# hyperplane-lab/RGBManip

Hardware: AMD Instinct MI355X
Metric: adapose_poses_per_sec_batch256 (higher is better)
Workload: dtype bf16

## Files before the change

### include/rgbm.h

```cpp
#ifndef RGBM_H_
#define RGBM_H_
#include <stddef.h>
#include <stdint.h>

#ifdef __cplusplus
extern "C" {
#endif

#define RGBM_VERSION 100
#define RGBM_F32 0
#define RGBM_BF16 1
#define RGBM_F16 2
#define RGBM_BF16X3 3

int rgbm_version(void);
const char* rgbm_last_error(void);

typedef struct rgbm_weight_desc {
  const char* name;
  const float* data;
  int ndim;
  const int64_t* shape;
} rgbm_weight_desc;

// ... 15 lines not shown
int rgbm_adapose_set_dropout(rgbm_adapose_t* h, float p, uint64_t seed);
int rgbm_adapose_dropout_masks(rgbm_adapose_t* h, int B, float* out_dev);
int rgbm_adapose_set_dropout_masks(rgbm_adapose_t* h, int B, const float* masks_dev);
int rgbm_adapose_forward(rgbm_adapose_t* h, int B, const float* img1, const float* img2, const int32_t* choose1,
                         const int32_t* choose2, const float* P1, const float* P2, const float* depths, void* workspace,
                         size_t workspace_bytes, const rgbm_adapose_out* out, void* stream);

int rgbm_adapose_postprocess(int B, int P, int img_size, const float* nocs1, const float* depth1, const float* r1,
                             const int32_t* choose1, const double* Kcrop, const double* E1, double* bbox_world, double* ts,
                             int32_t* valid, void* stream);
int rgbm_adapose_postprocess_scratch_bytes(int B, size_t* bytes);
int rgbm_adapose_postprocess_ws(int B, int P, int img_size, const float* nocs1, const float* depth1, const float* r1,
                                const int32_t* choose1, const double* Kcrop, const double* E1, double* bbox_world, double* ts,
                                int32_t* valid, void* scratch, size_t scratch_bytes, void* stream);

int rgbm_adapose_postprocess_regressed(int B, int P, const float* nocs1, const float* r1, const float* t1, const float* s1,
                                       const double* E1, double* bbox_world, double* ts, int32_t* valid, void* stream);

int rgbm_adapose_postprocess_ransac(int B, int P, int img_size, uint32_t seed, const float* nocs1, const float* depth1,
                                    const int32_t* choose1, const double* Kcrop, const double* E1, double* bbox_world, double* srt,
                                    int32_t* valid, void* stream);
int rgbm_adapose_postprocess_pnp(int B, int P, uint32_t seed, const float* nocs1, const float* pts2d1, const float* nocs2,
                                 const float* pts2d2, const double* K, const double* E1, const double* E2, double* bbox_out,
                                 double* srt_out, int32_t* info_out, int32_t* valid_out, void* stream);

int rgbm_prepare_inputs(const float* rgb_dev, const uint8_t* mask_dev, const double* K_dev, int N, int H, int W, int S, int P,
                        uint32_t seed, float* img_out, int32_t* choose_out, float* pts2d_out, double* Kcrop_out,
                        int32_t* window_out, int32_t* valid_out, uint8_t* scratch, void* stream);

int rgbm_prepare_inputs_indexed(const float* rgb_dev, const uint8_t* mask_dev, const double* K_dev, const int32_t* frame_map_dev,
                                int N, int H, int W, int S, int P, uint32_t seed, float* img_out, int32_t* choose_out,
                                float* pts2d_out, double* Kcrop_out, int32_t* window_out, int32_t* valid_out, uint8_t* scratch,
                                void* stream);
int rgbm_prepare_inputs_ex(const float* rgb_dev, const uint8_t* mask_dev, const double* K_dev, const int32_t* frame_map_dev,
                           int frame0, int N, int H, int W, int S, int P, uint32_t seed, float* img_out, int32_t* choose_out,
                           float* pts2d_out, double* Kcrop_out, int32_t* window_out, int32_t* valid_out, uint8_t* scratch,
                           void* stream);
int rgbm_prepare_inputs_u8(const uint8_t* rgb_dev, const uint8_t* mask_dev, const double* K_dev, const int32_t* frame_map_dev,
                           int frame0, int N, int H, int W, int S, int P, uint32_t seed, float* img_out, int32_t* choose_out,
                           float* pts2d_out, double* Kcrop_out, int32_t* window_out, int32_t* valid_out, uint8_t* scratch,
                           void* stream);
int rgbm_prepare_inputs_opt(const void* rgb_dev, int pixel_type, int normalize, const uint8_t* mask_dev, const double* K_dev,
                            const int32_t* frame_map_dev, int frame0, int N, int H, int W, int S, int P, uint32_t seed, float* img_out,
                            int32_t* choose_out, float* pts2d_out, double* Kcrop_out, int32_t* window_out, int32_t* valid_out,
                            uint8_t* scratch, void* stream);
int rgbm_prepare_inputs_windows(const void* pix_dev, int pixel_type, int normalize, const uint8_t* mask_pix_dev, const int64_t* offset_dev,
                                const int32_t* window_dev, const int32_t* valid_in_dev, const double* K_dev, int frame0, int N, int H, int W,
                                int S, int P, uint32_t seed, float* img_out, int32_t* choose_out, float* pts2d_out, double* Kcrop_out,
                                int32_t* valid_out, uint8_t* scratch, void* stream);
int rgbm_quantize_frames(const float* src_dev, uint8_t* dst_dev, size_t n, void* stream);

int rgbm_projection(const double* Kcrop_dev, const double* E_dev, float* P_dev, int N, void* stream);
int rgbm_mask_extent(const uint8_t* mask_dev, int N, int H, int W, int32_t* ext_out, int32_t* count_out, void* stream);

int rgbm_lookat_quat(const double* dir_dev, int N, int batch_zero, double* quat_dev, void* stream);
int rgbm_control_action_to_pose(const float* action_dev, int lda, const double* pose_mid, const double* pose_min,
                                const double* pose_max, int N, double* pose_dev, void* stream);
typedef struct rgbm_control_reward_args {
  const float* action;
  const double* cam_pose;
  const double* target;
  const float* move_success;
  const double* bbox;
  const double* avail;
  const double* gt_bbox;
  const double* pred_bbox;
  const double* pose_cur;
  const double* pose_prev;
  const double* robot_pose;
  const double* success;
  double* reward;
  double* terms;
  double coef[14];
  double proper_pos[3];
  double precision2;
  int N, T, lda, pots, first;
  int pad_;
} rgbm_control_reward_args;
int rgbm_control_reward(const rgbm_control_reward_args* args, void* stream);
int rgbm_control_grasp_frame(const double* est_dev, int N, double* center_dev, double* direction_dev, void* stream);

typedef struct rgbm_synth_scene {
  const double* cam_pose;
  const double* robot_pose;
  const double* box;
  double fx, fy, cx, cy;
  int N, H, W, env0;
} rgbm_synth_scene;
int rgbm_synth_camera(const rgbm_synth_scene* scene, double* K_dev, double* E_dev, double* rays_dev, void* stream);
int rgbm_synth_render(const rgbm_synth_scene* scene, const double* rays_dev, float* color_dev, uint8_t* mask_dev, void* stream);
int rgbm_synth_render_u8(const rgbm_synth_scene* scene, const double* rays_dev, uint8_t* color_dev, uint8_t* mask_dev,
                         int32_t* extent_dev, int32_t* count_dev, void* stream);

int rgbm_gae(int T, int N, const float* rewards, const uint8_t* dones, const float* values, const float* last_values,
             float gamma, float lam, float* returns, float* adv, double* sums, void* stream);
int rgbm_adv_normalise(int64_t n_local, float* adv, const double* sums, double count_total, void* stream);

typedef struct rgbm_policy_layout {
  int dims[5];
  int log_std;
  int w[2][4];
  int b[2][4];
  int total;
} rgbm_policy_layout;
int rgbm_policy_forward(const float* params, const rgbm_policy_layout* L, int n, int mode, const float* obs, const float* noise,
                        float* actions, float* logp, float* value, float* mu, void* stream);
int rgbm_ppo_partial_floats(const rgbm_policy_layout* L, int n, size_t* count);
int rgbm_ppo_minibatch_fwd_bwd(const float* params, const rgbm_policy_layout* L, int n, const float* obs, const float* actions,
                               const float* old_logp, const float* adv, const float* returns, const float* old_values,
                               const float* old_mu, const float* old_log_std, float clip, float vcoef, float ecoef,
                               float* partial_scratch, float* grads_flat, void* stream);
int rgbm_ppo_clip_adam(float* params, const float* grads_flat, float* exp_avg, float* exp_avg_sq, void* opt_state,
                       const rgbm_policy_layout* L, float inv_world, float max_norm, float desired_kl, float lr_min,
                       float lr_max, int adaptive, void* stream);

#define RGBM_POLICY_MAX_HIDDEN 6
#define RGBM_POLICY_MAX_WIDTH 512
#define RGBM_POLICY_MAX_ACT 32
#define RGBM_ACT_ELU 0
#define RGBM_ACT_SELU 1
#define RGBM_ACT_RELU 2
#define RGBM_ACT_LRELU 3
#define RGBM_ACT_TANH 4
#define RGBM_ACT_SIGMOID 5
typedef struct rgbm_policy_desc {
  int obs_dim, state_dim, act_dim;
  int activation;
  int asymmetric;
  int n_hidden[2];
  int hidden[2][RGBM_POLICY_MAX_HIDDEN];
  int w[2][RGBM_POLICY_MAX_HIDDEN + 1];
  int b[2][RGBM_POLICY_MAX_HIDDEN + 1];
  int log_std;
  int total;
} rgbm_policy_desc;
int rgbm_policy_forward_ex(const float* params, const rgbm_policy_desc* D, int n, int mode, const float* obs, const float* states,
                           const float* noise, float* actions, float* logp, float* value, float* mu, void* stream);
int rgbm_ppo_scratch_floats_ex(const rgbm_policy_desc* D, int n, int clipped_value_loss, size_t* count);
int rgbm_ppo_minibatch_fwd_bwd_ex(const float* params, const rgbm_policy_desc* D, int n, const float* obs, const float* states,
                                  const float* actions, const float* old_logp, const float* adv, const float* returns,
                                  const float* old_values, const float* old_mu, const float* old_log_std, float clip, float vcoef,
                                  float ecoef, int clipped_value_loss, float* scratch, float* grads_flat, void* stream);
int rgbm_ppo_clip_adam_ex(float* params, const float* grads_flat, float* exp_avg, float* exp_avg_sq, void* opt_state, int total,
                          float inv_world, float max_norm, float desired_kl, float lr_min, float lr_max, int adaptive, void* stream);

int rgbm_conv_nd(int dtype, const void* in_dev, int N, int D, int H, int W, int Cin, int Cin_pad, const float* w_host,
                 int Cout, int Cout_pad, int KD, int KH, int KW, int stride_d, int stride_hw, int pad_d, int pad_hw,
                 int dil_hw, int transposed, const float* bias_host, const float* bn_scale_host, const float* bn_shift_host,
                 const void* res_dev, int res_mode, int act, float slope, void* out_dev, void* stream);
#define RGBM_CONV_PLAN_INTS 9
int rgbm_conv_plan(int dtype, int N, int D, int H, int W, int Cin, int Cin_pad, int Cout, int Cout_pad, int KD, int KH, int KW,
                   int stride_d, int stride_hw, int pad_d, int pad_hw, int dil_hw, int transposed, int has_bias, int res_mode, int act,
                   int cls, int n_cu, int32_t* plan);
int rgbm_bn_per_sample_scratch_bytes(int V, size_t* bytes);
int rgbm_bn_per_sample(int dtype, void* y_dev, const void* res_dev, const float* gamma_dev, const float* beta_dev, void* scratch_dev,
                       int V, int64_t nvox, int C, int relu, void* stream);
int rgbm_conv3d_tile(int layer, int dtype, const void* in_dev, int N, int D, int H, int W, const float* w_host,
                     const float* bn_scale_host, const float* bn_shift_host, const void* res_dev, void* out_dev, void* stream);
int rgbm_upsample_conv3x3(int dtype, const void* in_dev, int V, int h, int w, int Cin, const float* w_host, int Cout,
                          const float* bias_host, int act, float slope, void* z_scratch_dev, void* out_dev, void* stream);
int rgbm_upsample_conv3x3_final(int dtype, const void* in_dev, int V, int h, int w, const float* w3_host, const float* b3_host,
                                float slope, const float* wf_host, const float* bf_host, void* out_dev, int out_f32, void* stream);
int rgbm_stem(int dtype, const float* img1_dev, const float* img2_dev, const float* w_host, void* out_dev, int B, int S, void* stream);
int rgbm_maxpool3x3s2(int dtype, const void* in_dev, void* out_dev, int V, int H, int W, int C, void* stream);
int rgbm_resize_bilinear_ac(int dtype, const void* in_dev, void* out_dev, int V, int Hs, int Ws, int C, int Ho, int Wo,
                            void* stream);
int rgbm_adaptive_avgpool(int dtype, const void* in_dev, void* out_dev, int V, int H, int W, int C, int S, void* stream);
int rgbm_build_volume(int dtype, const void* feat_dev, const float* P_views_dev, const float* depths_dev, float* homog_scratch,
                      void* vol_dev, int V, int B, int D, int H, int W, void* stream);
int rgbm_conv0_sweep(const void* feat_dev, const float* P_views_dev, const float* depths_dev, float* homog_scratch,
                     const float* w_host, const float* bn_scale_host, const float* bn_shift_host, void* out_dev,
                     int V, int B, int D, int H, int W, void* stream);
int rgbm_conv0_sweep_dt(int dtype, const void* feat_dev, const float* P_views_dev, const float* depths_dev, float* homog_scratch,
                        const float* w_host, const float* bn_scale_host, const float* bn_shift_host, void* out_dev,
                        int V, int B, int D, int H, int W, void* stream);
int rgbm_conv0_sweep_f16feat(const void* feat_f16_dev, const float* P_views_dev, const float* depths_dev, float* homog_scratch,
                             const float* w_host, const float* bn_scale_host, const float* bn_shift_host, void* out_bf16_dev,
                             int V, int B, int D, int H, int W, void* stream);
int rgbm_adapose_forward_ex(rgbm_adapose_t* h, int B, const float* img1, const float* img2, const int32_t* choose1,
                            const int32_t* choose2, const float* P1, const float* P2, const float* depths, void* workspace,
                            size_t workspace_bytes, const rgbm_adapose_out* out, int stop_after, void* stream);
int rgbm_adapose_forward_graph(rgbm_adapose_t* h, int B, const float* img1, const float* img2, const int32_t* choose1,
                               const int32_t* choose2, const float* P1, const float* P2, const float* depths, void* workspace,
                               size_t workspace_bytes, const rgbm_adapose_out* out, void* stream, int32_t* n_nodes, int32_t* captured);
int rgbm_adapose_graph_clear(rgbm_adapose_t* h);
int rgbm_adapose_feature_bytes(rgbm_adapose_t* h, size_t* bytes);
int rgbm_adapose_features_workspace_bytes(rgbm_adapose_t* h, int V, size_t* bytes);
int rgbm_adapose_features(rgbm_adapose_t* h, int V, const float* img, const int32_t* slots_dev, void* pool, int pool_records,
                          void* workspace, size_t workspace_bytes, void* stream);
int rgbm_adapose_forward_cached(rgbm_adapose_t* h, int B, const void* pool, int pool_records, const int32_t* slot1_dev,
                                const int32_t* slot2_dev, const int32_t* choose1, const int32_t* choose2, const float* P1, const float* P2,
                                const float* depths, void* workspace, size_t workspace_bytes, const rgbm_adapose_out* out, void* stream);
int rgbm_adapose_fetch(rgbm_adapose_t* h, int B, void* workspace, const char* name, float* out_dev, size_t capacity,
                       size_t* n_elems, void* stream);
int rgbm_crop_fingerprint(const float* img, int V, int n_words, uint64_t* keys_out, void* stream);

#define RGBM_PROF_ROWS 42
int rgbm_debug_flags(int flags);
int rgbm_set_tuning(const char* key, long long value);
int rgbm_microbench_mfma_scratch_floats(int* n);
int rgbm_microbench_mfma(float* scratch, int iters, int random_operands, double* flops, void* stream);
int rgbm_microbench_copy(const void* src, void* dst, size_t bytes, void* stream);
int rgbm_prof_rows(void);
int rgbm_prof_start(void);
int rgbm_prof_stop(double* stats);
int rgbm_prof_select(int row);

#ifdef __cplusplus
}
#endif
#endif
```

### rgbmanip_amd/_lib.py

```python
from __future__ import annotations

import ctypes as C
import os

_HERE = os.path.dirname(os.path.abspath(__file__))
LIB_PATH = os.environ.get("RGBM_HIP_LIB") or os.path.join(_HERE, "librgbm_hip.so")

F32, BF16, F16, BF16X3 = 0, 1, 2, 3
ACT_NONE, ACT_RELU, ACT_PRELU, ACT_TANH = 0, 1, 2, 3
RES_NONE, RES_PRE_ACT, RES_POST_ACT = 0, 1, 2


PROF_ROWS = 42
PROF_KERNELS = [
    ("conv_igemm_glds_kernel<float, 16, 256>", "fp32"), ("conv_igemm_glds_kernel<float, 32, 256>", "fp32"),
    ("conv_igemm_glds_kernel<float, 64, 256>", "fp32"), ("conv_igemm_glds_kernel<float, 128, 128>", "fp32"),
    ("conv_igemm_glds_kernel<unsigned short, 16, 256>", "bf16"), ("conv_igemm_glds_kernel<unsigned short, 32, 256>", "bf16"),
    ("conv_igemm_glds_kernel<unsigned short, 64, 256>", "bf16"), ("conv_igemm_glds_kernel<unsigned short, 128, 128>", "bf16"),
    ("conv3d_tile_kernel<float, ...> (conv1..conv11)", "fp32"), ("conv3d_tile_kernel<unsigned short, ...> (conv1..conv11)", "bf16"),
    ("conv3d_tile_kernel<float, 32, 16, 4, 8, 8, 1, false, true> (conv0 + fused plane sweep)", "fp32"),
    ("conv3d_tile_kernel<unsigned short, 32, 16, 4, 8, 8, 1, false, true> (conv0 + fused plane sweep)", "bf16"),
    ("conv_igemm_ws_kernel<float, ...>", "fp32"), ("conv_igemm_ws_kernel<unsigned short, false, false> (128 channels x 256 pixels)", "bf16"),
    ("conv0_sweep_persistent_kernel<unsigned short> (conv0 + fused plane sweep of bf16 nets; sweep_f16 = 0 / fp16 nets: conv0_sweep_kernel)", "bf16"), ("conv_igemm_ws64_kernel", "bf16"),
    ("conv3d_tile_kernel<unsigned short, 32, 16, 6, 8, 8, 1, false, false> (conv0 on a materialised volume)", "bf16"),
    ("conv3d_tile_kernel<unsigned short, 8, 16, 2, 8, 8, 2, false, false> (conv1)", "bf16"),
    ("conv3d_tile_kernel<unsigned short, 16, 16, 4, 8, 8, 1, false, false> (conv2)", "bf16"),
    ("conv3d_tile_kernel<unsigned short, 16, 32, 2, 8, 8, 2, false, false> (conv3)", "bf16"),
    ("conv3d_tile_kernel<unsigned short, 32, 32, 2, 8, 8, 1, false, false> (conv4)", "bf16"),
    ("conv3d_tile_kernel<unsigned short, 32, 64, 1, 8, 8, 2, false, false> (conv5)", "bf16"),
    ("conv3d_tile_kernel<unsigned short, 64, 64, 1, 8, 8, 1, false, false> (conv6)", "bf16"),
    ("conv3d_tile_kernel<unsigned short, 64, 32, 1, 8, 8, 1, true, false> (conv7)", "bf16"),
    ("conv3d_tile_kernel<unsigned short, 32, 16, 2, 8, 8, 1, true, false> (conv9)", "bf16"),
    ("conv3d_tile_kernel<unsigned short, 16, 16, 4, 8, 8, 1, true, false> (conv11)", "bf16"),
] + [("conv_igemm_glds_kernel<bx3_t, ...> (all channel tiles)", "bf16x3"), ("conv3d_tile_kernel<bx3_t, ...> (conv1..conv11)", "bf16x3"),
     ("conv0 + fused plane sweep <bx3_t>", "bf16x3"), ("conv_igemm_ws_kernel<rgbm::bx3_t, false, false> (128 channels x 256 pixels)", "bf16x3"),
     ("pose_mlp1_kernel (pose_mlp1.0 + pose_mlp1.2 of a bf16 net in one launch)", "bf16"),
     ("conv_igemm_m32_kernel<unsigned short, 256, 256> (256 channels x 256 pixels, 32x32x16 MFMAs; gemm_kernel = 0: conv_igemm_ws_kernel<unsigned short, true, false>, 256 x 128)", "bf16"),
     ("pose_mlp2_kernel (pose_mlp2.0 + pose_mlp2.2 + the sum over points of a bf16 net in one launch)", "bf16"),
     ("conv_igemm_m32_kernel<rgbm::bx3_t, 256, 256> (256 channels x 256 pixels, 32x32x16 MFMAs; gemm_kernel = 0: conv_igemm_ws_kernel<rgbm::bx3_t, true, false>, 256 x 128)", "bf16x3"),
     ("conv_igemm_ws_kernel<rgbm::bx3_t, false, false, true> (64 channels x 256 pixels, four multiply waves)", "bf16x3"),
     ("conv_igemm_ws_kernel<unsigned short, false, false, true> (64 channels x 256 pixels, four multiply waves)", "bf16"),
     ("conv_igemm_ws_kernel<float, false, false, true> (64 channels x 256 pixels, four multiply waves)", "fp32"),
     ("upconv_combine_kernel<16-bit> (PSPUpsample tap combination)", "bf16"), ("upconv_combine_kernel<4-byte> (PSPUpsample tap combination)", "bf16x3"),
     ("upconv_final_kernel (up_3 + final in one kernel; either storage width)", "bf16"),
     ("conv_igemm_m32_kernel<unsigned short, 128, 64 / 128 / 256> (128-pixel tiles: tail and small-batch launches of the 256-channel GEMM)", "bf16"),
     ("conv_igemm_m32_kernel<rgbm::bx3_t, 128, 64 / 128 / 256> (128-pixel tiles: tail and small-batch launches of the 256-channel GEMM)", "bf16x3")]
assert len(PROF_KERNELS) == PROF_ROWS


class RgbmError(RuntimeError):
    pass


class WeightDesc(C.Structure):
    _fields_ = [("name", C.c_char_p), ("data", C.c_void_p), ("ndim", C.c_int), ("shape", C.POINTER(C.c_int64))]


class PolicyLayout(C.Structure):
    _fields_ = [("dims", C.c_int * 5), ("log_std", C.c_int), ("w", (C.c_int * 4) * 2), ("b", (C.c_int * 4) * 2), ("total", C.c_int)]


POLICY_MAX_HIDDEN, POLICY_MAX_WIDTH, POLICY_MAX_ACT = 6, 512, 32
POLICY_ACTIVATIONS = {"elu": 0, "selu": 1, "relu": 2, "crelu": 2, "lrelu": 3, "tanh": 4, "sigmoid": 5}


class PolicyDesc(C.Structure):
    _fields_ = [("obs_dim", C.c_int), ("state_dim", C.c_int), ("act_dim", C.c_int), ("activation", C.c_int), ("asymmetric", C.c_int),
                ("n_hidden", C.c_int * 2), ("hidden", (C.c_int * POLICY_MAX_HIDDEN) * 2),
                ("w", (C.c_int * (POLICY_MAX_HIDDEN + 1)) * 2), ("b", (C.c_int * (POLICY_MAX_HIDDEN + 1)) * 2),
                ("log_std", C.c_int), ("total", C.c_int)]


class AdaposeOut(C.Structure):
    _fields_ = [(n, C.c_void_p) for n in ("view1_nocs", "view2_nocs", "view1_depth", "view2_depth", "view1_r", "view2_r",
                                           "view1_t", "view2_t", "view1_s", "view2_s")]


class ControlRewardArgs(C.Structure):
    _fields_ = [(n, C.c_void_p) for n in ("action", "cam_pose", "target", "move_success", "bbox", "avail", "gt_bbox", "pred_bbox",
                                           "pose_cur", "pose_prev", "robot_pose", "success", "reward", "terms")] + [
        ("coef", C.c_double * 14), ("proper_pos", C.c_double * 3), ("precision2", C.c_double),
        ("N", C.c_int), ("T", C.c_int), ("lda", C.c_int), ("pots", C.c_int), ("first", C.c_int), ("pad_", C.c_int)]


class SynthScene(C.Structure):
    _fields_ = [("cam_pose", C.c_void_p), ("robot_pose", C.c_void_p), ("box", C.c_void_p),
                ("fx", C.c_double), ("fy", C.c_double), ("cx", C.c_double), ("cy", C.c_double),
                ("N", C.c_int), ("H", C.c_int), ("W", C.c_int), ("env0", C.c_int)]


_vp, _i, _f, _d, _sz, _i64 = C.c_void_p, C.c_int, C.c_float, C.c_double, C.c_size_t, C.c_int64

SIGNATURES = {
    "rgbm_version": (_i, []),
    "rgbm_last_error": (C.c_char_p, []),
    "rgbm_adapose_create": (_i, [C.POINTER(_vp), _i, C.POINTER(WeightDesc), _i, _i, _i]),
    "rgbm_adapose_destroy": (_i, [_vp]),
    "rgbm_adapose_set_chunk": (_i, [_vp, _i]),
    "rgbm_adapose_set_option": (_i, [_vp, C.c_char_p, _i]),
    "rgbm_adapose_workspace_bytes": (_i, [_vp, _i, C.POINTER(_sz)]),
    "rgbm_adapose_set_dropout": (_i, [_vp, _f, C.c_uint64]),
    "rgbm_adapose_dropout_masks": (_i, [_vp, _i, _vp]),
    "rgbm_adapose_set_dropout_masks": (_i, [_vp, _i, _vp]),
    "rgbm_adapose_forward": (_i, [_vp, _i, _vp, _vp, _vp, _vp, _vp, _vp, _vp, _vp, _sz, C.POINTER(AdaposeOut), _vp]),
    "rgbm_adapose_forward_ex": (_i, [_vp, _i, _vp, _vp, _vp, _vp, _vp, _vp, _vp, _vp, _sz, C.POINTER(AdaposeOut), _i, _vp]),
    "rgbm_adapose_forward_graph": (_i, [_vp, _i, _vp, _vp, _vp, _vp, _vp, _vp, _vp, _vp, _sz, C.POINTER(AdaposeOut), _vp, C.POINTER(C.c_int32),
                                        C.POINTER(C.c_int32)]),
    "rgbm_adapose_graph_clear": (_i, [_vp]),
    "rgbm_adapose_feature_bytes": (_i, [_vp, C.POINTER(_sz)]),
    "rgbm_adapose_features_workspace_bytes": (_i, [_vp, _i, C.POINTER(_sz)]),
    "rgbm_adapose_features": (_i, [_vp, _i, _vp, _vp, _vp, _i, _vp, _sz, _vp]),
    "rgbm_adapose_forward_cached": (_i, [_vp, _i, _vp, _i, _vp, _vp, _vp, _vp, _vp, _vp, _vp, _vp, _sz, C.POINTER(AdaposeOut), _vp]),
    "rgbm_crop_fingerprint": (_i, [_vp, _i, _i, _vp, _vp]),
    "rgbm_adapose_fetch": (_i, [_vp, _i, _vp, C.c_char_p, _vp, _sz, C.POINTER(_sz), _vp]),
    "rgbm_adapose_postprocess": (_i, [_i, _i, _i, _vp, _vp, _vp, _vp, _vp, _vp, _vp, _vp, _vp, _vp]),
    "rgbm_adapose_postprocess_scratch_bytes": (_i, [_i, C.POINTER(_sz)]),
    "rgbm_adapose_postprocess_ws": (_i, [_i, _i, _i, _vp, _vp, _vp, _vp, _vp, _vp, _vp, _vp, _vp, _vp, _sz, _vp]),
    "rgbm_adapose_postprocess_regressed": (_i, [_i, _i, _vp, _vp, _vp, _vp, _vp, _vp, _vp, _vp, _vp]),
    "rgbm_adapose_postprocess_ransac": (_i, [_i, _i, _i, C.c_uint32, _vp, _vp, _vp, _vp, _vp, _vp, _vp, _vp, _vp]),
    "rgbm_adapose_postprocess_pnp": (_i, [_i, _i, C.c_uint32, _vp, _vp, _vp, _vp, _vp, _vp, _vp, _vp, _vp, _vp, _vp, _vp]),
    "rgbm_gae": (_i, [_i, _i, _vp, _vp, _vp, _vp, _f, _f, _vp, _vp, _vp, _vp]),
    "rgbm_adv_normalise": (_i, [_i64, _vp, _vp, _d, _vp]),
    "rgbm_policy_forward": (_i, [_vp, _vp, _i, _i, _vp, _vp, _vp, _vp, _vp, _vp, _vp]),
    "rgbm_ppo_partial_floats": (_i, [_vp, _i, C.POINTER(_sz)]),
    "rgbm_ppo_minibatch_fwd_bwd": (_i, [_vp, _vp, _i, _vp, _vp, _vp, _vp, _vp, _vp, _vp, _vp, _f, _f, _f, _vp, _vp, _vp]),
    "rgbm_ppo_clip_adam": (_i, [_vp, _vp, _vp, _vp, _vp, _vp, _f, _f, _f, _f, _f, _i, _vp]),
    "rgbm_policy_forward_ex": (_i, [_vp, _vp, _i, _i, _vp, _vp, _vp, _vp, _vp, _vp, _vp, _vp]),
    "rgbm_ppo_scratch_floats_ex": (_i, [_vp, _i, _i, C.POINTER(_sz)]),
    "rgbm_ppo_minibatch_fwd_bwd_ex": (_i, [_vp, _vp, _i, _vp, _vp, _vp, _vp, _vp, _vp, _vp, _vp, _vp, _f, _f, _f, _i, _vp, _vp, _vp]),
    "rgbm_ppo_clip_adam_ex": (_i, [_vp, _vp, _vp, _vp, _vp, _i, _f, _f, _f, _f, _f, _i, _vp]),
    "rgbm_conv_nd": (_i, [_i, _vp, _i, _i, _i, _i, _i, _i, _vp, _i, _i, _i, _i, _i, _i, _i, _i, _i, _i, _i, _vp, _vp, _vp,
                          _vp, _i, _i, _f, _vp, _vp]),
    "rgbm_conv_plan": (_i, [_i] * 23 + [C.POINTER(C.c_int32)]),
    "rgbm_bn_per_sample_scratch_bytes": (_i, [_i, C.POINTER(_sz)]),
    "rgbm_bn_per_sample": (_i, [_i, _vp, _vp, _vp, _vp, _vp, _i, _i64, _i, _i, _vp]),
    "rgbm_conv3d_tile": (_i, [_i, _i, _vp, _i, _i, _i, _i, _vp, _vp, _vp, _vp, _vp, _vp]),
    "rgbm_upsample_conv3x3": (_i, [_i, _vp, _i, _i, _i, _i, _vp, _i, _vp, _i, _f, _vp, _vp, _vp]),
    "rgbm_upsample_conv3x3_final": (_i, [_i, _vp, _i, _i, _i, _vp, _vp, _f, _vp, _vp, _vp, _i, _vp]),
    "rgbm_stem": (_i, [_i, _vp, _vp, _vp, _vp, _i, _i, _vp]),
    "rgbm_maxpool3x3s2": (_i, [_i, _vp, _vp, _i, _i, _i, _i, _vp]),
    "rgbm_resize_bilinear_ac": (_i, [_i, _vp, _vp, _i, _i, _i, _i, _i, _i, _vp]),
    "rgbm_adaptive_avgpool": (_i, [_i, _vp, _vp, _i, _i, _i, _i, _i, _vp]),
    "rgbm_build_volume": (_i, [_i, _vp, _vp, _vp, _vp, _vp, _i, _i, _i, _i, _i, _vp]),
    "rgbm_conv0_sweep": (_i, [_vp, _vp, _vp, _vp, _vp, _vp, _vp, _vp, _i, _i, _i, _i, _i, _vp]),
    "rgbm_conv0_sweep_dt": (_i, [_i, _vp, _vp, _vp, _vp, _vp, _vp, _vp, _vp, _i, _i, _i, _i, _i, _vp]),
    "rgbm_conv0_sweep_f16feat": (_i, [_vp, _vp, _vp, _vp, _vp, _vp, _vp, _vp, _i, _i, _i, _i, _i, _vp]),
    "rgbm_prepare_inputs": (_i, [_vp, _vp, _vp, _i, _i, _i, _i, _i, C.c_uint32, _vp, _vp, _vp, _vp, _vp, _vp, _vp, _vp]),
    "rgbm_prepare_inputs_indexed": (_i, [_vp, _vp, _vp, _vp, _i, _i, _i, _i, _i, C.c_uint32, _vp, _vp, _vp, _vp, _vp, _vp, _vp, _vp]),
    "rgbm_prepare_inputs_ex": (_i, [_vp, _vp, _vp, _vp, _i, _i, _i, _i, _i, _i, C.c_uint32, _vp, _vp, _vp, _vp, _vp, _vp, _vp, _vp]),
    "rgbm_prepare_inputs_u8": (_i, [_vp, _vp, _vp, _vp, _i, _i, _i, _i, _i, _i, C.c_uint32, _vp, _vp, _vp, _vp, _vp, _vp, _vp, _vp]),
    "rgbm_prepare_inputs_opt": (_i, [_vp, _i, _i, _vp, _vp, _vp, _i, _i, _i, _i, _i, _i, C.c_uint32, _vp, _vp, _vp, _vp, _vp, _vp, _vp, _vp]),
    "rgbm_prepare_inputs_windows": (_i, [_vp, _i, _i, _vp, _vp, _vp, _vp, _vp, _i, _i, _i, _i, _i, _i, C.c_uint32, _vp, _vp, _vp, _vp, _vp, _vp, _vp]),
    "rgbm_quantize_frames": (_i, [_vp, _vp, C.c_size_t, _vp]),
    "rgbm_projection": (_i, [_vp, _vp, _vp, _i, _vp]),
    "rgbm_mask_extent": (_i, [_vp, _i, _i, _i, _vp, _vp, _vp]),
    "rgbm_lookat_quat": (_i, [_vp, _i, _i, _vp, _vp]),
    "rgbm_control_action_to_pose": (_i, [_vp, _i, C.POINTER(C.c_double), C.POINTER(C.c_double), C.POINTER(C.c_double), _i, _vp, _vp]),
    "rgbm_control_reward": (_i, [C.POINTER(ControlRewardArgs), _vp]),
    "rgbm_control_grasp_frame": (_i, [_vp, _i, _vp, _vp, _vp]),
    "rgbm_synth_camera": (_i, [C.POINTER(SynthScene), _vp, _vp, _vp, _vp]),
    "rgbm_synth_render": (_i, [C.POINTER(SynthScene), _vp, _vp, _vp, _vp]),
    "rgbm_synth_render_u8": (_i, [C.POINTER(SynthScene), _vp, _vp, _vp, _vp, _vp, _vp]),
    "rgbm_debug_flags": (_i, [_i]),
    "rgbm_set_tuning": (_i, [C.c_char_p, _i64]),
    "rgbm_prof_rows": (_i, []),
    "rgbm_microbench_mfma_scratch_floats": (_i, [C.POINTER(C.c_int)]),
    "rgbm_microbench_mfma": (_i, [_vp, _i, _i, C.POINTER(C.c_double), _vp]),
    "rgbm_microbench_copy": (_i, [_vp, _vp, C.c_size_t, _vp]),
    "rgbm_prof_start": (_i, []),
    "rgbm_prof_select": (_i, [_i]),
    "rgbm_prof_stop": (_i, [C.POINTER(C.c_double)]),
}

_lib = None


def load():
    global _lib
    if _lib is not None:
        return _lib
    if not os.path.exists(LIB_PATH):
        raise RgbmError(f"{LIB_PATH} not found: build it with rgbmanip_amd/csrc/build.sh "
                        f"(or `python -c 'import __graft_entry__ as g; g.build()'`). There is no CPU fallback.")
    lib = C.CDLL(LIB_PATH)
    for name, (res, args) in SIGNATURES.items():
        fn = getattr(lib, name)
        fn.restype = res
        fn.argtypes = args
    if lib.rgbm_prof_rows() != PROF_ROWS:
        raise RgbmError(f"{LIB_PATH}: rgbm_prof_rows() = {lib.rgbm_prof_rows()}, this binding expects {PROF_ROWS} (stale build?)")
    _lib = lib
    return lib


def check(rc: int, what: str = ""):
    if rc != 0:
        msg = load().rgbm_last_error()
        raise RgbmError(f"{what} failed (code {rc}): {msg.decode() if msg else ''}")


def stream_ptr(stream=None):
    import torch
    s = stream if stream is not None else torch.cuda.current_stream()
    return C.c_void_p(s.cuda_stream)


def ptr(t):
    return C.c_void_p(t.data_ptr()) if t is not None else C.c_void_p(0)
```

### rgbmanip_amd/csrc/capi.cpp

```cpp
#include "../../include/rgbm.h"

#include <string.h>

#include <algorithm>
#include <string>
#include <vector>

#include "adapose.h"
#include "control.h"
#include "conv_plan.h"
#include "prof.h"

using namespace rgbm;

struct ForwardGraph {
  int B = 0;
  const void* in[7] = {nullptr};
  void* ws = nullptr;
  size_t ws_bytes = 0;
  rgbm_adapose_out out;
  int opt_version = 0;
  int tuning_version = 0;
  hipGraph_t graph = nullptr;
  hipGraphExec_t exec = nullptr;
  size_t nodes = 0;
  unsigned long long last_use = 0;
};

struct rgbm_adapose {
  AdaPose net;
  int device;
  int opt_version = 0;
  unsigned long long tick = 0;
  std::vector<ForwardGraph> graphs;
};
static const size_t kMaxGraphs = 8;

static int ensure_dropout_capacity(rgbm_adapose* h, int B) {
  AdaPose& n = h->net;
  if (2 * B <= n.drop_cap_views) return 0;
  const int views = std::max(2 * B, 2 * n.drop_cap_views);
  float* m = nullptr;
  RGBM_CHECK_HIP(hipMalloc(&m, (size_t)views * kDropoutPerView * sizeof(float)));
  if (n.drop_masks) {
    (void)hipDeviceSynchronize();
    (void)hipFree(n.drop_masks);
  }
  n.drop_masks = m;
  n.drop_cap_views = views;
  ++h->opt_version;
  return 0;
}

static void drop_graph(ForwardGraph& g) {
  if (g.exec) (void)hipGraphExecDestroy(g.exec);
  if (g.graph) (void)hipGraphDestroy(g.graph);
  g.exec = nullptr; g.graph = nullptr;
}


extern "C" {

int rgbm_version(void) { return RGBM_VERSION; }
const char* rgbm_last_error(void) { return last_error_cstr(); }

int rgbm_adapose_create(rgbm_adapose_t** h, int device, const rgbm_weight_desc* w, int n_w, int dtype, int norm_mode) {
  RGBM_REQUIRE(h != nullptr && w != nullptr && n_w > 0, "create arguments");
  RGBM_REQUIRE(dtype == RGBM_F32 || dtype == RGBM_BF16 || dtype == RGBM_F16 || dtype == RGBM_BF16X3, "dtype must be 0 (fp32), 1 (bf16), 2 (fp16) or 3 (bf16x3)");
  RGBM_REQUIRE(norm_mode == 0 || norm_mode == 1, "norm_mode: 0 = eval-mode (folded) BatchNorm3d, 1 = per-sample statistics");
  RGBM_CHECK_HIP(hipSetDevice(device));
  StateDict sd;
  for (int i = 0; i < n_w; ++i) {
    std::string name = w[i].name;
    if (name.rfind("module.", 0) == 0) name = name.substr(7);
    HostTensor t;
    t.data = w[i].data;
    for (int d = 0; d < w[i].ndim; ++d) t.shape.push_back(w[i].shape[d]);
    sd[name] = t;
  }
  rgbm_adapose* obj = new rgbm_adapose();
  obj->device = device;
  int rc = obj->net.create(sd, dtype, norm_mode);
  if (rc) { obj->net.destroy(); delete obj; return rc; }
  *h = obj;
  return 0;
}

int rgbm_adapose_destroy(rgbm_adapose_t* h) {
  if (!h) return 0;
  for (auto& g : h->graphs) drop_graph(g);
  h->net.destroy();
  delete h;
  return 0;
}

int rgbm_adapose_set_chunk(rgbm_adapose_t* h, int max_chunk_views) {
  RGBM_REQUIRE(h && max_chunk_views > 0, "set_chunk arguments");
  h->net.max_chunk = max_chunk_views;
  ++h->opt_version;
  return 0;
}

int rgbm_adapose_set_option(rgbm_adapose_t* h, const char* key, int value) {
  RGBM_REQUIRE(h && key, "set_option arguments");
  const std::string k = key;
  if (k == "max_chunk") { RGBM_REQUIRE(value > 0, "max_chunk"); h->net.max_chunk = value; }
  else if (k == "igemm_conv6") { RGBM_REQUIRE(value == 0 || value == 1, "igemm_conv6"); h->net.igemm_conv6 = value; }
  else if (k == "fuse_final") { RGBM_REQUIRE(value == 0 || value == 1, "fuse_final"); h->net.fuse_final = value; }
  else if (k == "sparse_tail") { RGBM_REQUIRE(value == 0 || value == 1, "sparse_tail"); h->net.sparse_tail = value; }
  else if (k == "upconv") { RGBM_REQUIRE(value >= 0 && value <= 7, "upconv"); h->net.upconv = value; }
  else if (k == "sparse_dec") { RGBM_REQUIRE(value >= 0 && value <= 2, "sparse_dec"); h->net.sparse_dec = value; }
  else if (k == "stem") { RGBM_REQUIRE(value == 0 || value == 1, "stem"); h->net.stem = value; }
  else if (k == "view2_heads") { RGBM_REQUIRE(value == 0 || value == 1, "view2_heads"); h->net.view2_heads = value; }
  else if (k == "sweep_f16") { RGBM_REQUIRE(value == 0 || value == 1, "sweep_f16"); h->net.sweep_f16 = value; }
  else if (k == "cost_impl") { RGBM_REQUIRE(value >= 0 && value <= 3, "cost_impl"); h->net.cost_impl = value; }
  else { set_error("unknown option " + k); return -1; }
  ++h->opt_version;
  return 0;
}

int rgbm_adapose_set_dropout(rgbm_adapose_t* h, float p, uint64_t seed) {
  RGBM_REQUIRE(h && (p == 0.f || (p > 0.f && p < 1.f)), "set_dropout: p must be 0 (off) or lie in (0, 1)");
  RGBM_CHECK_HIP(hipSetDevice(h->device));
  if (!h->net.drop_state) RGBM_CHECK_HIP(hipMalloc(&h->net.drop_state, 2 * sizeof(unsigned long long)));
  RGBM_CHECK_HIP(hipDeviceSynchronize());
  RGBM_CHECK_HIP(hipMemset(h->net.drop_state, 0, 2 * sizeof(unsigned long long)));
  RGBM_CHECK_HIP(hipDeviceSynchronize());
  h->net.drop_p = p;
  h->net.drop_seed = (unsigned long long)seed;
  ++h->opt_version;
  return 0;
}

int rgbm_adapose_dropout_masks(rgbm_adapose_t* h, int B, float* out_dev) {
  RGBM_REQUIRE(h && out_dev && B > 0, "dropout_masks arguments");
  RGBM_REQUIRE(h->net.drop_last_B == B && h->net.drop_masks, "dropout_masks: the last forward with dropout had batch " +
               std::to_string(h->net.drop_last_B) + ", not " + std::to_string(B));
  RGBM_CHECK_HIP(hipSetDevice(h->device));
  RGBM_CHECK_HIP(hipDeviceSynchronize());
  RGBM_CHECK_HIP(hipMemcpy(out_dev, h->net.drop_masks, (size_t)2 * B * kDropoutPerView * sizeof(float), hipMemcpyDeviceToDevice));
  return 0;
}

int rgbm_adapose_set_dropout_masks(rgbm_adapose_t* h, int B, const float* masks_dev) {
  RGBM_REQUIRE(h && masks_dev && B > 0, "set_dropout_masks arguments");
  RGBM_CHECK_HIP(hipSetDevice(h->device));
  if (int rc = ensure_dropout_capacity(h, B)) return rc;
  RGBM_CHECK_HIP(hipDeviceSynchronize());
  RGBM_CHECK_HIP(hipMemcpy(h->net.drop_masks, masks_dev, (size_t)2 * B * kDropoutPerView * sizeof(float), hipMemcpyDeviceToDevice));
  h->net.drop_explicit = B;
  return 0;
}

int rgbm_adapose_workspace_bytes(rgbm_adapose_t* h, int B, size_t* bytes) {
  RGBM_REQUIRE(h && bytes && B > 0, "workspace_bytes arguments");
  *bytes = h->net.workspace_bytes(B);
  return 0;
}

static AdaPose::Outputs to_out(const rgbm_adapose_out* o) {
  AdaPose::Outputs r;
  r.nocs1 = o->view1_nocs; r.nocs2 = o->view2_nocs; r.depth1 = o->view1_depth; r.depth2 = o->view2_depth;
  r.r1 = o->view1_r; r.r2 = o->view2_r; r.t1 = o->view1_t; r.t2 = o->view2_t; r.s1 = o->view1_s; r.s2 = o->view2_s;
// ... 64 lines not shown
    if (int rc = ensure_dropout_capacity(h, B)) return rc;
  if (prof_enabled() || h->net.drop_explicit) {
    if (captured) *captured = -1;
    return h->net.forward(B, img1, img2, choose1, choose2, P1, P2, depths, workspace, workspace_bytes, to_out(out), s, 0);
  }
  RGBM_REQUIRE(s != nullptr, "forward_graph: stream capture is not allowed on the default (null) stream; pass a created stream");
  const void* in[7] = {img1, img2, choose1, choose2, P1, P2, depths};
  ForwardGraph* hit = nullptr;
  for (size_t i = 0; i < h->graphs.size();) {
    ForwardGraph& g = h->graphs[i];
    if (g.opt_version != h->opt_version || g.tuning_version != g_tuning_version) {
      drop_graph(g);
      h->graphs.erase(h->graphs.begin() + i);
      continue;
    }
    if (g.B == B && !memcmp(g.in, in, sizeof(in)) && g.ws == workspace && g.ws_bytes == workspace_bytes &&
        !memcmp(&g.out, out, sizeof(*out))) hit = &g;
    ++i;
  }
  if (!hit) {
    h->net.drop_no_advance = 1;
    const int rw = h->net.forward(B, img1, img2, choose1, choose2, P1, P2, depths, workspace, workspace_bytes, to_out(out), s, 0);
    h->net.drop_no_advance = 0;
    if (rw) return rw;
    ForwardGraph g;
    g.B = B; memcpy(g.in, in, sizeof(in)); g.ws = workspace; g.ws_bytes = workspace_bytes; g.out = *out;
    g.opt_version = h->opt_version; g.tuning_version = g_tuning_version;
    RGBM_CHECK_HIP(hipStreamBeginCapture(s, hipStreamCaptureModeThreadLocal));
    const int rc = h->net.forward(B, img1, img2, choose1, choose2, P1, P2, depths, workspace, workspace_bytes, to_out(out), s, 0);
    const hipError_t ee = hipStreamEndCapture(s, &g.graph);
    if (rc) { if (g.graph) (void)hipGraphDestroy(g.graph); return rc; }
    if (ee != hipSuccess || !g.graph) { set_error(std::string("hipStreamEndCapture: ") + hipGetErrorString(ee)); return -2; }
    if (hipGraphGetNodes(g.graph, nullptr, &g.nodes) != hipSuccess) g.nodes = 0;
    const hipError_t ei = hipGraphInstantiate(&g.exec, g.graph, nullptr, nullptr, 0);
    if (ei != hipSuccess) { (void)hipGraphDestroy(g.graph); set_error(std::string("hipGraphInstantiate: ") + hipGetErrorString(ei)); return -2; }
    if (h->graphs.size() >= kMaxGraphs) {
      size_t lru = 0;
      for (size_t i = 1; i < h->graphs.size(); ++i) if (h->graphs[i].last_use < h->graphs[lru].last_use) lru = i;
      drop_graph(h->graphs[lru]);
      h->graphs.erase(h->graphs.begin() + lru);
    }
    h->graphs.push_back(g);
    hit = &h->graphs.back();
    if (captured) *captured = 1;
  }
  hit->last_use = ++h->tick;
  if (n_nodes) *n_nodes = (int32_t)hit->nodes;
  RGBM_CHECK_HIP(hipGraphLaunch(hit->exec, s));
  return 0;
}

int rgbm_adapose_fetch(rgbm_adapose_t* h, int B, void* workspace, const char* name, float* out_dev, size_t capacity,
                       size_t* n_elems, void* stream) {
  RGBM_REQUIRE(h && workspace && name && out_dev && n_elems, "fetch arguments");
  const AdaPose& n = h->net;
  Arena A(workspace, 0);
  AdaPose::Buffers bf;
  n.plan(B, A, bf);
  const size_t V = 2 * (size_t)B, S = n.img, P = n.n_pts, D = n.n_depth;
  const size_t Vc = n.chunk_views((int)V);
  const std::string nm = name;
  const void* src = nullptr; size_t cnt = 0; int dt = n.dtype;
  if (nm == "imgpad") { src = bf.imgpad; cnt = V * S * S * n.img_cpad; }
  else if (nm == "conv1") { src = bf.c1; cnt = V * (S / 2) * (S / 2) * 64; }
  else if (nm == "layer4") { src = bf.lb[n.last_f_index]; cnt = V * (S / 8) * (S / 8) * 512; }
  else if (nm == "cat") { src = bf.cat; cnt = V * (S / 8) * (S / 8) * 1024; }
  else if (nm == "u1") { src = bf.u1; cnt = V * (S / 4) * (S / 4) * 256; }
  else if (nm == "u2") { src = bf.u2; cnt = V * (S / 2) * (S / 2) * 64; }
  else if (nm == "u3") { src = bf.u3; cnt = V * S * S * 64; }
  else if (nm == "feat") { src = bf.feat; cnt = V * S * S * 32; if (n.feat_f32_only()) { src = bf.featf; dt = F32; } else if (n.feat_f16()) dt = F16; }
  else if (nm == "vol") { src = bf.vol; cnt = Vc * D * S * S * 32; }
  else if (nm == "c0") { src = bf.c[0]; cnt = Vc * D * S * S * 8; }
  else if (nm == "c2") { src = bf.c[2]; cnt = Vc * (D / 2) * (S / 2) * (S / 2) * 16; }
  else if (nm == "c4") { src = bf.c[4]; cnt = Vc * (D / 4) * (S / 4) * (S / 4) * 32; }
  else if (nm == "c6") { src = bf.c[6]; cnt = Vc * (D / 8) * (S / 8) * (S / 8) * 64; }
  else if (nm == "u7") { src = bf.u7; cnt = Vc * (D / 4) * (S / 4) * (S / 4) * 32; }
  else if (nm == "u9") { src = bf.u9; cnt = Vc * (D / 2) * (S / 2) * (S / 2) * 16; }
  else if (nm == "u11") { src = bf.u11; cnt = Vc * D * S * S * 8; }
  else if (nm == "homog") { src = bf.homog; cnt = V * 12; dt = F32; }
  else if (nm == "prob") { src = bf.prob; cnt = V * P * D; dt = F32; }
  else if (nm == "pf96") { src = bf.PF96; cnt = V * P * 96; dt = n.pose_dtype() == BF16X3 ? BF16X3 : F32; }
  else if (nm == "pf2") { src = bf.pf2; cnt = V * 256; dt = F32; }
  else if (nm == "r6") { src = bf.r6; cnt = V * 6; dt = F32; }
  RGBM_REQUIRE(src != nullptr, "unknown intermediate name: " + nm);
  const bool tap3d = nm == "c0" || nm == "c2" || nm == "c4" || nm == "c6" || nm == "u7" || nm == "u9";
  RGBM_REQUIRE(!(tap3d && n.sparse_active()), "tap '" + nm + "' needs a dense cost regularisation: set option sparse_dec = 0 before the forward "
               "(the default computes it only inside the chosen pixels' dependency cones)");
  *n_elems = cnt;
  RGBM_REQUIRE(cnt <= capacity, "fetch capacity too small");
  return launch_to_f32(dt, src, out_dev, (long long)cnt, (hipStream_t)stream);
}

int rgbm_adapose_postprocess(int B, int P, int img_size, const float* nocs1, const float* depth1, const float* r1,
                             const int32_t* choose1, const double* Kcrop, const double* E1, double* bbox_world, double* ts,
                             int32_t* valid, void* stream) {
  RGBM_REQUIRE(B > 0 && nocs1 && depth1 && r1 && choose1 && Kcrop && E1 && bbox_world && ts && valid, "postprocess arguments");
  return launch_postprocess(nocs1, depth1, r1, choose1, Kcrop, E1, bbox_world, ts, valid, B, P, img_size, (hipStream_t)stream);
}

int rgbm_adapose_postprocess_scratch_bytes(int B, size_t* bytes) {
  RGBM_REQUIRE(B > 0 && bytes, "postprocess_scratch_bytes arguments");
  *bytes = postprocess_slices(B) > 1 ? postprocess_scratch_bytes(B) : 0;
  return 0;
}

int rgbm_adapose_postprocess_ws(int B, int P, int img_size, const float* nocs1, const float* depth1, const float* r1,
                                const int32_t* choose1, const double* Kcrop, const double* E1, double* bbox_world, double* ts,
                                int32_t* valid, void* scratch, size_t scratch_bytes, void* stream) {
  RGBM_REQUIRE(B > 0 && nocs1 && depth1 && r1 && choose1 && Kcrop && E1 && bbox_world && ts && valid, "postprocess arguments");
  return launch_postprocess(nocs1, depth1, r1, choose1, Kcrop, E1, bbox_world, ts, valid, B, P, img_size, (hipStream_t)stream,
                            scratch, scratch_bytes);
}

int rgbm_adapose_postprocess_ransac(int B, int P, int img_size, uint32_t seed, const float* nocs1, const float* depth1,
                                    const int32_t* choose1, const double* Kcrop, const double* E1, double* bbox_world, double* srt,
                                    int32_t* valid, void* stream) {
  return launch_umeyama_ransac(nocs1, depth1, choose1, Kcrop, E1, bbox_world, srt, valid, B, P, img_size, seed, (hipStream_t)stream);
}

int rgbm_gae(int T, int N, const float* rewards, const uint8_t* dones, const float* values, const float* last_values,
             float gamma, float lam, float* returns, float* adv, double* sums, void* stream) {
  RGBM_REQUIRE(rewards && dones && values && last_values && returns && adv && sums, "gae arguments");
  return launch_gae(T, N, rewards, dones, values, last_values, gamma, lam, returns, adv, sums, (hipStream_t)stream);
}

int rgbm_adv_normalise(int64_t n_local, float* adv, const double* sums, double count_total, void* stream) {
  RGBM_REQUIRE(adv && sums && n_local > 0 && count_total > 1.0, "adv_normalise arguments");
  return launch_adv_normalise(n_local, adv, sums, count_total, (hipStream_t)stream);
}

static ConvGeom conv_nd_geom(int Cin, int Cout, int KD, int KH, int KW, int stride_d, int stride_hw, int pad_d, int pad_hw, int dil_hw,
                             int transposed, int act, float slope) {
  ConvGeom g;
  g.Cin = Cin; g.Cout = Cout; g.KD = KD; g.KH = KH; g.KW = KW;
  g.sd = stride_d; g.sh = g.sw = stride_hw; g.pd = pad_d; g.ph = g.pw = pad_hw;
  g.dild = 1; g.dilh = g.dilw = dil_hw; g.transposed = transposed != 0; g.act = act; g.slope = slope;
  return g;
}

int rgbm_conv_nd(int dtype, const void* in_dev, int N, int D, int H, int W, int Cin, int Cin_pad, const float* w_host,
                 int Cout, int Cout_pad, int KD, int KH, int KW, int stride_d, int stride_hw, int pad_d, int pad_hw,
                 int dil_hw, int transposed, const float* bias_host, const float* bn_scale_host, const float* bn_shift_host,
                 const void* res_dev, int res_mode, int act, float slope, void* out_dev, void* stream) {
  RGBM_REQUIRE(in_dev && w_host && out_dev, "conv arguments");
  const ConvGeom g = conv_nd_geom(Cin, Cout, KD, KH, KW, stride_d, stride_hw, pad_d, pad_hw, dil_hw, transposed, act, slope);
  ConvLayer L;
  int rc = L.init(dtype, g, w_host, bias_host, bn_scale_host, bn_shift_host, Cin_pad, Cout_pad);
  if (!rc) rc = L.run(in_dev, out_dev, N, D, H, W, Cout_pad, res_dev, res_mode, nullptr, 0, (hipStream_t)stream);
  if (!rc) { hipError_t e = hipStreamSynchronize((hipStream_t)stream); if (e != hipSuccess) { set_error(hipGetErrorString(e)); rc = -2; } }
  L.destroy();
  return rc;
}

int rgbm_conv_plan(int dtype, int N, int D, int H, int W, int Cin, int Cin_pad, int Cout, int Cout_pad, int KD, int KH, int KW,
                   int stride_d, int stride_hw, int pad_d, int pad_hw, int dil_hw, int transposed, int has_bias, int res_mode, int act,
                   int cls, int n_cu, int32_t* plan) {
  RGBM_REQUIRE(plan && n_cu >= 0 && dtype >= F32 && dtype <= BF16X3 && N > 0 && D > 0 && H > 0 && W > 0, "conv_plan arguments");
  const ConvGeom g = conv_nd_geom(Cin, Cout, KD, KH, KW, stride_d, stride_hw, pad_d, pad_hw, dil_hw, transposed, act, 0.f);
  PackedConv pc;
  if (int rc = conv_pack_geom(g, dtype, Cin_pad, Cout_pad, cls, &pc)) return rc;
  ConvDesc d;
  conv_desc_geom(d, g, pc, Cin_pad, Cout_pad, N, D, H, W, Cout_pad, cls);
  alignas(16) static const float buffer[4] = {};
  d.in = d.wgt = buffer; d.out = const_cast<float*>(buffer);
  d.bias = has_bias ? buffer : nullptr;
  d.res = res_mode != RES_NONE ? buffer : nullptr;
  d.res_mode = res_mode;
  ConvTuning t;
  ConvPlan p;
  if (int rc = conv_tuning(n_cu, &t)) return rc;
  if (int rc = plan_conv(d, dtype, t, &p)) return rc;
  const int32_t v[RGBM_CONV_PLAN_INTS] = {p.kernel, p.bch, p.bpix, p.ksplit, (int32_t)p.main_rows, p.tail_bch, p.identity_residual, (int32_t)d.M, d.KT};
  memcpy(plan, v, sizeof(v));
  return 0;
}

int rgbm_upsample_conv3x3(int dtype, const void* in_dev, int V, int h, int w, int Cin, const float* w_host, int Cout,
                          const float* bias_host, int act, float slope, void* z_scratch_dev, void* out_dev, void* stream) {
  RGBM_REQUIRE(in_dev && w_host && z_scratch_dev && out_dev, "upsample_conv3x3 arguments");
  UpConvLayer L;
  int rc = L.init(dtype, Cin, Cout, w_host, bias_host, act, slope);
  if (!rc) rc = L.run(in_dev, z_scratch_dev, out_dev, V, h, w, Cout, (hipStream_t)stream);
  if (!rc) { hipError_t e = hipStreamSynchronize((hipStream_t)stream); if (e != hipSuccess) { set_error(hipGetErrorString(e)); rc = -2; } }
  L.destroy();
  return rc;
}

int rgbm_upsample_conv3x3_final(int dtype, const void* in_dev, int V, int h, int w, const float* w3_host, const float* b3_host,
                                float slope, const float* wf_host, const float* bf_host, void* out_dev, int out_f32, void* stream) {
  RGBM_REQUIRE(in_dev && w3_host && b3_host && wf_host && bf_host && out_dev, "upsample_conv3x3_final arguments");
  UpConvFinal L;
  int rc = L.init(dtype, w3_host, b3_host, slope, wf_host, bf_host);
  if (!rc) rc = L.run(in_dev, out_dev, out_f32, V, h, w, (hipStream_t)stream);
  if (!rc) { hipError_t e = hipStreamSynchronize((hipStream_t)stream); if (e != hipSuccess) { set_error(hipGetErrorString(e)); rc = -2; } }
  L.destroy();
  return rc;
}

int rgbm_stem(int dtype, const float* img1_dev, const float* img2_dev, const float* w_host, void* out_dev, int B, int S, void* stream) {
  RGBM_REQUIRE(img1_dev && img2_dev && w_host && out_dev && B > 0, "stem arguments");
  std::vector<float> pk;
  stem_pack(w_host, pk);
  void* wd = nullptr;
  int rc = upload_packed(pk, dtype, &wd);
  if (!rc) rc = launch_stem(dtype, img1_dev, img2_dev, wd, out_dev, B, 2 * B, S, (hipStream_t)stream);
  if (!rc) { hipError_t e = hipStreamSynchronize((hipStream_t)stream); if (e != hipSuccess) { set_error(hipGetErrorString(e)); rc = -2; } }
  if (wd) (void)hipFree(wd);
  return rc;
}

int rgbm_bn_per_sample_scratch_bytes(int V, size_t* bytes) {
  RGBM_REQUIRE(V > 0 && bytes, "bn_per_sample_scratch_bytes arguments");
  *bytes = bn_scratch_bytes(V);
  return 0;
}
int rgbm_bn_per_sample(int dtype, void* y_dev, const void* res_dev, const float* gamma_dev, const float* beta_dev, void* scratch_dev,
                       int V, int64_t nvox, int C, int relu, void* stream) {
  RGBM_REQUIRE(y_dev && gamma_dev && beta_dev && scratch_dev, "bn_per_sample arguments");
  return launch_bn_per_sample(dtype, y_dev, res_dev, gamma_dev, beta_dev, scratch_dev, V, (long long)nvox, C, relu, (hipStream_t)stream);
}
int rgbm_maxpool3x3s2(int dtype, const void* in_dev, void* out_dev, int V, int H, int W, int C, void* stream) {
  return launch_maxpool3x3s2(dtype, in_dev, out_dev, V, H, W, C, (hipStream_t)stream);
}
int rgbm_resize_bilinear_ac(int dtype, const void* in_dev, void* out_dev, int V, int Hs, int Ws, int C, int Ho, int Wo,
                            void* stream) {
  return launch_resize_bilinear_ac(dtype, in_dev, out_dev, V, Hs, Ws, C, Ho, Wo, C, 0, (hipStream_t)stream);
}
int rgbm_adaptive_avgpool(int dtype, const void* in_dev, void* out_dev, int V, int H, int W, int C, int S, void* stream) {
  return launch_adaptive_avgpool(dtype, in_dev, out_dev, V, H, W, C, S, (hipStream_t)stream);
}
int rgbm_build_volume(int dtype, const void* feat_dev, const float* P_views_dev, const float* depths_dev, float* homog_scratch,
                      void* vol_dev, int V, int B, int D, int H, int W, void* stream) {
  if (int rc = launch_homography(P_views_dev, homog_scratch, V, B, (hipStream_t)stream)) return rc;
  return launch_build_volume(dtype, feat_dev, homog_scratch, depths_dev, vol_dev, 0, V, V, B, D, H, W, (hipStream_t)stream);
}

}

#include "prof.h"
extern "C" {
int rgbm_prof_rows(void) { return rgbm::kProfVariants; }
int rgbm_microbench_mfma_scratch_floats(int* n) {
  RGBM_REQUIRE(n, "microbench_mfma_scratch_floats arguments");
  return rgbm::microbench_mfma_scratch_floats(n);
}
int rgbm_microbench_mfma(float* scratch, int iters, int random_operands, double* flops, void* stream) {
  return rgbm::launch_microbench_mfma(scratch, iters, random_operands, flops, (hipStream_t)stream);
}
int rgbm_microbench_copy(const void* src, void* dst, size_t bytes, void* stream) {
  return rgbm::launch_microbench_copy(src, dst, bytes, (hipStream_t)stream);
}
int rgbm_prof_start(void) { return rgbm::prof_start(); }
int rgbm_prof_select(int row) {
  RGBM_REQUIRE(row >= -1 && row < rgbm::kProfVariants, "prof_select: row out of range");
  return rgbm::prof_select(row);
}
int rgbm_prof_stop(double* stats) {
  RGBM_REQUIRE(stats != nullptr, "prof_stop arguments");
  return rgbm::prof_stop(stats, rgbm::kProfVariants);
}
}

extern "C" int rgbm_conv3d_tile(int layer, int dtype, const void* in_dev, int N, int D, int H, int W, const float* w_host,
                                const float* bn_scale_host, const float* bn_shift_host, const void* res_dev, void* out_dev,
                                void* stream) {
  static const int cin[10] = {32, 8, 16, 16, 32, 32, 64, 64, 32, 16};
  static const int cout[10] = {8, 16, 16, 32, 32, 64, 64, 32, 16, 8};
  static const int stride[10] = {1, 2, 1, 2, 1, 2, 1, 1, 1, 1};
  RGBM_REQUIRE(layer >= 0 && layer < 10 && in_dev && w_host && bn_scale_host && bn_shift_host && out_dev, "conv3d_tile arguments");
  const bool tr = layer >= 7;
  const int coutp = cout[layer] < 16 ? 16 : cout[layer];
  std::vector<float> packed;
  conv3d_tile_pack(w_host, bn_scale_host, cin[layer], cout[layer], coutp, tr, dtype, packed);
  void* wdev = nullptr; float* bdev = nullptr;
  if (upload_packed(packed, dtype, &wdev)) return -2;
  std::vector<float> bpad(coutp, 0.f);
  for (int o = 0; o < cout[layer]; ++o) bpad[o] = bn_shift_host[o];
  if (upload_f32(bpad.data(), bpad.size(), &bdev)) return -2;
  Conv3dTileDesc d;
  memset(&d, 0, sizeof(d));
  d.in = in_dev; d.wgt = wdev; d.out = out_dev; d.bias = bdev; d.res = res_dev;
  d.N = N; d.Di = D; d.Hi = H; d.Wi = W;
  if (tr) { d.Do = 2 * D; d.Ho = 2 * H; d.Wo = 2 * W; d.Dq = D; d.Hq = H; d.Wq = W; }
  else {
    const int s = stride[layer];
    d.Do = (D + 2 - 3) / s + 1; d.Ho = (H + 2 - 3) / s + 1; d.Wo = (W + 2 - 3) / s + 1;
    d.Dq = d.Do; d.Hq = d.Ho; d.Wq = d.Wo;
  }
  d.Cout = cout[layer]; d.relu = 1; d.prof_variant = -1;
  int rc = launch_conv3d_tile(layer, dtype, d, (hipStream_t)stream);
  if (!rc) { hipError_t e = hipStreamSynchronize((hipStream_t)stream); if (e != hipSuccess) { set_error(hipGetErrorString(e)); rc = -2; } }
  (void)hipFree(wdev); (void)hipFree(bdev);
  return rc;
}

static int conv0_sweep_entry(int dtype, int feat_f16, const void* feat_dev, const float* P_views_dev, const float* depths_dev,
                             float* homog_scratch, const float* w_host, const float* bn_scale_host, const float* bn_shift_host,
                             void* out_dev, int V, int B, int D, int H, int W, void* stream) {
  RGBM_REQUIRE(feat_dev && P_views_dev && depths_dev && homog_scratch && w_host && bn_scale_host && bn_shift_host && out_dev,
               "conv0_sweep arguments");
  RGBM_REQUIRE(dtype == BF16 || dtype == F16 || dtype == BF16X3, "conv0_sweep: 16-bit storage types or bf16x3 (fp32 features in, split-pair c0 out)");
  if (int rc = launch_homography(P_views_dev, homog_scratch, V, B, (hipStream_t)stream)) return rc;
  std::vector<float> packed;
  conv0_sweep_pack(w_host, bn_scale_host, packed);
  void* wdev = nullptr; float* bdev = nullptr;
  if (dtype == BF16X3) { if (conv0_sweep_x3_upload(packed, &wdev)) return -2; }
  else if (upload_packed(packed, feat_f16 ? (int)F16 : dtype, &wdev)) return -2;
  std::vector<float> bpad(16, 0.f);
  for (int o = 0; o < 8; ++o) bpad[o] = bn_shift_host[o];
  if (upload_f32(bpad.data(), bpad.size(), &bdev)) return -2;
  Conv3dTileDesc d;
  memset(&d, 0, sizeof(d));
  d.wgt = wdev; d.out = out_dev; d.bias = bdev;
  d.N = V; d.Di = D; d.Hi = H; d.Wi = W; d.Do = D; d.Ho = H; d.Wo = W; d.Dq = D; d.Hq = H; d.Wq = W;
  d.Cout = 8; d.relu = 1; d.prof_variant = -1;
  d.feat = feat_dev; d.homog = homog_scratch; d.depths = depths_dev; d.v0 = 0; d.V = V; d.B = B;
  d.feat_f16 = feat_f16;
  int rc = dtype == BF16X3 ? launch_conv0_sweep_x3(d, (hipStream_t)stream) : launch_conv0_sweep(d, dtype, (hipStream_t)stream);
  if (!rc) { hipError_t e = hipStreamSynchronize((hipStream_t)stream); if (e != hipSuccess) { set_error(hipGetErrorString(e)); rc = -2; } }
  (void)hipFree(wdev); (void)hipFree(bdev);
  return rc;
}

extern "C" int rgbm_conv0_sweep_dt(int dtype, const void* feat_dev, const float* P_views_dev, const float* depths_dev,
                                   float* homog_scratch, const float* w_host, const float* bn_scale_host, const float* bn_shift_host,
                                   void* out_dev, int V, int B, int D, int H, int W, void* stream) {
  return conv0_sweep_entry(dtype, 0, feat_dev, P_views_dev, depths_dev, homog_scratch, w_host, bn_scale_host, bn_shift_host, out_dev, V, B, D,
                           H, W, stream);
}

extern "C" int rgbm_conv0_sweep_f16feat(const void* feat_f16_dev, const float* P_views_dev, const float* depths_dev,
                                        float* homog_scratch, const float* w_host, const float* bn_scale_host,
                                        const float* bn_shift_host, void* out_bf16_dev, int V, int B, int D, int H, int W, void* stream) {
  return conv0_sweep_entry(BF16, 1, feat_f16_dev, P_views_dev, depths_dev, homog_scratch, w_host, bn_scale_host, bn_shift_host, out_bf16_dev,
                           V, B, D, H, W, stream);
}

extern "C" int rgbm_conv0_sweep(const void* feat_dev, const float* P_views_dev, const float* depths_dev, float* homog_scratch,
                                const float* w_host, const float* bn_scale_host, const float* bn_shift_host, void* out_dev,
                                int V, int B, int D, int H, int W, void* stream) {
  return rgbm_conv0_sweep_dt(BF16, feat_dev, P_views_dev, depths_dev, homog_scratch, w_host, bn_scale_host, bn_shift_host, out_dev,
                             V, B, D, H, W, stream);
}

extern "C" int rgbm_prepare_inputs(const float* rgb_dev, const uint8_t* mask_dev, const double* K_dev, int N, int H, int W, int S,
                                   int P, uint32_t seed, float* img_out, int32_t* choose_out, float* pts2d_out, double* Kcrop_out,
                                   int32_t* window_out, int32_t* valid_out, uint8_t* scratch, void* stream) {
  return launch_prepare_inputs(rgb_dev, mask_dev, K_dev, nullptr, N, H, W, S, P, seed, img_out, choose_out, pts2d_out, Kcrop_out,
                               window_out, valid_out, scratch, (hipStream_t)stream);
}

extern "C" int rgbm_prepare_inputs_indexed(const float* rgb_dev, const uint8_t* mask_dev, const double* K_dev,
                                           const int32_t* frame_map_dev, int N, int H, int W, int S, int P, uint32_t seed,
                                           float* img_out, int32_t* choose_out, float* pts2d_out, double* Kcrop_out,
                                           int32_t* window_out, int32_t* valid_out, uint8_t* scratch, void* stream) {
  RGBM_REQUIRE(frame_map_dev, "prepare_inputs_indexed frame_map");
  return launch_prepare_inputs(rgb_dev, mask_dev, K_dev, frame_map_dev, N, H, W, S, P, seed, img_out, choose_out, pts2d_out,
                               Kcrop_out, window_out, valid_out, scratch, (hipStream_t)stream);
}

extern "C" int rgbm_prepare_inputs_ex(const float* rgb_dev, const uint8_t* mask_dev, const double* K_dev, const int32_t* frame_map_dev,
                                      int frame0, int N, int H, int W, int S, int P, uint32_t seed, float* img_out, int32_t* choose_out,
                                      float* pts2d_out, double* Kcrop_out, int32_t* window_out, int32_t* valid_out, uint8_t* scratch,
                                      void* stream) {
  RGBM_REQUIRE(frame0 >= 0, "prepare_inputs_ex frame0");
  return launch_prepare_inputs(rgb_dev, mask_dev, K_dev, frame_map_dev, N, H, W, S, P, seed, img_out, choose_out, pts2d_out,
                               Kcrop_out, window_out, valid_out, scratch, (hipStream_t)stream, frame0);
}

extern "C" int rgbm_prepare_inputs_u8(const uint8_t* rgb_dev, const uint8_t* mask_dev, const double* K_dev, const int32_t* frame_map_dev,
                                      int frame0, int N, int H, int W, int S, int P, uint32_t seed, float* img_out, int32_t* choose_out,
                                      float* pts2d_out, double* Kcrop_out, int32_t* window_out, int32_t* valid_out, uint8_t* scratch,
                                      void* stream) {
  RGBM_REQUIRE(frame0 >= 0, "prepare_inputs_u8 frame0");
  return launch_prepare_inputs_u8(rgb_dev, mask_dev, K_dev, frame_map_dev, N, H, W, S, P, seed, img_out, choose_out, pts2d_out,
                                  Kcrop_out, window_out, valid_out, scratch, (hipStream_t)stream, frame0);
}

extern "C" int rgbm_prepare_inputs_opt(const void* rgb_dev, int pixel_type, int normalize, const uint8_t* mask_dev, const double* K_dev,
                                       const int32_t* frame_map_dev, int frame0, int N, int H, int W, int S, int P, uint32_t seed,
                                       float* img_out, int32_t* choose_out, float* pts2d_out, double* Kcrop_out, int32_t* window_out,
                                       int32_t* valid_out, uint8_t* scratch, void* stream) {
  RGBM_REQUIRE(frame0 >= 0, "prepare_inputs_opt frame0");
  return launch_prepare_inputs_opt(rgb_dev, pixel_type, normalize, mask_dev, K_dev, frame_map_dev, N, H, W, S, P, seed, img_out, choose_out,
                                   pts2d_out, Kcrop_out, window_out, valid_out, scratch, (hipStream_t)stream, frame0);
}

extern "C" int rgbm_prepare_inputs_windows(const void* pix_dev, int pixel_type, int normalize, const uint8_t* mask_pix_dev,
                                           const int64_t* offset_dev, const int32_t* window_dev, const int32_t* valid_in_dev, const double* K_dev,
                                           int frame0, int N, int H, int W, int S, int P, uint32_t seed, float* img_out, int32_t* choose_out,
                                           float* pts2d_out, double* Kcrop_out, int32_t* valid_out, uint8_t* scratch, void* stream) {
  static_assert(sizeof(int64_t) == sizeof(long long), "offset table");
  return launch_prepare_inputs_windows(pix_dev, pixel_type, normalize, mask_pix_dev, reinterpret_cast<const long long*>(offset_dev), window_dev,
                                       valid_in_dev, K_dev, frame0, N, H, W, S, P, seed, img_out, choose_out, pts2d_out, Kcrop_out, valid_out,
                                       scratch, (hipStream_t)stream);
}

extern "C" int rgbm_adapose_postprocess_regressed(int B, int P, const float* nocs1, const float* r1, const float* t1, const float* s1,
                                                  const double* E1, double* bbox_out, double* ts_out, int32_t* valid_out, void* stream) {
  return launch_postprocess_regressed(nocs1, r1, t1, s1, E1, bbox_out, ts_out, valid_out, B, P, (hipStream_t)stream);
}

extern "C" int rgbm_quantize_frames(const float* src_dev, uint8_t* dst_dev, size_t n, void* stream) {
  return launch_quantize_frames(src_dev, dst_dev, n, (hipStream_t)stream);
}

extern "C" int rgbm_adapose_postprocess_pnp(int B, int P, uint32_t seed, const float* nocs1, const float* pts2d1, const float* nocs2,
                                            const float* pts2d2, const double* K, const double* E1, const double* E2, double* bbox_out,
                                            double* srt_out, int32_t* info_out, int32_t* valid_out, void* stream) {
  return launch_pnp_ransac(nocs1, pts2d1, nocs2, pts2d2, K, E1, E2, bbox_out, srt_out, info_out, valid_out, B, P, seed, (hipStream_t)stream);
}

extern "C" int rgbm_projection(const double* Kcrop_dev, const double* E_dev, float* P_dev, int N, void* stream) {
  return launch_projection(Kcrop_dev, E_dev, P_dev, N, (hipStream_t)stream);
}

extern "C" int rgbm_mask_extent(const uint8_t* mask_dev, int N, int H, int W, int32_t* ext_out, int32_t* count_out, void* stream) {
  return launch_mask_extent(mask_dev, N, H, W, ext_out, count_out, (hipStream_t)stream);
}

static_assert(sizeof(rgbm_control_reward_args) == sizeof(rgbm::ControlRewardArgs), "control reward args ABI mismatch");
static_assert(sizeof(rgbm_synth_scene) == sizeof(rgbm::SynthScene), "synth scene ABI mismatch");
extern "C" int rgbm_lookat_quat(const double* dir_dev, int N, int batch_zero, double* quat_dev, void* stream) {
  return rgbm::launch_lookat_quat(dir_dev, quat_dev, N, batch_zero, (hipStream_t)stream);
}
extern "C" int rgbm_control_action_to_pose(const float* action_dev, int lda, const double* pose_mid, const double* pose_min,
                                           const double* pose_max, int N, double* pose_dev, void* stream) {
  return rgbm::launch_control_action(action_dev, lda, pose_mid, pose_min, pose_max, pose_dev, N, (hipStream_t)stream);
}
extern "C" int rgbm_control_reward(const rgbm_control_reward_args* args, void* stream) {
  RGBM_REQUIRE(args, "control_reward args");
  return rgbm::launch_control_reward(*reinterpret_cast<const rgbm::ControlRewardArgs*>(args), (hipStream_t)stream);
}
extern "C" int rgbm_control_grasp_frame(const double* est_dev, int N, double* center_dev, double* direction_dev, void* stream) {
  return rgbm::launch_control_grasp_frame(est_dev, center_dev, direction_dev, N, (hipStream_t)stream);
}
extern "C" int rgbm_synth_camera(const rgbm_synth_scene* scene, double* K_dev, double* E_dev, double* rays_dev, void* stream) {
  RGBM_REQUIRE(scene, "synth_camera scene");
  return rgbm::launch_synth_camera(*reinterpret_cast<const rgbm::SynthScene*>(scene), K_dev, E_dev, rays_dev, (hipStream_t)stream);
}
extern "C" int rgbm_synth_render(const rgbm_synth_scene* scene, const double* rays_dev, float* color_dev, uint8_t* mask_dev,
                                 void* stream) {
  RGBM_REQUIRE(scene, "synth_render scene");
  return rgbm::launch_synth_render(*reinterpret_cast<const rgbm::SynthScene*>(scene), rays_dev, color_dev, mask_dev,
                                   (hipStream_t)stream);
}
extern "C" int rgbm_synth_render_u8(const rgbm_synth_scene* scene, const double* rays_dev, uint8_t* color_dev, uint8_t* mask_dev,
                                    int32_t* extent_dev, int32_t* count_dev, void* stream) {
  RGBM_REQUIRE(scene, "synth_render_u8 scene");
  return rgbm::launch_synth_render_u8(*reinterpret_cast<const rgbm::SynthScene*>(scene), rays_dev, color_dev, mask_dev, extent_dev,
                                      count_dev, (hipStream_t)stream);
}

extern "C" int rgbm_debug_flags(int flags) { rgbm::g_debug_flags = flags; ++rgbm::g_tuning_version; return 0; }

extern "C" int rgbm_set_tuning(const char* key, long long value) {
  RGBM_REQUIRE(key != nullptr, "set_tuning arguments");
  const std::string k = key;
  if (k == "ws_min_rows") { RGBM_REQUIRE(value >= 0, "ws_min_rows"); rgbm::g_ws_min_rows = value; }
  else if (k == "gemm_kernel") { RGBM_REQUIRE(value >= 0 && value <= 2, "gemm_kernel"); rgbm::g_gemm_kernel = (int)value; }
  else { set_error("unknown tuning key " + k); return -1; }
  ++rgbm::g_tuning_version;
  return 0;
}

static_assert(sizeof(rgbm_policy_layout) == sizeof(rgbm::PolicyLayout), "policy layout ABI mismatch");
static_assert(sizeof(rgbm::PolicyOptState) == 40 || sizeof(rgbm::PolicyOptState) == 48, "opt state size");
extern "C" {
int rgbm_policy_forward(const float* params, const rgbm_policy_layout* L, int n, int mode, const float* obs, const float* noise,
                        float* actions, float* logp, float* value, float* mu, void* stream) {
  RGBM_REQUIRE(params && L && obs && mu, "policy_forward arguments");
  RGBM_REQUIRE(mode == 1 || (logp && value && actions), "policy_forward outputs");
  RGBM_REQUIRE(mode != 0 || noise, "policy_forward: act needs noise");
  return launch_policy_forward(params, *reinterpret_cast<const PolicyLayout*>(L), n, mode, obs, noise, actions, logp, value, mu,
                               (hipStream_t)stream);
}
int rgbm_ppo_partial_floats(const rgbm_policy_layout* L, int n, size_t* count) {
  RGBM_REQUIRE(L && count && n > 0, "ppo_partial_floats arguments");
  *count = (size_t)policy_partial_floats(*reinterpret_cast<const PolicyLayout*>(L), n);
  return 0;
}
int rgbm_ppo_minibatch_fwd_bwd(const float* params, const rgbm_policy_layout* L, int n, const float* obs, const float* actions,
                               const float* old_logp, const float* adv, const float* returns, const float* old_values,
                               const float* old_mu, const float* old_log_std, float clip, float vcoef, float ecoef,
                               float* partial_scratch, float* grads_flat, void* stream) {
  RGBM_REQUIRE(params && L && obs && actions && old_logp && adv && returns && old_values && old_mu && old_log_std &&
               partial_scratch && grads_flat, "ppo_minibatch arguments");
  return launch_ppo_minibatch(params, *reinterpret_cast<const PolicyLayout*>(L), n, obs, actions, old_logp, adv, returns,
                              old_values, old_mu, old_log_std, clip, vcoef, ecoef, partial_scratch, grads_flat, (hipStream_t)stream);
}
static_assert(sizeof(rgbm_policy_desc) == sizeof(rgbm::PolicyDesc), "policy desc ABI mismatch");
static_assert(RGBM_POLICY_MAX_HIDDEN == rgbm::POLICY_MAX_HIDDEN && RGBM_POLICY_MAX_WIDTH == rgbm::POLICY_MAX_WIDTH &&
                  RGBM_POLICY_MAX_ACT == rgbm::POLICY_MAX_ACT && RGBM_ACT_ELU == rgbm::PACT_ELU && RGBM_ACT_SIGMOID == rgbm::PACT_SIGMOID,
              "policy desc constants");

int rgbm_policy_forward_ex(const float* params, const rgbm_policy_desc* D, int n, int mode, const float* obs, const float* states,
                           const float* noise, float* actions, float* logp, float* value, float* mu, void* stream) {
  RGBM_REQUIRE(params && D && obs && mu, "policy_forward_ex arguments");
  RGBM_REQUIRE(mode == 1 || (logp && value && actions), "policy_forward_ex outputs");
  RGBM_REQUIRE(mode != 0 || noise, "policy_forward_ex: act needs noise");
  return launch_policy_forward_ex(params, *reinterpret_cast<const PolicyDesc*>(D), n, mode, obs, states, noise, actions, logp, value,
                                  mu, (hipStream_t)stream);
}
int rgbm_ppo_scratch_floats_ex(const rgbm_policy_desc* D, int n, int clipped_value_loss, size_t* count) {
  RGBM_REQUIRE(D && count && n > 0, "ppo_scratch_floats_ex arguments");
  return ppo_scratch_floats_ex(*reinterpret_cast<const PolicyDesc*>(D), n, clipped_value_loss, count);
}
int rgbm_ppo_minibatch_fwd_bwd_ex(const float* params, const rgbm_policy_desc* D, int n, const float* obs, const float* states,
                                  const float* actions, const float* old_logp, const float* adv, const float* returns,
                                  const float* old_values, const float* old_mu, const float* old_sigma, float clip, float vcoef,
                                  float ecoef, int clipped_value_loss, float* scratch, float* grads_flat, void* stream) {
  RGBM_REQUIRE(params && D && obs && actions && old_logp && adv && returns && old_mu && old_sigma && scratch && grads_flat,
               "ppo_minibatch_ex arguments");
  return launch_ppo_minibatch_ex(params, *reinterpret_cast<const PolicyDesc*>(D), n, obs, states, actions, old_logp, adv, returns,
                                 old_values, old_mu, old_sigma, clip, vcoef, ecoef, clipped_value_loss, scratch, grads_flat,
                                 (hipStream_t)stream);
}
int rgbm_ppo_clip_adam_ex(float* params, const float* grads_flat, float* exp_avg, float* exp_avg_sq, void* opt_state, int total,
                          float inv_world, float max_norm, float desired_kl, float lr_min, float lr_max, int adaptive, void* stream) {
  RGBM_REQUIRE(params && grads_flat && exp_avg && exp_avg_sq && opt_state && total > 0, "ppo_clip_adam_ex arguments");
  return launch_ppo_adam(params, grads_flat, exp_avg, exp_avg_sq, reinterpret_cast<PolicyOptState*>(opt_state), total, inv_world,
                         max_norm, desired_kl, lr_min, lr_max, adaptive, (hipStream_t)stream);
}
int rgbm_ppo_clip_adam(float* params, const float* grads_flat, float* exp_avg, float* exp_avg_sq, void* opt_state,
                       const rgbm_policy_layout* L, float inv_world, float max_norm, float desired_kl, float lr_min,
                       float lr_max, int adaptive, void* stream) {
  RGBM_REQUIRE(params && grads_flat && exp_avg && exp_avg_sq && opt_state && L, "ppo_clip_adam arguments");
  return launch_ppo_adam(params, grads_flat, exp_avg, exp_avg_sq, reinterpret_cast<PolicyOptState*>(opt_state), L->total,
                         inv_world, max_norm, desired_kl, lr_min, lr_max, adaptive, (hipStream_t)stream);
}
}
```

### rgbmanip_amd/csrc/common.h

```cpp
#pragma once
#include <hip/hip_runtime.h>
#include <stdint.h>
#include <stdio.h>
#include <string>

namespace rgbm {

enum DType { F32 = 0, BF16 = 1, F16 = 2, BF16X3 = 3 };
enum Act { ACT_NONE = 0, ACT_RELU = 1, ACT_PRELU = 2, ACT_TANH = 3 };
enum ResMode { RES_NONE = 0, RES_PRE_ACT = 1, RES_POST_ACT = 2 };

typedef __attribute__((ext_vector_type(8))) __bf16 bf16x8;
typedef _Float16 f16_t;
typedef __attribute__((ext_vector_type(8))) _Float16 f16x8;
typedef __attribute__((ext_vector_type(4))) _Float16 f16x4;
typedef __attribute__((ext_vector_type(8))) float f32x8;
typedef __attribute__((ext_vector_type(4))) float f32x4;

void set_error(const std::string& s);
int fail(const char* what, const char* file, int line);

#define RGBM_CHECK_HIP(expr)                                                             \
  do {                                                                                   \
    hipError_t _e = (expr);                                                              \
// ... 37 lines not shown

template <typename T> struct Elem;
template <> struct Elem<float> {
  static constexpr int kPerChunk = 4;
  __device__ static __forceinline__ float ld(const float* p) { return *p; }
  __device__ static __forceinline__ void st(float* p, float v) { *p = v; }
};
template <> struct Elem<unsigned short> {
  static constexpr int kPerChunk = 8;
  __device__ static __forceinline__ float ld(const unsigned short* p) { return bf16_to_f32(*p); }
  __device__ static __forceinline__ void st(unsigned short* p, float v) { *p = f32_to_bf16(v); }
};

template <> struct Elem<f16_t> {
  static constexpr int kPerChunk = 8;
  __device__ static __forceinline__ float ld(const f16_t* p) { return (float)*p; }
  __device__ static __forceinline__ void st(f16_t* p, float v) { *p = (f16_t)(v != v ? v : fminf(fmaxf(v, -65504.f), 65504.f)); }
};
struct bx3_t { unsigned raw; };

__device__ __forceinline__ uint4 bx3_split4(float a, float b, float c, float d) {
  uint4 o;
  o.x = pack2_bf16(a, b);
  o.y = pack2_bf16(c, d);
  o.z = pack2_bf16(a - __uint_as_float(o.x << 16), b - __uint_as_float(o.x & 0xffff0000u));
  o.w = pack2_bf16(c - __uint_as_float(o.y << 16), d - __uint_as_float(o.y & 0xffff0000u));
  return o;
}
__device__ __forceinline__ void bx3_join4(const uint4& c, float* v) {
  v[0] = __uint_as_float(c.x << 16) + __uint_as_float(c.z << 16);
  v[1] = __uint_as_float(c.x & 0xffff0000u) + __uint_as_float(c.z & 0xffff0000u);
  v[2] = __uint_as_float(c.y << 16) + __uint_as_float(c.w << 16);
  v[3] = __uint_as_float(c.y & 0xffff0000u) + __uint_as_float(c.w & 0xffff0000u);
}
template <> struct Elem<bx3_t> {
  static constexpr int kPerChunk = 4;
  __device__ static __forceinline__ float ld(const bx3_t* p) {
    const unsigned long long a = (unsigned long long)p;
    const unsigned short* ch = reinterpret_cast<const unsigned short*>(a & ~15ull);
    const int e = (int)((a >> 2) & 3);
    return bf16_to_f32(ch[e]) + bf16_to_f32(ch[4 + e]);
  }
  __device__ static __forceinline__ void st(bx3_t* p, float v) {
    const unsigned long long a = (unsigned long long)p;
    unsigned short* ch = reinterpret_cast<unsigned short*>(a & ~15ull);
    const int e = (int)((a >> 2) & 3);
    const unsigned short h = f32_to_bf16(v);
    ch[e] = h;
    ch[4 + e] = f32_to_bf16(v - bf16_to_f32(h));
  }
};

__device__ __forceinline__ float sat_f16(float v) { return v != v ? v : fminf(fmaxf(v, -65504.f), 65504.f); }

__device__ __forceinline__ void load4(const float* p, float v[4]) {
  float4 t = *reinterpret_cast<const float4*>(p);
  v[0] = t.x; v[1] = t.y; v[2] = t.z; v[3] = t.w;
}
__device__ __forceinline__ void load4(const unsigned short* p, float v[4]) {
  uint2 t = *reinterpret_cast<const uint2*>(p);
  v[0] = __uint_as_float(t.x << 16); v[1] = __uint_as_float(t.x & 0xffff0000u);
  v[2] = __uint_as_float(t.y << 16); v[3] = __uint_as_float(t.y & 0xffff0000u);
}
__device__ __forceinline__ void load4(const f16_t* p, float v[4]) {
  const f16x4 t = *reinterpret_cast<const f16x4*>(p);
  v[0] = (float)t[0]; v[1] = (float)t[1]; v[2] = (float)t[2]; v[3] = (float)t[3];
}
__device__ __forceinline__ void store4(f16_t* p, const float v[4]) {
  f16x4 t;
  t[0] = (f16_t)sat_f16(v[0]); t[1] = (f16_t)sat_f16(v[1]); t[2] = (f16_t)sat_f16(v[2]); t[3] = (f16_t)sat_f16(v[3]);
  *reinterpret_cast<f16x4*>(p) = t;
}
__device__ __forceinline__ void store4(float* p, const float v[4]) {
  *reinterpret_cast<float4*>(p) = make_float4(v[0], v[1], v[2], v[3]);
}
__device__ __forceinline__ void store4(unsigned short* p, const float v[4]) {
  uint2 t;
  t.x = pack2_bf16(v[0], v[1]);
  t.y = pack2_bf16(v[2], v[3]);
  *reinterpret_cast<uint2*>(p) = t;
}
__device__ __forceinline__ void load4(const bx3_t* p, float v[4]) { bx3_join4(*reinterpret_cast<const uint4*>(p), v); }
__device__ __forceinline__ void store4(bx3_t* p, const float v[4]) { *reinterpret_cast<uint4*>(p) = bx3_split4(v[0], v[1], v[2], v[3]); }
__device__ __forceinline__ void unpack_chunk(const uint4& c, float* v, bx3_t ) { bx3_join4(c, v); }
__device__ __forceinline__ uint4 pack_chunk(const float* v, bx3_t ) { return bx3_split4(v[0], v[1], v[2], v[3]); }
__device__ __forceinline__ void unpack_chunk(const uint4& c, float* v, float ) {
  v[0] = __uint_as_float(c.x); v[1] = __uint_as_float(c.y); v[2] = __uint_as_float(c.z); v[3] = __uint_as_float(c.w);
}
__device__ __forceinline__ void unpack_chunk(const uint4& c, float* v, unsigned short ) {
  v[0] = __uint_as_float(c.x << 16); v[1] = __uint_as_float(c.x & 0xffff0000u);
  v[2] = __uint_as_float(c.y << 16); v[3] = __uint_as_float(c.y & 0xffff0000u);
  v[4] = __uint_as_float(c.z << 16); v[5] = __uint_as_float(c.z & 0xffff0000u);
  v[6] = __uint_as_float(c.w << 16); v[7] = __uint_as_float(c.w & 0xffff0000u);
}
__device__ __forceinline__ void unpack_chunk(const uint4& c, float* v, f16_t ) {
  const f16x8 h = __builtin_bit_cast(f16x8, c);
#pragma unroll
  for (int e = 0; e < 8; ++e) v[e] = (float)h[e];
}
__device__ __forceinline__ uint4 pack_chunk(const float* v, f16_t ) {
  f16x8 h;
#pragma unroll
  for (int e = 0; e < 8; ++e) h[e] = (f16_t)sat_f16(v[e]);
  return __builtin_bit_cast(uint4, h);
}
__device__ __forceinline__ uint4 pack_chunk(const float* v, float ) {
  return make_uint4(__float_as_uint(v[0]), __float_as_uint(v[1]), __float_as_uint(v[2]), __float_as_uint(v[3]));
}
__device__ __forceinline__ uint4 pack_chunk(const float* v, unsigned short ) {
  uint4 c;
  c.x = pack2_bf16(v[0], v[1]);
  c.y = pack2_bf16(v[2], v[3]);
  c.z = pack2_bf16(v[4], v[5]);
  c.w = pack2_bf16(v[6], v[7]);
  return c;
}

typedef __attribute__((ext_vector_type(4))) short rgbm_s16x4;
__device__ __forceinline__ f32x4 mma_bx3_k16(const uint4& a, const uint4& b, f32x4 c) {
  const rgbm_s16x4 ah = __builtin_bit_cast(rgbm_s16x4, make_uint2(a.x, a.y)), al = __builtin_bit_cast(rgbm_s16x4, make_uint2(a.z, a.w));
  const rgbm_s16x4 bh = __builtin_bit_cast(rgbm_s16x4, make_uint2(b.x, b.y)), bl = __builtin_bit_cast(rgbm_s16x4, make_uint2(b.z, b.w));
  c = __builtin_amdgcn_mfma_f32_16x16x16bf16_1k(al, bh, c, 0, 0, 0);
  c = __builtin_amdgcn_mfma_f32_16x16x16bf16_1k(ah, bl, c, 0, 0, 0);
  c = __builtin_amdgcn_mfma_f32_16x16x16bf16_1k(ah, bh, c, 0, 0, 0);
  return c;
}
__device__ __forceinline__ void bx3_pair(const uint4& c0, const uint4& c1, uint4& hi, uint4& lo) {
  hi = make_uint4(c0.x, c0.y, c1.x, c1.y);
  lo = make_uint4(c0.z, c0.w, c1.z, c1.w);
}

struct ConvDesc {
  const void* in; const void* wgt; void* out; const float* bias; const void* res;
  int N, Di, Hi, Wi, Cin, lcin;
  int Dq, Hq, Wq;
  int sd, sh, sw, pd, ph, pw;
  int KD, KH, KW, dild, dilh, dilw;
  int ntaps, KT, Kpad;
  int Cout, ldo;
  int Do, Ho, Wo;
  int osd, osh, osw, opd, oph, opw;
  int act; float slope; int res_mode; int bias_stride;
  long long M;
  int n_pix_tiles, n_ch_tiles;
  int n_tiles; unsigned fd_m[3]; int fd_s[3];
  int korder;
  int buf_ok;
  const void* ident;
  long long m0;
  const void* w2; const float* bias2; void* out2; int ldo2, cout2, kpad2, act2; float slope2;
  double algo_flops, algo_bytes;
  int out_f32;
  int ksplit; float* kscratch; unsigned* kcount;
};

int launch_conv(const ConvDesc& d, int dtype, hipStream_t s);
bool conv_ws64_eligible(const ConvDesc& d, int dtype);
int conv_ch_tile(int Cout);
int conv_bk(int dtype);

}
```

### rgbmanip_amd/csrc/conv_igemm_glds.hip

```cpp
#include <map>
#include <mutex>
#include <type_traits>
#include <vector>
#include "common.h"
#include "conv_plan.h"
#include "kernels.h"
#include "prof.h"

#ifndef WS_BUF
#define WS_BUF 1
#endif

namespace rgbm {

int g_gemm_kernel = 2;
__device__ uint4 g_zero_page[4];

typedef __attribute__((address_space(3))) void* lds_ptr_t;
typedef const __attribute__((address_space(1))) void* gbl_ptr_t;

__device__ __forceinline__ void glds16(const void* gsrc, unsigned lds_off) {
  asm volatile("s_mov_b32 m0, %1\n\ts_nop 0\n\tglobal_load_lds_dwordx4 %0, off" :: "v"(gsrc), "s"(lds_off) : "memory");
}
__device__ __forceinline__ void blds16(unsigned voff, const __amdgpu_buffer_rsrc_t& rsrc, unsigned soff, unsigned lds_off) {
  asm volatile("s_mov_b32 m0, %3\n\ts_nop 0\n\tbuffer_load_dwordx4 %0, %1, %2 offen lds" :: "v"(voff), "s"(rsrc), "s"(soff), "s"(lds_off) : "memory");
}
__device__ __forceinline__ unsigned lds_addr(const void* p) {
  return (unsigned)(unsigned long long)(__attribute__((address_space(3))) const void*)p;
}

#define RGBM_BARRIER() do { asm volatile("" ::: "memory"); __builtin_amdgcn_s_barrier(); asm volatile("" ::: "memory"); } while (0)

template <typename T> struct MmaG;
template <> struct MmaG<unsigned short> {
  __device__ static __forceinline__ void run(const uint4& a, const uint4& b, f32x4& c) {
    c = __builtin_amdgcn_mfma_f32_16x16x32_bf16(__builtin_bit_cast(bf16x8, a), __builtin_bit_cast(bf16x8, b), c, 0, 0, 0);
  }
  __device__ static __forceinline__ f32x4 run2(const uint4& a, const uint4& b, const f32x4& c) {
    return __builtin_amdgcn_mfma_f32_16x16x32_bf16(__builtin_bit_cast(bf16x8, a), __builtin_bit_cast(bf16x8, b), c, 0, 0, 0);
  }
};
template <> struct MmaG<f16_t> {
  __device__ static __forceinline__ void run(const uint4& a, const uint4& b, f32x4& c) {
    c = __builtin_amdgcn_mfma_f32_16x16x32_f16(__builtin_bit_cast(f16x8, a), __builtin_bit_cast(f16x8, b), c, 0, 0, 0);
  }
  __device__ static __forceinline__ f32x4 run2(const uint4& a, const uint4& b, const f32x4& c) {
    return __builtin_amdgcn_mfma_f32_16x16x32_f16(__builtin_bit_cast(f16x8, a), __builtin_bit_cast(f16x8, b), c, 0, 0, 0);
  }
};
template <> struct MmaG<float> {
  __device__ static __forceinline__ void run(const uint4& a, const uint4& b, f32x4& c) {
    c = __builtin_amdgcn_mfma_f32_16x16x4f32(__uint_as_float(a.x), __uint_as_float(b.x), c, 0, 0, 0);
    c = __builtin_amdgcn_mfma_f32_16x16x4f32(__uint_as_float(a.y), __uint_as_float(b.y), c, 0, 0, 0);
    c = __builtin_amdgcn_mfma_f32_16x16x4f32(__uint_as_float(a.z), __uint_as_float(b.z), c, 0, 0, 0);
    c = __builtin_amdgcn_mfma_f32_16x16x4f32(__uint_as_float(a.w), __uint_as_float(b.w), c, 0, 0, 0);
  }
};

template <> struct MmaG<bx3_t> {
  __device__ static __forceinline__ void run(const uint4& a, const uint4& b, f32x4& c) { c = mma_bx3_k16(a, b, c); }
};
template <typename T> constexpr int prof_row_generic(int bch) {
  return std::is_same<T, bx3_t>::value ? 26 : (sizeof(T) == 2 ? 4 : 0) + (bch == 16 ? 0 : bch == 32 ? 1 : bch == 64 ? 2 : 3);
}
template <typename T> constexpr int prof_row_ws() { return std::is_same<T, bx3_t>::value ? 29 : sizeof(T) == 2 ? 13 : 12; }

template <int FM, int FN>
__device__ __forceinline__ void mma_bx3_tile(const uint4 (&a0)[FM], const uint4 (&a1)[FM], const uint4 (&b0)[FN], const uint4 (&b1)[FN],
                                             f32x4 (&acc)[FM][FN]) {
  uint4 ah[FM], al[FM], bh[FN], bl[FN];
#pragma unroll
  for (int a = 0; a < FM; ++a) bx3_pair(a0[a], a1[a], ah[a], al[a]);
#pragma unroll
  for (int b = 0; b < FN; ++b) bx3_pair(b0[b], b1[b], bh[b], bl[b]);
#pragma unroll
  for (int a = 0; a < FM; ++a)
#pragma unroll
    for (int b = 0; b < FN; ++b) MmaG<unsigned short>::run(al[a], bh[b], acc[a][b]);
#pragma unroll
  for (int a = 0; a < FM; ++a)
#pragma unroll
    for (int b = 0; b < FN; ++b) MmaG<unsigned short>::run(ah[a], bl[b], acc[a][b]);
#pragma unroll
  for (int a = 0; a < FM; ++a)
#pragma unroll
    for (int b = 0; b < FN; ++b) MmaG<unsigned short>::run(ah[a], bh[b], acc[a][b]);
}

template <int OFF>
__device__ __forceinline__ void lds_rd8(uint2& dst, unsigned addr) {
  asm volatile("ds_read_b64 %0, %1 offset:%2" : "=v"(dst) : "v"(addr), "n"(OFF) : "memory");
}

template <int FM, int FN>
__device__ __forceinline__ void mma_bx3_ops(const uint4 (&ah)[FM], const uint4 (&al)[FM], const uint4 (&bh)[FN], const uint4 (&bl)[FN],
                                            f32x4 (&acc)[FM][FN]) {
#pragma unroll
  for (int a = 0; a < FM; ++a)
#pragma unroll
    for (int b = 0; b < FN; ++b) MmaG<unsigned short>::run(al[a], bh[b], acc[a][b]);
#pragma unroll
  for (int a = 0; a < FM; ++a)
#pragma unroll
    for (int b = 0; b < FN; ++b) MmaG<unsigned short>::run(ah[a], bl[b], acc[a][b]);
#pragma unroll
  for (int a = 0; a < FM; ++a)
#pragma unroll
    for (int b = 0; b < FN; ++b) MmaG<unsigned short>::run(ah[a], bh[b], acc[a][b]);
}

template <int N> struct IC { static constexpr int value = N; };

__device__ __forceinline__ float apply_act_g(float v, int act, float slope) {
  if (act == ACT_RELU) return v < 0.f ? 0.f : v;
  if (act == ACT_PRELU) return v < 0.f ? v * slope : v;
  if (act == ACT_TANH) return tanhf(v);
  return v;
}

template <typename T, int BCH, int BPIX, bool UNI>
__global__ __launch_bounds__(256, 2) void conv_igemm_glds_kernel(const ConvDesc d) {
  constexpr int E = 16 / sizeof(T);
  constexpr int BK = 8 * E;
  constexpr int XR = BPIX / 32;
  constexpr int WL = BCH >= 32 ? BCH / 32 : 1;
  constexpr int WCH = BCH < 64 ? BCH : 64;
  constexpr int FM = WCH / 16;
  constexpr int FN = 4;
  constexpr int STAGE = (BCH + BPIX) * 8;
  __shared__ uint4 lds[2 * STAGE];

  const int tid = threadIdx.x;
  const int lane = tid & 63;
  const int wave = __builtin_amdgcn_readfirstlane(tid >> 6);

  const int nblk = gridDim.x;
  const int bq = nblk >> 3, br = nblk & 7;
  const int xcd = blockIdx.x & 7, bidx = blockIdx.x >> 3;
  const int lid = (xcd < br ? xcd * (bq + 1) : br * (bq + 1) + (xcd - br) * bq) + bidx;
  const int pix_tile = lid / d.n_ch_tiles;
  const int ch_tile = lid - pix_tile * d.n_ch_tiles;

  const T* __restrict__ in = reinterpret_cast<const T*>(d.in);
  const T* __restrict__ wgt = reinterpret_cast<const T*>(d.wgt);

  const int j = tid & 7;
  const int r0 = tid >> 3;
  const int js = j ^ ((r0 >> 1) & 7);
  int xn[XR], xd0[XR], xh0[XR], xw0[XR];
  const char* rowp[XR];
  unsigned rmask[XR];
#pragma unroll
  for (int i = 0; i < XR; ++i) {
    const long long m = (long long)pix_tile * BPIX + r0 + 32 * i;
    if (m < d.M) {
      unsigned t = (unsigned)m;
      const unsigned qw = t % (unsigned)d.Wq; t /= (unsigned)d.Wq;
      const unsigned qh = t % (unsigned)d.Hq; t /= (unsigned)d.Hq;
      const unsigned qd = t % (unsigned)d.Dq; t /= (unsigned)d.Dq;
      xn[i] = (int)t * d.Di;
      xd0[i] = (int)qd * d.sd - d.pd;
      xh0[i] = (int)qh * d.sh - d.ph;
      xw0[i] = (int)qw * d.sw - d.pw;
    } else {
      xn[i] = 0; xd0[i] = -(1 << 20); xh0[i] = 0; xw0[i] = 0;
    }
    if (UNI) {
      unsigned mk = 0;
// ... 1376 lines not shown
        RGBM_BARRIER();
        const uint4* W = lds3 + (st & 1) * STAGE;
        const uint4* X = W + HWROWS * 8;
#pragma unroll
        for (int kw = 0; kw < 3; ++kw) {
#pragma unroll
          for (int s2 = 0; s2 < 2; ++s2) {
            const int cidx = s2 * 4 + lg;
            uint4 af[FM], bf[FN];
#pragma unroll
            for (int a = 0; a < FM; ++a) {
              const int row = kw * 64 + a * 16 + lr;
              af[a] = W[row * 8 + (cidx ^ ((row >> 1) & 7))];
            }
#pragma unroll
            for (int b = 0; b < FN; ++b) {
              const int row = wpix + b * 16 + lr + kw * dil;
              const bool edge = kw == 0 ? eL[b] : (kw == 2 ? eR[b] : false);
              const uint4* src = edge ? zrow + cidx : X + row * 8 + (cidx ^ ((row >> 1) & 7));
              bf[b] = *src;
            }
#pragma unroll
            for (int a = 0; a < FM; ++a)
#pragma unroll
              for (int b = 0; b < FN; ++b) MmaG<T>::run(af[a], bf[b], acc[a][b]);
          }
        }
        ++st;
      }
    } else {
    for (int kt = 0; kt < KT; ++kt) {
      asm volatile("s_waitcnt lgkmcnt(0)" ::: "memory");
      RGBM_BARRIER();
      load_half(st, 0, af0, bf0);
      __builtin_amdgcn_sched_barrier(0);
      if (kt > 0) mma_half(af1, bf1);
      __builtin_amdgcn_sched_barrier(0);
      load_half(st, 1, af1, bf1);
      __builtin_amdgcn_sched_barrier(0);
      mma_half(af0, bf0);
      __builtin_amdgcn_sched_barrier(0);
      st = st == 2 ? 0 : st + 1;
    }
    mma_half(af1, bf1);
    }
    if (bias_lds && d.act != ACT_TANH) {
      const float slope = d.slope;
      auto pack_tile = [&](auto actc) {
        constexpr int ACT = decltype(actc)::value;
#pragma unroll
        for (int b = 0; b < FN; ++b) {
          const int row = wpix + b * 16 + lr;
#pragma unroll
          for (int a = 0; a < FM; ++a) {
            float v[4];
#pragma unroll
            for (int e = 0; e < 4; ++e) {
              const float x = acc[a][b][e];
              v[e] = ACT == ACT_RELU ? (x < 0.f ? 0.f : x) : ACT == ACT_PRELU ? (x < 0.f ? x * slope : x) : x;
            }
            store4(reinterpret_cast<T*>(stg + row * SROW + (a * 16 + lg * 4) * 2), v);
          }
        }
      };
      if (d.act == ACT_RELU) pack_tile(IC<ACT_RELU>{});
      else if (d.act == ACT_PRELU) pack_tile(IC<ACT_PRELU>{});
      else pack_tile(IC<ACT_NONE>{});
      continue;
    }
    const int pix_tile = tile_of(k);
#pragma unroll
    for (int b = 0; b < FN; ++b) {
      const int row = wpix + b * 16 + lr;
      int n = 0;
      if (d.bias && d.bias_stride != 0) {
        const long long m = (long long)pix_tile * BPIX + row;
        unsigned nn, qd, qh, qw;
        decode_row(d, m < d.M ? (unsigned)m : 0u, nn, qd, qh, qw);
        n = (int)nn;
      }
#pragma unroll
      for (int a = 0; a < FM; ++a) {
        const int ch = a * 16 + lg * 4;
        float v[4] = {acc[a][b][0], acc[a][b][1], acc[a][b][2], acc[a][b][3]};
        if (d.bias && !bias_lds && ch < d.Cout) {
          const float* bp = d.bias + (long long)n * d.bias_stride + ch;
#pragma unroll
          for (int e = 0; e < 4; ++e) v[e] += bp[e];
        }
#pragma unroll
        for (int e = 0; e < 4; ++e) v[e] = apply_act_g(v[e], d.act, d.slope);
        store4(reinterpret_cast<T*>(stg + row * SROW + ch * 2), v);
      }
    }
  }
  asm volatile("s_waitcnt lgkmcnt(0)" ::: "memory");
  RGBM_BARRIER();
}

template <typename T>
static int launch_ws64(ConvDesc d, bool rh, hipStream_t s) {
  constexpr int BCH = 64, BPIX = 256;
  const size_t LDS = (rh ? 2 * (size_t)(3 * BCH + 264) * 8 * sizeof(uint4) + 128 + (size_t)BPIX * 144
                         : 3 * (size_t)(BCH + BPIX) * 8 * sizeof(uint4) + (size_t)BPIX * 144) + BCH * sizeof(float);
  d.n_pix_tiles = (int)((d.M + BPIX - 1) / BPIX);
  d.n_ch_tiles = 1;
  d.n_tiles = d.n_pix_tiles;
  make_fastdiv(d.Wq, d.fd_m[0], d.fd_s[0]);
  make_fastdiv(d.Hq, d.fd_m[1], d.fd_s[1]);
  make_fastdiv(d.Dq, d.fd_m[2], d.fd_s[2]);
  if (int rc = ensure_dynamic_lds(reinterpret_cast<const void*>(conv_igemm_ws64_kernel<false, T>), 160 * 1024)) return rc;
  if (int rc = ensure_dynamic_lds(reinterpret_cast<const void*>(conv_igemm_ws64_kernel<true, T>), 160 * 1024)) return rc;
  int n_cu = 0;
  if (int rc = persistent_grid_cus(&n_cu)) return rc;
  const int grid = d.n_tiles < n_cu ? d.n_tiles : n_cu;
  prof_begin_launch(s, 15, d.algo_flops, d.algo_bytes);
  if (rh) hipLaunchKernelGGL((conv_igemm_ws64_kernel<true, T>), dim3((unsigned)grid), dim3(768), LDS, s, d);
  else hipLaunchKernelGGL((conv_igemm_ws64_kernel<false, T>), dim3((unsigned)grid), dim3(768), LDS, s, d);
  prof_end_launch(s);
  RGBM_CHECK_HIP(hipGetLastError());
  return 0;
}

template <typename T, bool UNI>
static int launch_v3(ConvDesc d, hipStream_t s) {
  constexpr int BCH = 128, BPIX = 256;
  constexpr size_t LDS = 3 * (BCH + BPIX) * 8 * sizeof(uint4);
  d.n_pix_tiles = (int)((d.M + BPIX - 1) / BPIX);
  d.n_ch_tiles = (d.Cout + BCH - 1) / BCH;
  const long long nblk = (long long)d.n_pix_tiles * d.n_ch_tiles;
  RGBM_REQUIRE(nblk > 0 && nblk < (1ll << 31), "conv grid out of range");
  if (int rc = ensure_dynamic_lds(reinterpret_cast<const void*>(conv_igemm_v3_kernel<T, UNI>), (int)LDS)) return rc;
  prof_begin_launch(s, prof_row_ws<T>(), d.algo_flops, d.algo_bytes);
  hipLaunchKernelGGL((conv_igemm_v3_kernel<T, UNI>), dim3((unsigned)nblk), dim3(512), LDS, s, d);
  prof_end_launch(s);
  RGBM_CHECK_HIP(hipGetLastError());
  return 0;
}

template <typename T, int BCH, int BPIX, bool UNI>
static int launch_one_g(ConvDesc d, hipStream_t s) {
  d.n_pix_tiles = (int)((d.M + BPIX - 1) / BPIX);
  d.n_ch_tiles = (d.Cout + BCH - 1) / BCH;
  const long long nblk = (long long)d.n_pix_tiles * d.n_ch_tiles;
  RGBM_REQUIRE(nblk > 0 && nblk < (1ll << 31), "conv grid out of range");
  prof_begin_launch(s, prof_row_generic<T>(BCH), d.algo_flops, d.algo_bytes);
  hipLaunchKernelGGL((conv_igemm_glds_kernel<T, BCH, BPIX, UNI>), dim3((unsigned)nblk), dim3(256), 0, s, d);
  prof_end_launch(s);
  RGBM_CHECK_HIP(hipGetLastError());
  return 0;
}

int conv_tuning(int n_cu, ConvTuning* t) {
  *t = ConvTuning{g_debug_flags, g_gemm_kernel, g_ws_min_rows, n_cu};
  return n_cu > 0 ? 0 : persistent_grid_cus(&t->n_cu);
}

template <typename T>
static int launch_plan(const ConvDesc& d, const ConvPlan& p, hipStream_t s) {
  constexpr bool M32 = sizeof(T) == 2 || std::is_same<T, bx3_t>::value;
  switch (p.kernel) {
    case CONV_GENERIC: {
      auto tile = [&](auto uni) {
        constexpr bool UNI = decltype(uni)::value;
        switch (p.bch) {
          case 16: return launch_one_g<T, 16, 256, UNI>(d, s);
          case 32: return launch_one_g<T, 32, 256, UNI>(d, s);
          case 64: return launch_one_g<T, 64, 256, UNI>(d, s);
          default: return launch_one_g<T, 128, 128, UNI>(d, s);
        }
      };
      return p.uniform_taps ? tile(IC<true>{}) : tile(IC<false>{});
    }
    case CONV_M32_SMALL:
      if constexpr (M32) return launch_m32_small<T>(d, p, s);
      break;
    case CONV_WS_SLIM: return launch_ws<T, false, false, true>(d, p, s);
    case CONV_M32:
      if constexpr (M32) return launch_m32<T>(d, p, s);
      break;
    case CONV_WS_WIDE: return launch_ws<T, true, false>(d, p, s);
    case CONV_WS: return launch_ws<T, false, false>(d, p, s);
    case CONV_V3: return p.uniform_taps ? launch_v3<T, true>(d, s) : launch_v3<T, false>(d, s);
    case CONV_WS64:
    case CONV_WS64_ROWHALO:
      if constexpr (sizeof(T) == 2) return launch_ws64<T>(d, p.kernel == CONV_WS64_ROWHALO, s);
      break;
  }
  RGBM_REQUIRE(false, "conv plan names a kernel this storage type does not have");
}

int launch_conv(const ConvDesc& d, int dtype, hipStream_t s) {
  ConvTuning t;
  ConvPlan p;
  if (int rc = conv_tuning(0, &t)) return rc;
  if (int rc = plan_conv(d, dtype, t, &p)) return rc;
  return dtype == BF16 ? launch_plan<unsigned short>(d, p, s) : dtype == F16 ? launch_plan<f16_t>(d, p, s)
         : dtype == BF16X3 ? launch_plan<bx3_t>(d, p, s) : launch_plan<float>(d, p, s);
}

bool conv_ws64_eligible(const ConvDesc& d, int dtype) {
  ConvTuning t;
  ConvPlan p;
  return !conv_tuning(0, &t) && !plan_conv(d, dtype, t, &p) && (p.kernel == CONV_WS64 || p.kernel == CONV_WS64_ROWHALO);
}

}
```

### rgbmanip_amd/csrc/conv_igemm_m32.inc

```
#ifndef M32_SHIFT
#define M32_SHIFT 1
#endif
#ifndef M32_RACE_PROBE
#define M32_RACE_PROBE 0
#endif
typedef __attribute__((ext_vector_type(16))) float f32x16;

template <typename T> struct Mma32;
template <> struct Mma32<unsigned short> {
  __device__ static __forceinline__ void run(const uint4& a, const uint4& b, f32x16& c) {
    c = __builtin_amdgcn_mfma_f32_32x32x16_bf16(__builtin_bit_cast(bf16x8, a), __builtin_bit_cast(bf16x8, b), c, 0, 0, 0);
  }
};
template <> struct Mma32<f16_t> {
  __device__ static __forceinline__ void run(const uint4& a, const uint4& b, f32x16& c) {
    c = __builtin_amdgcn_mfma_f32_32x32x16_f16(__builtin_bit_cast(f16x8, a), __builtin_bit_cast(f16x8, b), c, 0, 0, 0);
  }
};

template <> struct Mma32<bx3_t> {
  __device__ static __forceinline__ void run(const uint4&, const uint4&, f32x16&) {}
};

__device__ __forceinline__ int m32_row_channel(int i) { return ((i >> 2) & 1) * 16 + (i & 3) + 4 * (i >> 3); }

template <typename T, int BPIX, int BCH = 256>
__global__ __launch_bounds__(BPIX == 256 ? 768 : 512) void conv_igemm_m32_kernel(const ConvDesc d) {
  constexpr bool BIG = BPIX == 256;
  constexpr bool STAGED = BIG && BCH == 256;
  constexpr bool X3 = std::is_same<T, bx3_t>::value;
  constexpr int NMW = BIG ? 8 : 4;
  constexpr int NTH = (NMW + 4) * 64;
  constexpr int NST = BIG ? 2 : 3;
  static_assert(BCH == 256 || BCH == 128 || BCH == 64, "channel tiles of 256 / 128 / 64");
  constexpr int E = 16 / sizeof(T);
  constexpr int BK = 8 * E;
  constexpr int XR = BPIX / 32;
  constexpr int WL = BCH / 32;
  constexpr int NP = XR + WL;
  constexpr int FA = BCH / 64, FB = 2;
  constexpr int WCHW = FA * 32;
  constexpr int STAGE = (BCH + BPIX) * 8;
  extern __shared__ __attribute__((aligned(16))) uint4 lds3[];

  const int tid = threadIdx.x;
  const int lane = tid & 63;
  const int wave = __builtin_amdgcn_readfirstlane(tid >> 6);
  constexpr bool KSPLIT = !BIG && BCH <= 128;
  int KT = d.KT, kt0 = 0, part = 0, nsp = 1, vtile = -1;
  if constexpr (KSPLIT) {
    if (d.ksplit > 1) {
      nsp = d.ksplit;
      part = (int)blockIdx.x % nsp;
      vtile = (int)blockIdx.x / nsp;
      kt0 = (int)((long long)part * d.KT / nsp);
      KT = (int)((long long)(part + 1) * d.KT / nsp) - kt0;
    }
  }
  const bool res_in_acc = d.ident != nullptr && d.res_mode == RES_PRE_ACT;
  const int KR = (res_in_acc && part == nsp - 1) ? BCH / BK : 0;
  const int KTT = KT + KR;
  const int n_my = vtile >= 0 ? 1 : ((int)d.n_tiles - (int)blockIdx.x + (int)gridDim.x - 1) / (int)gridDim.x;
  const int total = n_my * KTT;
  auto tile_of = [&](int k, int& pix_tile, int& ch_tile) {
    const int v = vtile >= 0 ? vtile : (int)blockIdx.x + k * (int)gridDim.x;
    const int nblk = d.n_tiles, bq = nblk >> 3, br = nblk & 7, xcd = v & 7, bidx = v >> 3;
    const int lid = (xcd < br ? xcd * (bq + 1) : br * (bq + 1) + (xcd - br) * bq) + bidx;
    pix_tile = lid / d.n_ch_tiles;
    ch_tile = lid - pix_tile * d.n_ch_tiles;
  };

  float* lbias = reinterpret_cast<float*>(lds3 + NST * STAGE);
  const bool bias_lds = d.bias != nullptr && d.bias_stride == 0 && d.Cout <= 2560;
  if (bias_lds)
    for (int i = tid; i < d.Cout; i += NTH) lbias[i] = d.bias[i];
  __syncthreads();

  if (wave >= NMW) {
    const int pw = wave - NMW;
    const int tp = tid - NMW * 64;
    const int j = tp & 7;
    const int r0 = tp >> 3;
    const int js = j ^ ((r0 >> 1) & 7);
    unsigned rmask[XR], xoff[XR], woff[WL], roff[XR];
    int tkd = 0, tkh = 0, tkw = 0, tc = 0;
    unsigned wko = 0;
    const unsigned lds0 = __builtin_amdgcn_readfirstlane(lds_addr(lds3 + pw * 64));
    const long long xbias = ((long long)(d.pd * d.Hi + d.ph) * d.Wi + d.pw) * d.Cin * (long long)sizeof(T);
    const __amdgpu_buffer_rsrc_t rsrc_x = __builtin_amdgcn_make_buffer_rsrc(
        const_cast<char*>(reinterpret_cast<const char*>(d.in)) - xbias, 0,
        (int)(unsigned)((long long)d.N * d.Di * d.Hi * d.Wi * d.Cin * (long long)sizeof(T) + xbias), 0x00020000);
    const __amdgpu_buffer_rsrc_t rsrc_w = __builtin_amdgcn_make_buffer_rsrc(
        const_cast<char*>(reinterpret_cast<const char*>(d.wgt)), 0, (int)(unsigned)((long long)d.n_ch_tiles * BCH * d.Kpad * (long long)sizeof(T)), 0x00020000);

    const __amdgpu_buffer_rsrc_t rsrc_r = __builtin_amdgcn_make_buffer_rsrc(
        const_cast<char*>(reinterpret_cast<const char*>(d.res)), 0, (int)(unsigned)(d.M * d.ldo * (long long)sizeof(T)), 0x00020000);
    const __amdgpu_buffer_rsrc_t rsrc_i = __builtin_amdgcn_make_buffer_rsrc(
        const_cast<char*>(reinterpret_cast<const char*>(d.ident)), 0, (int)(unsigned)(256 * 256 * sizeof(T)), 0x00020000);
    long long mybase = 0;
    unsigned mymask = 0;
    int my_ch_tile = 0, my_pix_tile = 0;
    auto prepare_tile = [&](int k) {
      int pix_tile, ch_tile;
      tile_of(k, pix_tile, ch_tile);
      my_ch_tile = ch_tile;
      my_pix_tile = pix_tile;
      mybase = 0;
      mymask = 0;
      if (j < XR) {
        const long long m = d.m0 + (long long)pix_tile * BPIX + r0 + 32 * j;
        int xn = 0, xd0 = -(1 << 20), xh0 = 0, xw0 = 0;
        if (m < d.M) {
          unsigned n, qd, qh, qw;
          decode_row(d, (unsigned)m, n, qd, qh, qw);
          xn = (int)n * d.Di;
          xd0 = (int)qd * d.sd - d.pd;
          xh0 = (int)qh * d.sh - d.ph;
          xw0 = (int)qw * d.sw - d.pw;
        }
        for (int kk = 0; kk < d.KD; ++kk) mymask |= (unsigned)((unsigned)(xd0 + kk * d.dild) < (unsigned)d.Di) << kk;
        for (int kk = 0; kk < d.KH; ++kk) mymask |= (unsigned)((unsigned)(xh0 + kk * d.dilh) < (unsigned)d.Hi) << (8 + kk);
        for (int kk = 0; kk < d.KW; ++kk) mymask |= (unsigned)((unsigned)(xw0 + kk * d.dilw) < (unsigned)d.Wi) << (16 + kk);
        const long long pix0 = ((long long)(xn + xd0) * d.Hi + xh0) * d.Wi + xw0;
        mybase = pix0 * d.Cin * (long long)sizeof(T);
      }
    };
    auto enter_tile = [&]() {
      const int grp = (tp & 63) & 56;
#pragma unroll
      for (int i = 0; i < XR; ++i) {
        const long long b = __shfl(mybase, grp | i, 64);
        rmask[i] = (unsigned)__shfl((int)mymask, grp | i, 64);
        xoff[i] = (unsigned)(b + xbias + (long long)(js * E) * (long long)sizeof(T));
        if (KR) {
          const long long m = d.m0 + (long long)my_pix_tile * BPIX + r0 + 32 * i;
          roff[i] = m < d.M ? (unsigned)((m * d.ldo + my_ch_tile * BCH + js * E) * (long long)sizeof(T)) : 0xffffffffu;
        }
      }
#pragma unroll
      for (int i = 0; i < WL; ++i) {
        const int row = r0 + 32 * i;
        woff[i] = (unsigned)(((long long)(my_ch_tile * BCH + row) * d.Kpad + js * E) * (long long)sizeof(T));
      }
      tkd = tkh = tkw = tc = 0;
      wko = 0;
      if (kt0 > 0) {
        if (d.korder && d.lcin >= 0) {
          const int tap = kt0 % d.ntaps, cb = kt0 / d.ntaps;
          tkw = tap % d.KW; tkh = (tap / d.KW) % d.KH; tkd = tap / (d.KW * d.KH);
          tc = cb * BK;
          wko = (unsigned)(((long long)tap * d.Cin + tc) * (long long)sizeof(T));
        } else {
          wko = (unsigned)kt0 * (unsigned)(BK * sizeof(T));
          if (d.lcin >= 0) {
            const int cpt = d.Cin / BK, tap = kt0 / cpt;
            tc = (kt0 - tap * cpt) * BK;
            tkw = tap % d.KW; tkh = (tap / d.KW) % d.KH; tkd = tap / (d.KW * d.KH);
          } else {
            tc = kt0 * BK;
          }
        }
      }
    };

    int ikt = 0, itile = 0;
    auto issue = [&](int stage) {
      if (ikt == 0) enter_tile();
      const unsigned sbase = lds0 + (unsigned)stage * (STAGE * 16);
      const unsigned sel = (1u << tkd) | (256u << tkh) | (65536u << tkw);
      const unsigned soff = (unsigned)(((long long)((tkd * d.dild * d.Hi + tkh * d.dilh) * d.Wi + tkw * d.dilw) * d.Cin + tc) * (long long)sizeof(T));
      const bool cok = tkd < d.KD && tc + js * E < d.Cin;
      if (ikt >= KT) {
        const unsigned ro = (unsigned)(ikt - KT) * (unsigned)(BK * sizeof(T));
#pragma unroll
        for (int i = 0; i < XR; ++i) blds16(roff[i], rsrc_r, ro, sbase + (BCH * 8 + i * 256) * 16);
        if (!BIG) {
#pragma unroll
          for (int i = 0; i < WL; ++i) blds16((unsigned)(((r0 + 32 * i) * 256 + js * E) * (int)sizeof(T)), rsrc_i, ro, sbase + (i * 256) * 16);
        }
      } else {
#pragma unroll
        for (int i = 0; i < XR; ++i) {
          const bool ok = cok && (rmask[i] & sel) == sel;
          blds16(ok ? xoff[i] : 0xffffffffu, rsrc_x, soff, sbase + (BCH * 8 + i * 256) * 16);
        }
#pragma unroll
        for (int i = 0; i < WL; ++i) blds16(woff[i], rsrc_w, wko, sbase + (i * 256) * 16);
      }
      if (ikt >= KT) {
      } else if (d.korder && d.lcin >= 0) {
        wko += (unsigned)d.Cin * (unsigned)sizeof(T);
        if (++tkw == d.KW) { tkw = 0; if (++tkh == d.KH) { tkh = 0; if (++tkd == d.KD) { tkd = 0; tc += BK; wko = (unsigned)tc * (unsigned)sizeof(T); } } }
      } else {
        wko += BK * (unsigned)sizeof(T);
        tc += BK;
        if (d.lcin >= 0 && tc >= d.Cin) {
          tc = 0;
          if (++tkw == d.KW) { tkw = 0; if (++tkh == d.KH) { tkh = 0; ++tkd; } }
        }
      }
      if (++ikt == KTT) { ikt = 0; ++itile; if (itile < n_my) prepare_tile(itile); }
    };

    if (total > 0) prepare_tile(0);
    if (total > 0) issue(0);
    if (NST == 3 && total > 1) issue(1);
    int st = 0, gk = 0;
    for (int g = 0; g < total; ++g) {
      if (NST == 2 || g + 1 >= total) asm volatile("s_waitcnt vmcnt(0)" ::: "memory");
      else asm volatile("s_waitcnt vmcnt(%0)" :: "n"(NP) : "memory");
      RGBM_BARRIER();
      if (NST == 3) { if (g + 2 < total) issue(st == 0 ? 2 : st - 1); }
      else { if (g + 1 < total) issue(st ^ 1); }
      st = st == NST - 1 ? 0 : st + 1;
      if (STAGED) { if (++gk == KTT) { gk = 0; RGBM_BARRIER(); } }
    }
    return;
  }

  const int wch = BIG ? (wave >> 2) * WCHW : (wave >> 1) * WCHW;
  const int wpix = BIG ? (wave & 3) * 64 : (wave & 1) * 64;
  const int li = lane & 31, lh = lane >> 5;
  const int rowA = wch + m32_row_channel(li), rowB = wpix + li;
  const unsigned offA = (unsigned)(rowA * 8 + (lh ^ ((rowA >> 1) & 7))) * 16u;
  const unsigned offB = (unsigned)(BCH * 8 + rowB * 8 + (lh ^ ((rowB >> 1) & 7))) * 16u;
  const char* ldsc = reinterpret_cast<const char*>(lds3);
  f32x16 acc[FA][FB];
  auto ident_frag = [&](int sub) {
    int lq = lane;
    asm volatile("" : "+v"(lq));
    const int qi = lq & 31, qh = lq >> 5;
    const int id_s = (qi >> 2) & 1, id_c = (qi & 3) + 4 * (qi >> 3);
    const int lh = qh;
    const unsigned one = std::is_same<T, f16_t>::value ? 0x3c00u : 0x3f80u;
    const bool mine = sub == id_s && lh == (id_c >> 3);
    const unsigned w = mine ? one << (16 * (id_c & 1)) : 0u;
    const int q = (id_c & 7) >> 1;
    return make_uint4(q == 0 ? w : 0u, q == 1 ? w : 0u, q == 2 ? w : 0u, q == 3 ? w : 0u);
  };
  auto load_step = [&](int st, int s, uint4 (&af)[FA], uint4 (&bf)[FB]) {
    const char* base = ldsc + st * (STAGE * 16);
    const unsigned oa = offA ^ ((unsigned)s << 5), ob = offB ^ ((unsigned)s << 5);
#pragma unroll
    for (int b = 0; b < FB; ++b) bf[b] = *reinterpret_cast<const uint4*>(base + ob + b * 4096);
#pragma unroll
    for (int a = 0; a < FA; ++a) af[a] = *reinterpret_cast<const uint4*>(base + oa + a * 4096);
  };
  auto mma_step = [&](const uint4 (&af)[FA], const uint4 (&bf)[FB]) {
#pragma unroll
    for (int a = 0; a < FA; ++a)
#pragma unroll
      for (int b = 0; b < FB; ++b) {
        Mma32<T>::run(af[a], bf[b], acc[a][b]);
      }
  };
  T* __restrict__ out = reinterpret_cast<T*>(d.out);
  const T* __restrict__ res = reinterpret_cast<const T*>(d.res);
  auto tile_interior = [&](int pix_tile, int ch_tile) {
    return (d.bias == nullptr || bias_lds) && d.m0 + (long long)(pix_tile + 1) * BPIX <= d.M && (ch_tile + 1) * BCH <= d.Cout && d.act != ACT_TANH;
  };
  int st = 0;
  for (int k = 0; k < n_my; ++k) {
    {
      int pt, ct;
      tile_of(k, pt, ct);
      if (tile_interior(pt, ct) && d.bias && part == 0) {
        const float* bp = lbias + ct * BCH + wch + lh * 16;
#pragma unroll
        for (int a = 0; a < FA; ++a) {
          f32x16 b16;
#pragma unroll
          for (int q = 0; q < 4; ++q) {
            const f32x4 b4 = *reinterpret_cast<const f32x4*>(bp + a * 32 + q * 4);
            b16[q * 4 + 0] = b4[0]; b16[q * 4 + 1] = b4[1]; b16[q * 4 + 2] = b4[2]; b16[q * 4 + 3] = b4[3];
          }
#pragma unroll
          for (int b = 0; b < FB; ++b) acc[a][b] = b16;
        }
      } else {
#pragma unroll
        for (int a = 0; a < FA; ++a)
#pragma unroll
          for (int b = 0; b < FB; ++b)
#pragma unroll
            for (int e = 0; e < 16; ++e) acc[a][b][e] = 0.f;
      }
    }
    if constexpr (X3) {
      const int zA = (rowA >> 1) & 7, zB = (rowB >> 1) & 7;
      unsigned oA3 = (unsigned)(rowA * 128) + (unsigned)(((2 * lh) ^ zA) << 4);
      unsigned oB3 = (unsigned)(BCH * 128 + rowB * 128) + (unsigned)(((2 * lh) ^ zB) << 4);
      const char* sb = ldsc;
      auto rdp = [&](unsigned off, uint4& hi, uint4& lo) {
        const uint4 c0 = *reinterpret_cast<const uint4*>(sb + off), c1 = *reinterpret_cast<const uint4*>(sb + (off ^ 16u));
        hi = make_uint4(c0.x, c0.y, c1.x, c1.y);
        lo = make_uint4(c0.z, c0.w, c1.z, c1.w);
      };
      const int KTM = BIG ? KT : KTT;
      for (int kt = 0; kt < KTM; ++kt) {
        asm volatile("s_waitcnt lgkmcnt(0)" ::: "memory");
        RGBM_BARRIER();
        asm volatile("" : "+v"(oA3), "+v"(oB3));
        sb = ldsc + st * (STAGE * 16);
#pragma unroll
        for (int s = 0; s < 2; ++s) {
          uint4 Bh[FB], Bl[FB], Al, Ah, Aln, Ahn;
          const unsigned ob = oB3 ^ ((unsigned)s << 6), oa = oA3 ^ ((unsigned)s << 6);
#pragma unroll
          for (int b = 0; b < FB; ++b) rdp(ob + b * 4096, Bh[b], Bl[b]);
          rdp(oa, Ah, Al);
          __builtin_amdgcn_sched_barrier(0);
#pragma unroll
          for (int a = 0; a < FA; ++a) {
            if (a + 1 < FA) rdp(oa + (a + 1) * 4096, Ahn, Aln);
            __builtin_amdgcn_sched_barrier(0);
#pragma unroll
            for (int b = 0; b < FB; ++b) Mma32<unsigned short>::run(Al, Bh[b], acc[a][b]);
#pragma unroll
            for (int b = 0; b < FB; ++b) Mma32<unsigned short>::run(Ah, Bl[b], acc[a][b]);
#pragma unroll
            for (int b = 0; b < FB; ++b) Mma32<unsigned short>::run(Ah, Bh[b], acc[a][b]);
            __builtin_amdgcn_sched_barrier(0);
            if (a + 1 < FA) { Al = Aln; Ah = Ahn; }
          }
        }
        st = st == NST - 1 ? 0 : st + 1;
      }
      if constexpr (BIG) {
        if (KR) {
#pragma unroll
          for (int r = 0; r < BCH / BK; ++r) {
            asm volatile("s_waitcnt lgkmcnt(0)" ::: "memory");
            RGBM_BARRIER();
            if (wch == ((32 * r) / WCHW) * WCHW) {
              asm volatile("" : "+v"(oB3));
              sb = ldsc + st * (STAGE * 16);
#pragma unroll
              for (int s2 = 0; s2 < 2; ++s2) {
                uint4 Bh[FB], Bl[FB];
                const unsigned ob = oB3 ^ ((unsigned)s2 << 6);
#pragma unroll
                for (int b = 0; b < FB; ++b) rdp(ob + b * 4096, Bh[b], Bl[b]);
                const uint4 Aid = ident_frag(s2);
#pragma unroll
                for (int b = 0; b < FB; ++b) Mma32<unsigned short>::run(Aid, Bl[b], acc[((32 * r) % WCHW) / 32][b]);
#pragma unroll
                for (int b = 0; b < FB; ++b) Mma32<unsigned short>::run(Aid, Bh[b], acc[((32 * r) % WCHW) / 32][b]);
              }
            }
            st ^= 1;
          }
        }
      }
    } else if constexpr (BIG) {
      uint4 A[FA], B[FB], Bn[FB];
      unsigned oA = offA, oB = offB;
      auto ldA = [&](int s, int a) { A[a] = *reinterpret_cast<const uint4*>(ldsc + st * (STAGE * 16) + (oA ^ ((unsigned)s << 5)) + a * 4096); };
      auto ldB = [&](int s, uint4 (&bf)[FB]) {
#pragma unroll
        for (int b = 0; b < FB; ++b) bf[b] = *reinterpret_cast<const uint4*>(ldsc + st * (STAGE * 16) + (oB ^ ((unsigned)s << 5)) + b * 4096);
      };
      auto ldAs = [&](int stg, int s, int a) { A[a] = *reinterpret_cast<const uint4*>(ldsc + stg * (STAGE * 16) + (oA ^ ((unsigned)s << 5)) + a * 4096); };
      auto ldBs = [&](int stg, int s, uint4 (&bf)[FB]) {
#pragma unroll
        for (int b = 0; b < FB; ++b) bf[b] = *reinterpret_cast<const uint4*>(ldsc + stg * (STAGE * 16) + (oB ^ ((unsigned)s << 5)) + b * 4096);
      };
      auto first3 = [&]() {
#pragma unroll
        for (int s = 0; s < 3; ++s) {
          ldBs(st, s + 1, Bn);
          __builtin_amdgcn_sched_barrier(0);
#pragma unroll
          for (int a = 0; a < FA; ++a) {
            Mma32<T>::run(A[a], B[0], acc[a][0]);
            Mma32<T>::run(A[a], B[1], acc[a][1]);
            __builtin_amdgcn_sched_barrier(0);
            ldAs(st, s + 1, a);
            __builtin_amdgcn_sched_barrier(0);
          }
          B[0] = Bn[0]; B[1] = Bn[1];
        }
      };
      asm volatile("s_waitcnt lgkmcnt(0)" ::: "memory");
      RGBM_BARRIER();
      asm volatile("" : "+v"(oA), "+v"(oB));
      ldBs(st, 0, B);
#pragma unroll
      for (int a = 0; a < FA; ++a) ldAs(st, 0, a);
      __builtin_amdgcn_sched_barrier(0);
      for (int kt = 0; kt + 1 < KT; ++kt) {
        first3();
        if (M32_SHIFT) {
          asm volatile("s_waitcnt lgkmcnt(0)" ::: "memory");
          RGBM_BARRIER();
          asm volatile("" : "+v"(oA), "+v"(oB));
          ldBs(st ^ 1, 0, Bn);
          __builtin_amdgcn_sched_barrier(0);
#pragma unroll
          for (int a = 0; a < FA; ++a) {
            Mma32<T>::run(A[a], B[0], acc[a][0]);
            Mma32<T>::run(A[a], B[1], acc[a][1]);
            __builtin_amdgcn_sched_barrier(0);
            ldAs(st ^ 1, 0, a);
            __builtin_amdgcn_sched_barrier(0);
          }
          B[0] = Bn[0]; B[1] = Bn[1];
        } else {
#pragma unroll
          for (int a = 0; a < FA; ++a) {
            Mma32<T>::run(A[a], B[0], acc[a][0]);
            Mma32<T>::run(A[a], B[1], acc[a][1]);
            __builtin_amdgcn_sched_barrier(0);
          }
          asm volatile("s_waitcnt lgkmcnt(0)" ::: "memory");
          RGBM_BARRIER();
          asm volatile("" : "+v"(oA), "+v"(oB));
          ldBs(st ^ 1, 0, B);
#pragma unroll
          for (int a = 0; a < FA; ++a) ldAs(st ^ 1, 0, a);
          __builtin_amdgcn_sched_barrier(0);
        }
        st ^= 1;
      }
      first3();
#if M32_RACE_PROBE
      if (wave == 5 && !KR) { for (int q = 0; q < 32; ++q) __builtin_amdgcn_s_sleep(2); }
#endif
#pragma unroll
      for (int a = 0; a < FA; ++a) {
        Mma32<T>::run(A[a], B[0], acc[a][0]);
        Mma32<T>::run(A[a], B[1], acc[a][1]);
        __builtin_amdgcn_sched_barrier(0);
      }
      st ^= 1;
      if (KR) {
#pragma unroll
        for (int r = 0; r < BCH / BK; ++r) {
          asm volatile("s_waitcnt lgkmcnt(0)" ::: "memory");
          RGBM_BARRIER();
#if M32_RACE_PROBE
          if (wave == 5 && r == BCH / BK - 1) { for (int q = 0; q < 32; ++q) __builtin_amdgcn_s_sleep(2); }
#endif
          asm volatile("" : "+v"(oB));
#pragma unroll
          for (int s = 0; s < 4; ++s) {
            if (wch == ((64 * r + 16 * s) / WCHW) * WCHW) {
              ldB(s, B);
              const uint4 Aid = ident_frag(s & 1);
              Mma32<T>::run(Aid, B[0], acc[((64 * r + 16 * s) % WCHW) / 32][0]);
              Mma32<T>::run(Aid, B[1], acc[((64 * r + 16 * s) % WCHW) / 32][1]);
            }
          }
          st ^= 1;
        }
      }
    } else {
      uint4 A0[FA], B0[FB], A1[FA], B1[FB];
      for (int kt = 0; kt < KTT; ++kt) {
        asm volatile("s_waitcnt lgkmcnt(0)" ::: "memory");
        RGBM_BARRIER();
        load_step(st, 0, A0, B0);
        __builtin_amdgcn_sched_barrier(0);
        if (kt > 0) mma_step(A1, B1);
        __builtin_amdgcn_sched_barrier(0);
        load_step(st, 1, A1, B1);
        __builtin_amdgcn_sched_barrier(0);
        mma_step(A0, B0);
        __builtin_amdgcn_sched_barrier(0);
        load_step(st, 2, A0, B0);
        __builtin_amdgcn_sched_barrier(0);
        mma_step(A1, B1);
        __builtin_amdgcn_sched_barrier(0);
        load_step(st, 3, A1, B1);
        __builtin_amdgcn_sched_barrier(0);
        mma_step(A0, B0);
        __builtin_amdgcn_sched_barrier(0);
        st = st == 2 ? 0 : st + 1;
      }
      mma_step(A1, B1);
    }

    if constexpr (STAGED) {
      asm volatile("s_waitcnt lgkmcnt(0)" ::: "memory");
      RGBM_BARRIER();
    }
    if constexpr (KSPLIT) {
      if (nsp > 1) {
        constexpr int WFL = FA * FB * 64 * 16;
        float* sc = d.kscratch + (((long long)vtile * nsp + part) * NMW + wave) * WFL;
#pragma unroll
        for (int a = 0; a < FA; ++a)
#pragma unroll
          for (int b = 0; b < FB; ++b)
#pragma unroll
            for (int q = 0; q < 4; ++q)
            {
              const f32x4 v = f32x4{acc[a][b][4 * q], acc[a][b][4 * q + 1], acc[a][b][4 * q + 2], acc[a][b][4 * q + 3]};
              asm volatile("global_store_dwordx4 %0, %1, off sc1" :: "v"(sc + (((a * FB + b) * 4 + q) * 64 + lane) * 4), "v"(v) : "memory");
            }
        asm volatile("s_waitcnt vmcnt(0)" ::: "memory");
        unsigned arrived = 0;
        if (lane == 0) arrived = __hip_atomic_fetch_add(d.kcount + (long long)vtile * NMW + wave, 1u, __ATOMIC_RELAXED, __HIP_MEMORY_SCOPE_AGENT);
        arrived = (unsigned)__builtin_amdgcn_readfirstlane((int)arrived);
        if (arrived != (unsigned)(nsp - 1)) continue;
#pragma unroll
        for (int a = 0; a < FA; ++a)
#pragma unroll
          for (int b = 0; b < FB; ++b)
#pragma unroll
            for (int e = 0; e < 16; ++e) acc[a][b][e] = 0.f;
        for (int p = 0; p < nsp; ++p) {
          const float* sp = d.kscratch + (((long long)vtile * nsp + p) * NMW + wave) * WFL;
          f32x4 t[FA * FB * 4];
#pragma unroll
          for (int i = 0; i < FA * FB * 4; ++i)
            asm volatile("global_load_dwordx4 %0, %1, off sc1" : "=v"(t[i]) : "v"(sp + (i * 64 + lane) * 4) : "memory");
          asm volatile("s_waitcnt vmcnt(0)" ::: "memory");
#pragma unroll
          for (int i = 0; i < FA * FB * 4; ++i) asm volatile("" : "+v"(t[i]));
#pragma unroll
          for (int a = 0; a < FA; ++a)
#pragma unroll
            for (int b = 0; b < FB; ++b)
#pragma unroll
              for (int q = 0; q < 4; ++q)
#pragma unroll
                for (int e = 0; e < 4; ++e) acc[a][b][4 * q + e] += t[(a * FB + b) * 4 + q][e];
        }
        if (lane == 0) __hip_atomic_store(d.kcount + (long long)vtile * NMW + wave, 0u, __ATOMIC_RELAXED, __HIP_MEMORY_SCOPE_AGENT);
      }
    }
    int pix_tile, ch_tile;
    tile_of(k, pix_tile, ch_tile);
    const bool interior = tile_interior(pix_tile, ch_tile);
    long long obase[FB];
    int nn[FB];
    bool pok[FB];
    const bool dense_out = d.osd == 1 && d.osh == 1 && d.osw == 1 && d.opd == 0 && d.oph == 0 && d.opw == 0 && d.Dq == d.Do &&
                           d.Hq == d.Ho && d.Wq == d.Wo;
#pragma unroll
    for (int b = 0; b < FB; ++b) {
      const long long m = d.m0 + (long long)pix_tile * BPIX + wpix + b * 32 + li;
      pok[b] = m < d.M;
      if (dense_out && (interior || d.bias_stride == 0)) {
        nn[b] = 0;
        obase[b] = (pok[b] ? m : 0ll) * d.ldo;
        continue;
      }
      unsigned n, qd, qh, qw;
      decode_row(d, pok[b] ? (unsigned)m : 0u, n, qd, qh, qw);
      nn[b] = (int)n;
      obase[b] = ((((long long)n * d.Do + (qd * d.osd + d.opd)) * d.Ho + (qh * d.osh + d.oph)) * d.Wo + (qw * d.osw + d.opw)) * d.ldo;
    }
    constexpr int CHK = 16 / (int)sizeof(T);
    constexpr int NQ = 16 / CHK;
    if (interior) {
      const float nslope = d.act == ACT_RELU ? 0.f : d.act == ACT_PRELU ? d.slope : 1.f;
      auto fast = [&](auto resc) {
        constexpr int RES = decltype(resc)::value;
        constexpr int NF = FA * FB;
        constexpr int AR = FA < (X3 ? 2 : 4) ? FA : (X3 ? 2 : 4);
        static_assert(FA % AR == 0, "whole store rounds");
        uint4 pk[AR][NQ];
        uint4 rr[4][NQ];
        const long long mrow = d.m0 + (long long)pix_tile * BPIX + wpix;
        const int ch0 = ch_tile * BCH + wch;
        unsigned lofs_c = (unsigned)((li * d.ldo + lh * 16) * (int)sizeof(T));
        asm volatile("" : "+v"(lofs_c));
        auto rd = [&](int i) {
          const int b = i / FA, a = i % FA;
          const char* ub = reinterpret_cast<const char*>(res + (mrow + b * 32) * d.ldo + ch0 + a * 32);
#pragma unroll
          for (int q = 0; q < NQ; ++q) rr[i & 3][q] = *reinterpret_cast<const uint4*>(ub + lofs_c + q * 16);
        };
        auto make = [&](int i) {
          const int b = i / FA, a = i % FA;
#pragma unroll
          for (int q = 0; q < NQ; ++q) {
            float v[CHK], rv[CHK];
#pragma unroll
            for (int e = 0; e < CHK; ++e) v[e] = acc[a][b][q * CHK + e];
            if (RES != RES_NONE) unpack_chunk(rr[i & 3][q], rv, T());
            if (RES == RES_PRE_ACT) {
#pragma unroll
              for (int e = 0; e < CHK; ++e) v[e] += rv[e];
            }
#pragma unroll
            for (int e = 0; e < CHK; ++e) v[e] = v[e] < 0.f ? __builtin_fmaxf(v[e], -3.402823466e38f) * nslope : v[e];
            if (RES == RES_POST_ACT) {
#pragma unroll
              for (int e = 0; e < CHK; ++e) v[e] += rv[e];
            }
            pk[a % AR][q] = pack_chunk(v, T());
          }
        };
        auto store_round = [&](int b, int ar) {
          if constexpr (STAGED) {
            char* stg = const_cast<char*>(ldsc) + (st ^ 1) * (STAGE * 16) + wave * 8192;
            unsigned wofs = (unsigned)(li * 256 + (((lh * NQ) ^ (li & 15)) << 4));
            unsigned rofs = (unsigned)((lane >> 4) * 256 + (((lane & 15) ^ (lane >> 4)) << 4));
            unsigned gofs = (unsigned)(((lane >> 4) * d.ldo + (lane & 15) * CHK) * (int)sizeof(T));
            asm volatile("" : "+v"(wofs), "+v"(rofs), "+v"(gofs));
#pragma unroll
            for (int a = 0; a < AR; ++a)
#pragma unroll
              for (int q = 0; q < NQ; ++q)
                *reinterpret_cast<uint4*>(stg + (wofs ^ (unsigned)((a * 2 * NQ + q) << 4))) = pk[a][q];
            char* ob = reinterpret_cast<char*>(out + (mrow + b * 32) * d.ldo + ch0 + ar * AR * 32);
#pragma unroll
            for (int t = 0; t < 8; ++t) {
              const uint4 v = *reinterpret_cast<const uint4*>(stg + t * 1024 + (rofs ^ (unsigned)(((4 * t) & 15) << 4)));
              *reinterpret_cast<uint4*>(ob + (long long)(4 * t) * d.ldo * (long long)sizeof(T) + gofs) = v;
            }
          } else {
#pragma unroll
            for (int a = 0; a < AR; ++a)
#pragma unroll
              for (int q = 0; q < NQ; ++q)
                *reinterpret_cast<uint4*>(reinterpret_cast<char*>(out + (mrow + b * 32) * d.ldo + ch0 + (ar * AR + a) * 32) + lofs_c + q * 16) = pk[a][q];
          }
        };
        if (RES != RES_NONE) { rd(0); rd(1); __builtin_amdgcn_sched_barrier(0); }
#pragma unroll
        for (int i = 0; i < NF; ++i) {
          make(i);
          __builtin_amdgcn_sched_barrier(0);
          if (RES != RES_NONE) {
            if (i < FA - 1) rd(i + 2);
            else if (i == FA - 1) {
#pragma unroll
              for (int k = FA + 1; k < NF; ++k) rd(k);
            }
            __builtin_amdgcn_sched_barrier(0);
          }
          if (i % AR == AR - 1) { store_round(i / FA, (i % FA) / AR); __builtin_amdgcn_sched_barrier(0); }
        }
      };
      if (BIG || res_in_acc) fast(IC<RES_NONE>{});
      else if (d.res_mode == RES_NONE) fast(IC<RES_NONE>{});
      else if (d.res_mode == RES_PRE_ACT) fast(IC<RES_PRE_ACT>{});
      else fast(IC<RES_POST_ACT>{});
      continue;
    }
    if constexpr (BIG) continue;
#pragma unroll
    for (int a = 0; a < FA; ++a) {
      const int chL = ch_tile * BCH + wch + a * 32 + lh * 16;
#pragma unroll
      for (int b = 0; b < FB; ++b) {
#pragma unroll
        for (int q = 0; q < NQ; ++q) {
          const int c = chL + q * CHK;
          if (!pok[b] || c >= d.Cout) continue;
          const bool whole = c + CHK <= d.Cout;
          float v[CHK], rv[CHK];
#pragma unroll
          for (int e = 0; e < CHK; ++e) v[e] = acc[a][b][q * CHK + e];
          if (d.bias) {
            const float* bp = d.bias + (long long)nn[b] * d.bias_stride + c;
#pragma unroll
            for (int e = 0; e < CHK; ++e) if (e < 4 || whole) v[e] += bp[e];
          }
#pragma unroll
          for (int e = 0; e < CHK; ++e) rv[e] = 0.f;
          if (d.res_mode != RES_NONE && !res_in_acc) {
            if (whole) unpack_chunk(*reinterpret_cast<const uint4*>(res + obase[b] + c), rv, T());
            else load4(res + obase[b] + c, rv);
          }
          if (d.res_mode == RES_PRE_ACT && !res_in_acc) {
#pragma unroll
            for (int e = 0; e < CHK; ++e) v[e] += rv[e];
          }
#pragma unroll
          for (int e = 0; e < CHK; ++e) v[e] = apply_act_g(v[e], d.act, d.slope);
          if (d.res_mode == RES_POST_ACT) {
#pragma unroll
            for (int e = 0; e < CHK; ++e) v[e] += rv[e];
          }
          if (whole) *reinterpret_cast<uint4*>(out + obase[b] + c) = pack_chunk(v, T());
          else store4(out + obase[b] + c, v);
        }
      }
    }
  }
}

template <typename T, int BPIX, int BCH = 256>
static int launch_m32_range(ConvDesc d, hipStream_t s) {
  constexpr int NST = BPIX == 256 ? 2 : 3;
  constexpr size_t LDS = ((size_t)NST * (BCH + BPIX) * 8) * sizeof(uint4) + 2560 * sizeof(float);
  d.n_pix_tiles = (int)((d.M - d.m0 + BPIX - 1) / BPIX);
  d.n_ch_tiles = (d.Cout + BCH - 1) / BCH;
  const long long ntiles = (long long)d.n_pix_tiles * d.n_ch_tiles;
  RGBM_REQUIRE(ntiles > 0 && ntiles < (1ll << 31) && d.M < (1ll << 31), "conv grid out of range");
  d.n_tiles = (int)ntiles;
  make_fastdiv(d.Wq, d.fd_m[0], d.fd_s[0]);
  make_fastdiv(d.Hq, d.fd_m[1], d.fd_s[1]);
  make_fastdiv(d.Dq, d.fd_m[2], d.fd_s[2]);
  if (int rc = ensure_dynamic_lds(reinterpret_cast<const void*>(conv_igemm_m32_kernel<T, BPIX, BCH>), (int)LDS)) return rc;
  int n_cu = 0;
  if (int rc = persistent_grid_cus(&n_cu)) return rc;
  RGBM_REQUIRE(d.ksplit <= 1 || (BPIX == 128 && BCH <= 128 && ntiles * d.ksplit <= 4096 && d.kscratch && d.kcount), "K split: 64 / 128-channel x 128-pixel tiles, one workgroup per (tile, part)");
  const int grid = d.ksplit > 1 ? (int)(ntiles * d.ksplit) : ntiles < n_cu ? (int)ntiles : n_cu;
  prof_begin_launch(s, BPIX == 256 && BCH == 256 ? (std::is_same<T, bx3_t>::value ? 33 : 31) : (std::is_same<T, bx3_t>::value ? 41 : 40), d.algo_flops, d.algo_bytes);
  hipLaunchKernelGGL((conv_igemm_m32_kernel<T, BPIX, BCH>), dim3((unsigned)grid), dim3(BPIX == 256 ? 768 : 512), LDS, s, d);
  prof_end_launch(s);
  RGBM_CHECK_HIP(hipGetLastError());
  return 0;
}

template <typename T>
static int m32_identity(const void** out) {
  static std::mutex mu;
  static std::map<int, void*> per_dev;
  int dev = 0;
  RGBM_CHECK_HIP(hipGetDevice(&dev));
  std::lock_guard<std::mutex> lock(mu);
  void*& p = per_dev[dev];
  if (!p) {
    if (std::is_same<T, bx3_t>::value) {
      std::vector<unsigned short> h(256 * 256 * 2, 0);
      for (int i = 0; i < 256; ++i) h[(i * 256 + (i & ~3)) * 2 + (i & 3)] = 0x3f80;
      RGBM_CHECK_HIP(hipMalloc(&p, h.size() * 2));
      RGBM_CHECK_HIP(hipMemcpy(p, h.data(), h.size() * 2, hipMemcpyHostToDevice));
    } else {
      std::vector<unsigned short> h(256 * 256, 0);
      const unsigned short one = std::is_same<T, f16_t>::value ? 0x3c00 : 0x3f80;
      for (int i = 0; i < 256; ++i) h[i * 256 + i] = one;
      RGBM_CHECK_HIP(hipMalloc(&p, h.size() * 2));
      RGBM_CHECK_HIP(hipMemcpy(p, h.data(), h.size() * 2, hipMemcpyHostToDevice));
    }
  }
  *out = p;
  return 0;
}

static int m32_ksplit_buffers(hipStream_t s, float** scratch, unsigned** count) {
  static std::mutex mu;
  static std::map<std::pair<int, hipStream_t>, std::pair<float*, unsigned*>> per_stream;
  int dev = 0;
  RGBM_CHECK_HIP(hipGetDevice(&dev));
  std::lock_guard<std::mutex> lock(mu);
  auto& e = per_stream[std::make_pair(dev, s)];
  if (!e.first) {
    hipStreamCaptureStatus cs = hipStreamCaptureStatusNone;
    if (hipStreamIsCapturing(s, &cs) == hipSuccess && cs != hipStreamCaptureStatusNone) { *scratch = nullptr; *count = nullptr; return 0; }
    float* sc = nullptr; unsigned* cn = nullptr;
    RGBM_CHECK_HIP(hipMalloc(&sc, kM32SplitFloats * sizeof(float)));
    RGBM_CHECK_HIP(hipMalloc(&cn, kM32SplitCounters * sizeof(unsigned)));
    RGBM_CHECK_HIP(hipMemsetAsync(cn, 0, kM32SplitCounters * sizeof(unsigned), s));
    e.first = sc; e.second = cn;
  }
  *scratch = e.first; *count = e.second;
  return 0;
}

template <typename T>
static int m32_setup(ConvDesc& d, const ConvPlan& p, hipStream_t s) {
  d.m0 = 0;
  d.ident = nullptr;
  d.korder = p.korder;
  d.ksplit = 1; d.kscratch = nullptr; d.kcount = nullptr;
  if (p.ksplit > 1) {
    if (int rc = m32_ksplit_buffers(s, &d.kscratch, &d.kcount)) return rc;
    if (d.kscratch) d.ksplit = p.ksplit;
  }
  return p.identity_residual ? m32_identity<T>(&d.ident) : 0;
}

template <typename T>
static int launch_m32_tiles128(const ConvDesc& d, int bch, hipStream_t s) {
  return bch == 64 ? launch_m32_range<T, 128, 64>(d, s) : bch == 128 ? launch_m32_range<T, 128, 128>(d, s) : launch_m32_range<T, 128, 256>(d, s);
}

template <typename T>
static int launch_m32_small(ConvDesc d, const ConvPlan& p, hipStream_t s) {
  if (int rc = m32_setup<T>(d, p, s)) return rc;
  return launch_m32_tiles128<T>(d, p.bch, s);
}

template <typename T>
static int launch_m32(ConvDesc d, const ConvPlan& p, hipStream_t s) {
  if (int rc = m32_setup<T>(d, p, s)) return rc;
  if (p.main_rows > 0) {
    ConvDesc m = d;
    m.M = p.main_rows;
    const double frac = (double)m.M / (double)d.M;
    m.algo_flops = d.algo_flops * frac; m.algo_bytes = d.algo_bytes * frac;
    if (int rc = launch_m32_range<T, 256, 256>(m, s)) return rc;
    d.m0 = m.M;
    d.algo_flops *= 1.0 - frac; d.algo_bytes *= 1.0 - frac;
  }
  return p.tail_bch ? launch_m32_tiles128<T>(d, p.tail_bch, s) : 0;
}
```

### rgbmanip_amd/csrc/conv_plan.cpp

```cpp
#include "conv_plan.h"

#include "kernels.h"

namespace rgbm {

#ifndef M32_KSPLIT_MAX
#define M32_KSPLIT_MAX 4
#endif
#ifndef M32_KSPLIT_MINSTEPS
#define M32_KSPLIT_MINSTEPS 8
#endif

namespace {

bool uniform_taps(const ConvDesc& d, int bk) {
  if (d.KD > 8 || d.KH > 8 || d.KW > 8) return false;
  if (d.lcin < 0) return d.ntaps == 1;
  return d.Cin % bk == 0;
}

bool buffer_offsets_ok(const ConvDesc& d, int bch, long long esz) {
  const long long xbytes = ((long long)d.N * d.Di * d.Hi * d.Wi + (long long)(d.pd * d.Hi + d.ph) * d.Wi + d.pw) * d.Cin * esz;
  const long long wbytes = (long long)((d.Cout + bch - 1) / bch) * bch * d.Kpad * esz;
  return xbytes < (1ll << 32) - 65536 && wbytes < (1ll << 32) - 65536 && d.pd >= 0 && d.ph >= 0 && d.pw >= 0;
}

bool rowhalo_ok(const ConvDesc& d) {
  return d.KD == 1 && d.KH == 3 && d.KW == 3 && d.sd == 1 && d.sh == 1 && d.sw == 1 && d.Dq == 1 && d.Di == 1 &&
         d.dilh == d.dilw && d.dilw >= 1 && d.dilw <= 4 && d.ph == d.dilh && d.pw == d.dilw && d.pd == 0 &&
         d.lcin >= 6 && d.Hq == d.Hi && d.Wq == d.Wi && d.Wi > 2 * d.dilw && d.osh == 1 && d.osw == 1;
}

int m32_small_choice(const ConvDesc& d, int n_cu, bool slim_ok) {
  const long long p128 = (d.M + 127) / 128, p256 = (d.M + 255) / 256;
  auto cost = [&](long long tiles, int kb) { return (double)((tiles + n_cu - 1) / n_cu) * (double)(kb + 8); };
  double best = slim_ok ? cost(p256 * (d.Cout / 64), 40) : 1e30;
  int pick = 0;
  const int bch[3] = {64, 128, 256}, kb[3] = {24, 32, 48};
  for (int i = 0; i < 3; ++i) {
    if (d.Cout % bch[i]) continue;
    const double c = cost(p128 * (d.Cout / bch[i]), kb[i]);
    if (c < best * 0.999) { best = c; pick = bch[i]; }
  }
  return pick;
}

int m32_ksplit_choice(const ConvDesc& d, int flags, long long tiles, int n_cu, int bch, int n_waves) {
  if ((flags & DBG_NO_KSPLIT) || tiles <= 0 || bch > 128) return 1;
  int n = (int)(n_cu / tiles);
  if (n > M32_KSPLIT_MAX) n = M32_KSPLIT_MAX;
  while (n > 1 && d.KT / n < M32_KSPLIT_MINSTEPS) --n;
  if (n < 2) return 1;
  if ((size_t)tiles * n * bch * 128 > kM32SplitFloats || (size_t)tiles * n_waves > kM32SplitCounters) return 1;
  return n;
}

}

int plan_conv(const ConvDesc& d, int dtype, const ConvTuning& t, ConvPlan* out) {
  RGBM_REQUIRE(d.M > 0 && d.M < (1ll << 31), "conv M out of range");
  RGBM_REQUIRE(d.Cout % 4 == 0 && d.ldo % 4 == 0, "conv Cout/ldo must be multiples of 4");
  RGBM_REQUIRE(d.KT > 0 && d.Kpad == d.KT * conv_bk(dtype), "conv K padding mismatch");
  RGBM_REQUIRE(d.Cin % dtype_chunk(dtype) == 0, "conv Cin must be a multiple of the 16-byte chunk");
  if (d.lcin >= 0) {
    RGBM_REQUIRE((1 << d.lcin) == d.Cin, "conv lcin mismatch");
  } else {
    RGBM_REQUIRE(d.ntaps == 1, "linear-K mode needs a single tap");
  }
  const int f = t.flags, n_cu = t.n_cu;
  const long long esz = (long long)dtype_size(dtype);
  const bool bits16 = esz == 2, mfma32 = dtype != F32;
  const int ch_tile = conv_ch_tile(d.Cout);
  const bool uni = uniform_taps(d, conv_bk(dtype)) && !(f & DBG_NONUNIFORM_TAPS);
  const bool out16 = (((unsigned long long)d.out | (unsigned long long)(d.ldo * esz)) & 15ull) == 0ull;
  const bool rows16 = out16 && ((unsigned long long)d.res & 15ull) == 0ull;
  const bool dense_out = d.osd == 1 && d.osh == 1 && d.osw == 1 && d.opd == 0 && d.oph == 0 && d.opw == 0 && d.Dq == d.Do && d.Hq == d.Ho && d.Wq == d.Wo;
  const bool ident_ok = dense_out && d.res_mode == RES_PRE_ACT && d.res != nullptr && d.M * d.ldo * esz < (1ll << 32) - 65536;
  const bool ws_rows = d.M >= (t.ws_min_rows > 0 ? t.ws_min_rows : 1024);

  ConvPlan p = {};
  p.uniform_taps = uni;
  p.ksplit = 1;
  p.korder = (f & DBG_KORDER_TAPS_OUTER) ? 0 : 1;
  auto pick = [&](int kernel, int bch, int bpix) {
    p.kernel = kernel; p.bch = bch; p.bpix = bpix;
    p.buf_ok = buffer_offsets_ok(d, bch, esz) && !(f & DBG_GLOBAL_ADDR);
    *out = p;
    return 0;
  };
  auto generic = [&]() { return pick(CONV_GENERIC, ch_tile, ch_tile == 128 ? 128 : 256); };
  auto small = [&](int bch) {
    p.ksplit = m32_ksplit_choice(d, f, ((d.M + 127) / 128) * ((d.Cout + bch - 1) / bch), n_cu, bch, 4);
    p.identity_residual = ident_ok && d.Cout % 256 == 0;
    return pick(CONV_M32_SMALL, bch, 128);
  };

  if (d.out_f32) {
    RGBM_REQUIRE(dtype == BF16X3 && d.w2 == nullptr, "out_f32 is a bf16x3 option of the generic kernel");
    return generic();
  }
  if (ch_tile == 128 && !(f & DBG_NO_WS) && ws_rows) {
    if (!uni || (f & DBG_V3_FOR_WS) || !rows16) return pick(CONV_V3, 128, 256);
    if (!(f & DBG_NO_SLIM_SMALL) && d.Cout % 64 == 0) {
      const long long slim_tiles = ((d.M + 255) / 256) * (d.Cout / 64);
      if (mfma32) {
        if (d.Cout % 256 == 0 && ((d.M + 255) / 256) * (d.Cout / 256) < n_cu && t.gemm_kernel >= 1 && !(f & (DBG_M32_TAILS_R5 | DBG_WS_128x256)) &&
            buffer_offsets_ok(d, 256, esz)) {
          const int bch = t.gemm_kernel == 1 ? 256 : m32_small_choice(d, n_cu, slim_tiles <= n_cu);
          if (bch) return small(bch);
        }
        if (d.Cout == 128 && ((d.M + 127) / 128) * 2 * 2 <= n_cu && t.gemm_kernel == 2 &&
            !(f & (DBG_M32_TAILS_R5 | DBG_WS_128x256 | DBG_NO_KSPLIT | DBG_L2_SLIM_TILE)) && d.w2 == nullptr && buffer_offsets_ok(d, 64, esz))
          return small(64);
      }
      if (slim_tiles <= n_cu) return pick(CONV_WS_SLIM, 64, 256);
    }
    if (d.Cout % 256 == 0 && !(f & DBG_WS_128x256)) {
      if (!(mfma32 && buffer_offsets_ok(d, 256, esz) && t.gemm_kernel >= 1)) return pick(CONV_WS_WIDE, 256, 128);
      const bool big_ok = dense_out && (d.bias == nullptr || (d.bias_stride == 0 && d.Cout <= 2560)) && d.act != ACT_TANH &&
                          (d.res_mode == RES_NONE || (d.res_mode == RES_PRE_ACT && d.res != nullptr)) && d.M * d.ldo * esz < (1ll << 32) - 65536;
      const long long P = d.M / 256, n_ch = d.Cout / 256, tiles = P * n_ch;
      long long Pm = 0;
      if (t.gemm_kernel != 1 && big_ok && tiles >= n_cu) {
        const long long rem = tiles % n_cu;
        Pm = (rem == 0 || rem * 10 >= (long long)n_cu * 6) ? P : (tiles - rem) / n_ch;
      }
      p.main_rows = Pm * 256;
      p.identity_residual = ident_ok;
      p.tail_bch = p.main_rows == d.M ? 0 : 256;
      const long long pt = (d.M - p.main_rows + 127) / 128;
      if (p.tail_bch && t.gemm_kernel != 1 && !(f & DBG_M32_TAILS_R5)) {
        if (pt * (d.Cout / 64) <= n_cu) p.tail_bch = 64;
        else if (pt * (d.Cout / 128) <= n_cu) p.tail_bch = 128;
      }
      return pick(CONV_M32, 256, 256);
    }
    return pick(CONV_WS, 128, 256);
  }
  if (bits16 && uni && !(f & DBG_NO_WS64) && ch_tile == 64 && d.res_mode == RES_NONE && d.KT >= 2 && ws_rows &&
      (d.w2 ? d.Cout == 64 && d.kpad2 == 64 && (d.cout2 == 16 || d.cout2 == 32) && d.ldo2 % 4 == 0 : out16))
    return rowhalo_ok(d) && !(f & DBG_NO_ROWHALO) ? pick(CONV_WS64_ROWHALO, 64, 256) : pick(CONV_WS64, 64, 256);
  RGBM_REQUIRE(d.w2 == nullptr, "a fused 1x1 needs the ws64 kernel (check conv_ws64_eligible first)");
  if (ch_tile == 64 && uni && ws_rows && !(f & (DBG_NO_WS | DBG_V3_FOR_WS | DBG_NO_SLIM64)) && rows16) return pick(CONV_WS_SLIM, 64, 256);
  return generic();
}

}
```

### rgbmanip_amd/csrc/conv_plan.h

```cpp
#pragma once
#include "common.h"

namespace rgbm {

struct ConvTuning {
  int flags;
  int gemm_kernel;
  long long ws_min_rows;
  int n_cu;
};

enum ConvKernel {
  CONV_GENERIC = 0,
  CONV_V3 = 1,
  CONV_WS = 2,
  CONV_WS_WIDE = 3,
  CONV_WS_SLIM = 4,
  CONV_WS64 = 5,
  CONV_WS64_ROWHALO = 6,
  CONV_M32 = 7,
  CONV_M32_SMALL = 8,
};

struct ConvPlan {
  int kernel;
  int bch, bpix;
  bool uniform_taps;
  long long main_rows;
  int tail_bch;
  int ksplit;
  bool identity_residual;
  int korder, buf_ok;
};

constexpr size_t kM32SplitFloats = 8u << 20, kM32SplitCounters = 16384;

int plan_conv(const ConvDesc& d, int dtype, const ConvTuning& t, ConvPlan* out);
int conv_tuning(int n_cu, ConvTuning* t);

}
```

### rgbmanip_amd/csrc/kernels.h

```cpp
#pragma once
#include <vector>

#include "common.h"

namespace rgbm {

int launch_nchw_to_nhwc_pad(int dtype, const float* in, void* out, int V, int C, int H, int W, int Cp, hipStream_t s);
int launch_maxpool3x3s2(int dtype, const void* in, void* out, int V, int H, int W, int C, hipStream_t s);
int launch_resize_bilinear_ac(int dtype, const void* in, void* out, int V, int Hs, int Ws, int C, int Ho, int Wo, int ldo,
                              int ch_off, hipStream_t s);
int launch_copy_channels(int dtype, const void* in, void* out, long long npix, int C, int ldo, int ch_off, hipStream_t s);
int launch_adaptive_avgpool(int dtype, const void* in, void* out, int V, int H, int W, int C, int S, hipStream_t s);
int launch_adaptive_avgpool_multi(int dtype, const void* in, void* const* outs, const int* bins, int nb, int V, int H, int W, int C,
                                  hipStream_t s);
int launch_psp_pool_conv(int dtype, const void* in, int ldi, const void* const* w, void* const* outs, const int* bins, int V, int H, int W,
                         int act, float slope, hipStream_t s);
int launch_psp_resize_cat(int dtype, const void* f, const void* const* stages, const int* bins, void* out, int V, int Ho, int Wo, hipStream_t s);
int launch_homography(const float* P_views, float* out, int V, int B, hipStream_t s);
int launch_build_volume(int dtype, const void* feat, const float* homog, const float* depths, void* vol, int v0, int Vc, int V,
                        int B, int D, int H, int W, hipStream_t s);

int launch_upconv_combine(int dtype, const void* z, const float* bias, void* out, int V, int h, int w, int Co, int ldo, int act,
                          float slope, hipStream_t s, const float* drop = nullptr);
int launch_upconv_final(int dtype, const void* x, const void* wz, const float* bias, float slope, const void* wf, const float* biasf,
                        void* out, int out_f32, int V, int h, int w, hipStream_t s, const void* wf_f16 = nullptr);

constexpr int kDropoutPerView = 256 + 64;
unsigned dropout_threshold(float p);
float dropout_scale(float p);
int launch_dropout_masks(float* masks, unsigned long long* state, int B, float p, unsigned long long seed, int advance, hipStream_t s);

size_t bn_scratch_bytes(int V);
int launch_bn_per_sample(int dtype, void* y, const void* res, const float* gamma, const float* beta, void* scratch, int V,
                         long long nvox, int C, int relu, hipStream_t s);

int launch_to_f32(int dtype, const void* in, float* out, long long n, hipStream_t s);

int launch_gather_points(int dtype, const void* feat, const int* choose, float* out, int V, int P, int HW, int C, hipStream_t s);
int launch_prob_softmax_depth(int dtype, const void* u11, const float* wprob, const int* choose, const float* depths,
                              float* prob, float* depth_out, int v0, int Vc, int B, int P, int D, int H, int W, int classmajor,
                              hipStream_t s);
int launch_fuse_points(int dtype, const void* feat, const float* homog, const float* depths, const int* choose,
                       const float* prob, float* out, int V, int B, int P, int D, int H, int W, int ldo, int ch_off,
                       hipStream_t s, int Vn = -1);
int launch_mean_points(int dtype, const void* in, float* out, float* scratch, int V, int P, int C, hipStream_t s);
int launch_f32_to_f16(const float* in, void* out, long long n, hipStream_t s);
void stem_pack(const float* w, std::vector<float>& packed);
int launch_stem(int dtype, const float* img1, const float* img2, const void* wpk, void* out, int B, int V, int S, hipStream_t s);
int launch_stem_views(int dtype, const float* img, const void* wpk, void* out, int V, int S, hipStream_t s);
int launch_feature_store(const void* src, void* pool, const int* slots, int V, int pool_records, size_t part_off, size_t part_bytes,
                         size_t record_bytes, hipStream_t s);
int launch_feature_gather(const void* pool, void* dst, const int* slot1, const int* slot2, int B, int pool_records, size_t part_off,
                          size_t part_bytes, size_t record_bytes, hipStream_t s);
int launch_feature_bad_slot_nan(const int* slot1, const int* slot2, int B, int pool_records, float* const out[10], const int per_pose[10],
                                hipStream_t s);
int launch_crop_fingerprint(const float* img, int V, int n_words, unsigned long long* keys_out, hipStream_t s);
int launch_f32_to_bx3(const float* in, void* out, long long n, hipStream_t s);
int launch_view_linear(const float* x, const float* W, const float* bias, float* out, int V, int I, int O, int ldw, int i0,
                       int relu, hipStream_t s);
struct PointMlpDesc {
  const float* table;
  const void* feat;
  const int* choose;
  float* nocs4;
  float* pf;
  int ldpf, P, HW;
  long long N;
};
int point_mlp_table_floats();
void point_mlp_pack(const float* const w[6], const float* const b[6], float* table);
int launch_point_mlp(int feat_dtype, const PointMlpDesc& d, hipStream_t s);
int launch_ortho6d(const float* r6, float* R, int V, hipStream_t s);
int launch_mean_points_partial(int dtype, const void* in, float* scratch, int V, int P, int C, hipStream_t s);
int launch_view_linear_mean(const float* partial, int P, float* mean_out, const float* W, const float* bias, float* out, int V, int I, int O,
                            int ldw, int i0, int relu, hipStream_t s);
int launch_pose_heads_mean(const float* partial, int P, float* mean_out, float* R, float* const w[3][3], float* const b[3][3],
                           float* const out[3], const int odim[3], int V, hipStream_t s);
constexpr int kMeanSplit = 8;
constexpr int kPoseMlpSlab = 128;
struct PoseMlpDesc {
  const float* pf96;
  const void* w[4];
  int ldw[4];
  const float* bias[4];
  const float* vbias;
  void* q128;
  float* part128;
  float* part256;
  int V, P;
};
bool pose_mlp_fits(int P);
int launch_pose_mlp1(const PoseMlpDesc& d, hipStream_t s);
int launch_pose_mlp2(const PoseMlpDesc& d, hipStream_t s);
int launch_pose_heads(const float* pf2, float* const w[3][3], float* const b[3][3], float* const out[3], const int odim[3], int V,
                      hipStream_t s);
int launch_stage_in(const float* P1, const float* P2, const int* c1, const int* c2, float* Pviews, int* choose, int B, int P, hipStream_t s);
int launch_stage_out(const float* nocs4, const float* depth, const float* R, const float* tv, const float* sv, float* const nocs[2],
                     float* const dep[2], float* const r[2], float* const t[2], float* const sz[2], int B, int P, int view2, hipStream_t s);
int launch_copy_cols(const float* in, float* out, long long rows, int ldi, int ldo, int n, hipStream_t s);

struct Conv3dTileDesc {
  const void* in; const void* wgt; void* out; const float* bias; const void* res;
  int N, Di, Hi, Wi;
  int Do, Ho, Wo;
  int Dq, Hq, Wq;
  int ntd, nth, ntw;
  int Cout, relu;
  const void* feat; const float* homog; const float* depths; int v0, V, B;
  int prof_variant; double algo_flops, algo_bytes;
  int out_classmajor;
  int feat_f16;
  const int* tile_list; const int* tile_count;
  int tile_mask_stride;
  const unsigned char* tile_mask;
};
enum DebugFlag {
  DBG_NO_WS = 8, DBG_NONUNIFORM_TAPS = 16, DBG_V3_FOR_WS = 64, DBG_NO_WS64 = 128, DBG_NO_ROWHALO = 256, DBG_GENERIC_RESIZE = 512,
  DBG_PSP_STAGE_R5 = 1024, DBG_POINT_MLP_R5 = 2048, DBG_TILE_CONV0 = 4096, DBG_NO_KSPLIT = 16384, DBG_L2_SLIM_TILE = 32768,
  DBG_WS_128x256 = 65536, DBG_NO_SLIM64 = 262144, DBG_KORDER_TAPS_OUTER = 1 << 20, DBG_SWEEP_ALT_BLEND = 1 << 21, DBG_SWEEP_DOT2 = 1 << 22,
  DBG_PP_ONE_KERNEL = 1 << 23, DBG_NO_SLIM_SMALL = 1 << 24, DBG_PP_GENERIC_SELECT = 1 << 25, DBG_PP_GUARD = 1 << 26, DBG_GLOBAL_ADDR = 1 << 27,
  DBG_SWEEP_PER_TILE = 1 << 28, DBG_SPARSE_TAIL_R5 = 1 << 29, DBG_M32_TAILS_R5 = 1 << 30, DBG_POSE_MLP_R6 = 1 << 19,
};
extern int g_debug_flags;
extern long long g_ws_min_rows;
extern int g_tuning_version;
extern int g_gemm_kernel;
void conv3d_tile_pack(const float* w, const float* scale, int Cin, int Cout, int coutp, bool transposed, int dtype,
                      std::vector<float>& packed);
int launch_conv3d_tile(int layer, int dtype, const Conv3dTileDesc& d, hipStream_t s);
int sparse_mask_bytes_per_view(int S);
int sparse_mask_offset(int S, int layer);
int launch_sparse_masks(const int* choose, int v0, int Vc, int P, int S, unsigned char* masks, int* sweep_list, int* sweep_count,
                        hipStream_t s);
int conv3d_tile_dims(int layer, int dtype, int* TD, int* TH, int* TW);

void conv0_sweep_pack(const float* w, const float* scale, std::vector<float>& packed);
int launch_conv0_sweep(const Conv3dTileDesc& d, int dtype, hipStream_t s);

int conv0_sweep_x3_upload(const std::vector<float>& packed, void** dev);
int launch_conv0_sweep_x3(const Conv3dTileDesc& d, hipStream_t s);
int launch_bx3_to_f32(const void* in, float* out, long long n, hipStream_t s);

int launch_prob_sparse(const void* u9, const void* c0, const void* w11_packed, const float* bias11, const float* wprob,
                       const int* choose, const float* depths, float* prob, float* depth_out, int v0, int Vc, int B, int P,
                       int D, int H, int W, int dtype, hipStream_t s, const void* w11_taps = nullptr);
void prob_sparse_pack(const float* w, const float* scale, std::vector<float>& packed);

int launch_prepare_inputs(const float* rgb, const unsigned char* mask, const double* K, const int* frame_map, int N, int H, int W, int S, int P,
                          unsigned seed, float* img, int* choose, float* pts2d, double* Kcrop, int* window, int* valid,
                          unsigned char* small_scratch, hipStream_t s, int frame0 = 0);
int launch_prepare_inputs_u8(const unsigned char* rgb, const unsigned char* mask, const double* K, const int* frame_map, int N, int H, int W,
                             int S, int P, unsigned seed, float* img, int* choose, float* pts2d, double* Kcrop, int* window, int* valid,
                             unsigned char* small_scratch, hipStream_t s, int frame0 = 0);
int launch_prepare_inputs_opt(const void* rgb, int pixel_type, int normalize, const unsigned char* mask, const double* K, const int* frame_map,
                              int N, int H, int W, int S, int P, unsigned seed, float* img, int* choose, float* pts2d, double* Kcrop,
                              int* window, int* valid, unsigned char* small_scratch, hipStream_t s, int frame0 = 0);
int launch_prepare_inputs_windows(const void* pix, int pixel_type, int normalize, const unsigned char* mask_pix, const long long* offset,
                                  const int* window, const int* valid_in, const double* K, int frame0, int N, int H, int W, int S, int P,
                                  unsigned seed, float* img, int* choose, float* pts2d, double* Kcrop, int* valid, unsigned char* small_scratch,
                                  hipStream_t s);
int launch_quantize_frames(const float* src, unsigned char* dst, size_t n, hipStream_t s);

int launch_umeyama_ransac(const float* nocs, const float* depth, const int* choose, const double* Kc, const double* E1,
                          double* bbox, double* srt, int* valid, int B, int P, int img, unsigned seed, hipStream_t s);

int launch_projection(const double* Kc, const double* E, float* P, int n, hipStream_t s);
int launch_pnp_ransac(const float* nocs1, const float* pts1, const float* nocs2, const float* pts2, const double* K, const double* E1,
                      const double* E2, double* bbox, double* srt, int* info, int* valid, int B, int P, unsigned seed, hipStream_t s);

int launch_mask_extent(const unsigned char* mask, int N, int H, int W, int* ext, int* count, hipStream_t s);

int launch_postprocess(const float* nocs, const float* depth, const float* rot, const int* choose, const double* Kc,
                       const double* E1, double* bbox, double* ts_out, int* valid, int B, int P, int img, hipStream_t s,
                       void* scratch = nullptr, size_t scratch_bytes = 0);
int launch_postprocess_regressed(const float* nocs, const float* rot, const float* tr, const float* sv, const double* E1, double* bbox,
                                 double* ts_out, int* valid, int B, int P, hipStream_t s);
int launch_microbench_mfma(float* scratch, int iters, int random_operands, double* flops, hipStream_t s);
int microbench_mfma_scratch_floats(int* n);
int launch_microbench_copy(const void* src, void* dst, size_t bytes, hipStream_t s);
size_t postprocess_scratch_bytes(int B);
int postprocess_slices(int B);

int launch_gae(int T, int N, const float* rewards, const unsigned char* dones, const float* values, const float* last_values,
               float gamma, float lam, float* returns, float* adv, double* sums, hipStream_t s);
int launch_adv_normalise(long long n_local, float* adv, const double* sums, double count_total, hipStream_t s);

struct PolicyLayout { int dims[5]; int log_std; int w[2][4]; int b[2][4]; int total; };
struct PolicyOptState { int t; int n_updates; float lr; float last_kl; float last_norm; float pad_; double sum_surr; double sum_vloss; };
int launch_policy_forward(const float* params, const PolicyLayout& L, int n, int mode, const float* obs, const float* noise,
                          float* actions, float* logp, float* value, float* mu, hipStream_t s);
int policy_partial_floats(const PolicyLayout& L, int n);
int launch_ppo_minibatch(const float* params, const PolicyLayout& L, int n, const float* obs, const float* actions,
                         const float* old_logp, const float* adv, const float* returns, const float* old_values,
                         const float* old_mu, const float* old_sigma, float clip, float vcoef, float ecoef, float* partial,
                         float* grads, hipStream_t s);
constexpr int POLICY_MAX_HIDDEN = 6, POLICY_MAX_WIDTH = 512, POLICY_MAX_ACT = 32;
enum { PACT_ELU = 0, PACT_SELU = 1, PACT_RELU = 2, PACT_LRELU = 3, PACT_TANH = 4, PACT_SIGMOID = 5 };
struct PolicyDesc {
  int obs_dim, state_dim, act_dim, activation, asymmetric;
  int n_hidden[2];
  int hidden[2][POLICY_MAX_HIDDEN];
  int w[2][POLICY_MAX_HIDDEN + 1];
  int b[2][POLICY_MAX_HIDDEN + 1];
  int log_std, total;
};
int launch_policy_forward_ex(const float* params, const PolicyDesc& D, int n, int mode, const float* obs, const float* states,
                             const float* noise, float* actions, float* logp, float* value, float* mu, hipStream_t s);
int ppo_scratch_floats_ex(const PolicyDesc& D, int n, int clipped_vloss, size_t* count);
int launch_ppo_minibatch_ex(const float* params, const PolicyDesc& D, int n, const float* obs, const float* states,
                            const float* actions, const float* old_logp, const float* adv, const float* returns,
                            const float* old_values, const float* old_mu, const float* old_sigma, float clip, float vcoef, float ecoef,
                            int clipped_vloss, float* scratch, float* grads, hipStream_t s);
int launch_ppo_adam(float* params, const float* grads, float* m, float* v, PolicyOptState* st, int total, float inv_world,
                    float max_norm, float desired_kl, float lr_min, float lr_max, int adaptive, hipStream_t s);

}
```

Baseline: 5958.

## Reorder conv output rows into border classes to skip padded taps in m32 GEMM

Adds a border-class row ordering for 3x3 same-padded 2-D convolutions in the m32 implicit-GEMM kernel. Output pixels are grouped into nine bands (interior, edges, corners), so each pixel tile only iterates over the taps that are in-bounds for its band, cutting k-steps that would otherwise load zero padding. Results are scattered back to natural row order through a per-tile LDS offset table. This costs more LDS, indirect stores, and extra decode arithmetic, and it turns off K-split for these layers. It is enabled by default through a new tuning key and exposed through a probe API.

```diff
diff --git a/include/rgbm.h b/include/rgbm.h
--- a/include/rgbm.h
+++ b/include/rgbm.h
@@ -191,6 +191,9 @@
 int rgbm_conv_plan(int dtype, int N, int D, int H, int W, int Cin, int Cin_pad, int Cout, int Cout_pad, int KD, int KH, int KW,
                    int stride_d, int stride_hw, int pad_d, int pad_hw, int dil_hw, int transposed, int has_bias, int res_mode, int act,
                    int cls, int n_cu, int32_t* plan);
+int rgbm_conv_row_probe(int dtype, int N, int D, int H, int W, int Cin, int Cin_pad, int Cout, int Cout_pad, int KD, int KH, int KW,
+                        int stride_d, int stride_hw, int pad_d, int pad_hw, int dil_hw, int transposed, int has_bias, int res_mode, int act,
+                        int cls, int n_cu, long long row0, int nrows, int32_t* row_order, int32_t* nyx, int32_t* tap_mask);
 int rgbm_bn_per_sample_scratch_bytes(int V, size_t* bytes);
 int rgbm_bn_per_sample(int dtype, void* y_dev, const void* res_dev, const float* gamma_dev, const float* beta_dev, void* scratch_dev,
                        int V, int64_t nvox, int C, int relu, void* stream);
diff --git a/rgbmanip_amd/_lib.py b/rgbmanip_amd/_lib.py
--- a/rgbmanip_amd/_lib.py
+++ b/rgbmanip_amd/_lib.py
@@ -132,6 +132,7 @@
     "rgbm_conv_nd": (_i, [_i, _vp, _i, _i, _i, _i, _i, _i, _vp, _i, _i, _i, _i, _i, _i, _i, _i, _i, _i, _i, _vp, _vp, _vp,
                           _vp, _i, _i, _f, _vp, _vp]),
     "rgbm_conv_plan": (_i, [_i] * 23 + [C.POINTER(C.c_int32)]),
+    "rgbm_conv_row_probe": (_i, [_i] * 23 + [C.c_longlong, _i] + [C.POINTER(C.c_int32)] * 3),
     "rgbm_bn_per_sample_scratch_bytes": (_i, [_i, C.POINTER(_sz)]),
     "rgbm_bn_per_sample": (_i, [_i, _vp, _vp, _vp, _vp, _vp, _i, _i64, _i, _i, _vp]),
     "rgbm_conv3d_tile": (_i, [_i, _i, _vp, _i, _i, _i, _i, _vp, _vp, _vp, _vp, _vp, _vp]),
diff --git a/rgbmanip_amd/csrc/capi.cpp b/rgbmanip_amd/csrc/capi.cpp
--- a/rgbmanip_amd/csrc/capi.cpp
+++ b/rgbmanip_amd/csrc/capi.cpp
@@ -9,6 +9,7 @@
 #include "adapose.h"
 #include "control.h"
 #include "conv_plan.h"
+#include "conv_row_order.h"
 #include "prof.h"
 
 using namespace rgbm;
@@ -379,14 +380,13 @@
   return rc;
 }
 
-int rgbm_conv_plan(int dtype, int N, int D, int H, int W, int Cin, int Cin_pad, int Cout, int Cout_pad, int KD, int KH, int KW,
-                   int stride_d, int stride_hw, int pad_d, int pad_hw, int dil_hw, int transposed, int has_bias, int res_mode, int act,
-                   int cls, int n_cu, int32_t* plan) {
-  RGBM_REQUIRE(plan && n_cu >= 0 && dtype >= F32 && dtype <= BF16X3 && N > 0 && D > 0 && H > 0 && W > 0, "conv_plan arguments");
+static int conv_plan_of(int dtype, int N, int D, int H, int W, int Cin, int Cin_pad, int Cout, int Cout_pad, int KD, int KH, int KW,
+                        int stride_d, int stride_hw, int pad_d, int pad_hw, int dil_hw, int transposed, int has_bias, int res_mode, int act,
+                        int cls, int n_cu, ConvDesc& d, ConvPlan& p) {
+  RGBM_REQUIRE(n_cu >= 0 && dtype >= F32 && dtype <= BF16X3 && N > 0 && D > 0 && H > 0 && W > 0, "conv_plan arguments");
   const ConvGeom g = conv_nd_geom(Cin, Cout, KD, KH, KW, stride_d, stride_hw, pad_d, pad_hw, dil_hw, transposed, act, 0.f);
   PackedConv pc;
   if (int rc = conv_pack_geom(g, dtype, Cin_pad, Cout_pad, cls, &pc)) return rc;
-  ConvDesc d;
   conv_desc_geom(d, g, pc, Cin_pad, Cout_pad, N, D, H, W, Cout_pad, cls);
   alignas(16) static const float buffer[4] = {};
   d.in = d.wgt = buffer; d.out = const_cast<float*>(buffer);
@@ -394,11 +394,47 @@
   d.res = res_mode != RES_NONE ? buffer : nullptr;
   d.res_mode = res_mode;
   ConvTuning t;
+  if (int rc = conv_tuning(n_cu, &t)) return rc;
+  return plan_conv(d, dtype, t, &p);
+}
+
+int rgbm_conv_plan(int dtype, int N, int D, int H, int W, int Cin, int Cin_pad, int Cout, int Cout_pad, int KD, int KH, int KW,
+                   int stride_d, int stride_hw, int pad_d, int pad_hw, int dil_hw, int transposed, int has_bias, int res_mode, int act,
+                   int cls, int n_cu, int32_t* plan) {
+  RGBM_REQUIRE(plan, "conv_plan arguments");
+  ConvDesc d;
   ConvPlan p;
-  if (int rc = conv_tuning(n_cu, &t)) return rc;
-  if (int rc = plan_conv(d, dtype, t, &p)) return rc;
+  if (int rc = conv_plan_of(dtype, N, D, H, W, Cin, Cin_pad, Cout, Cout_pad, KD, KH, KW, stride_d, stride_hw, pad_d, pad_hw, dil_hw, transposed,
+                            has_bias, res_mode, act, cls, n_cu, d, p)) return rc;
   const int32_t v[RGBM_CONV_PLAN_INTS] = {p.kernel, p.bch, p.bpix, p.ksplit, (int32_t)p.main_rows, p.tail_bch, p.identity_residual, (int32_t)d.M, d.KT};
   memcpy(plan, v, sizeof(v));
+  return 0;
+}
+
+int rgbm_conv_row_probe(int dtype, int N, int D, int H, int W, int Cin, int Cin_pad, int Cout, int Cout_pad, int KD, int KH, int KW,
+                        int stride_d, int stride_hw, int pad_d, int pad_hw, int dil_hw, int transposed, int has_bias, int res_mode, int act,
+                        int cls, int n_cu, long long row0, int nrows, int32_t* row_order, int32_t* nyx, int32_t* tap_mask) {
+  if (row_order) {
+    ConvDesc d;
+    ConvPlan p;
+    if (int rc = conv_plan_of(dtype, N, D, H, W, Cin, Cin_pad, Cout, Cout_pad, KD, KH, KW, stride_d, stride_hw, pad_d, pad_hw, dil_hw, transposed,
+                              has_bias, res_mode, act, cls, n_cu, d, p)) return rc;
+    *row_order = p.row_order;
+  }
+  if (nyx || tap_mask) {
+    RGBM_REQUIRE(N > 0 && D == 1 && dil_hw >= 1 && H >= 2 * dil_hw && W >= 2 * dil_hw && (long long)N * H * W < (1ll << 31),
+                 "conv_row_probe: the border-class order needs a 2-D map of at least 2 x dilation pixels per side");
+    RGBM_REQUIRE(row0 >= 0 && row0 < (1ll << 31) && nrows > 0, "conv_row_probe row range");
+    if (nyx) {
+      for (int i = 0; i < nrows; ++i) {
+        if (row0 + i >= (long long)N * H * W) { nyx[3 * i] = nyx[3 * i + 1] = nyx[3 * i + 2] = -1; continue; }
+        unsigned n, y, x;
+        rgbm::border_row_decode(N, H, W, dil_hw, dil_hw, (unsigned)(row0 + i), n, y, x);
+        nyx[3 * i] = (int32_t)n; nyx[3 * i + 1] = (int32_t)y; nyx[3 * i + 2] = (int32_t)x;
+      }
+    }
+    if (tap_mask) *tap_mask = (int32_t)rgbm::border_tap_mask(N, H, W, dil_hw, dil_hw, (unsigned)row0, (unsigned)nrows);
+  }
   return 0;
 }
 
@@ -686,6 +722,7 @@
   const std::string k = key;
   if (k == "ws_min_rows") { RGBM_REQUIRE(value >= 0, "ws_min_rows"); rgbm::g_ws_min_rows = value; }
   else if (k == "gemm_kernel") { RGBM_REQUIRE(value >= 0 && value <= 2, "gemm_kernel"); rgbm::g_gemm_kernel = (int)value; }
+  else if (k == "gemm_tap_skip") { RGBM_REQUIRE(value == 0 || value == 1, "gemm_tap_skip"); rgbm::g_gemm_tap_skip = (int)value; }
   else { set_error("unknown tuning key " + k); return -1; }
   ++rgbm::g_tuning_version;
   return 0;
diff --git a/rgbmanip_amd/csrc/common.h b/rgbmanip_amd/csrc/common.h
--- a/rgbmanip_amd/csrc/common.h
+++ b/rgbmanip_amd/csrc/common.h
@@ -213,6 +213,7 @@
   double algo_flops, algo_bytes;
   int out_f32;
   int ksplit; float* kscratch; unsigned* kcount;
+  int row_order;
 };
 
 int launch_conv(const ConvDesc& d, int dtype, hipStream_t s);
diff --git a/rgbmanip_amd/csrc/conv_igemm_glds.hip b/rgbmanip_amd/csrc/conv_igemm_glds.hip
--- a/rgbmanip_amd/csrc/conv_igemm_glds.hip
+++ b/rgbmanip_amd/csrc/conv_igemm_glds.hip
@@ -4,6 +4,7 @@
 #include <vector>
 #include "common.h"
 #include "conv_plan.h"
+#include "conv_row_order.h"
 #include "kernels.h"
 #include "prof.h"
 
@@ -14,6 +15,7 @@
 namespace rgbm {
 
 int g_gemm_kernel = 2;
+int g_gemm_tap_skip = 1;
 __device__ uint4 g_zero_page[4];
 
 typedef __attribute__((address_space(3))) void* lds_ptr_t;
@@ -1696,7 +1698,7 @@
 }
 
 int conv_tuning(int n_cu, ConvTuning* t) {
-  *t = ConvTuning{g_debug_flags, g_gemm_kernel, g_ws_min_rows, n_cu};
+  *t = ConvTuning{g_debug_flags, g_gemm_kernel, g_ws_min_rows, n_cu, g_gemm_tap_skip};
   return n_cu > 0 ? 0 : persistent_grid_cus(&t->n_cu);
 }
 
diff --git a/rgbmanip_amd/csrc/conv_igemm_m32.inc b/rgbmanip_amd/csrc/conv_igemm_m32.inc
--- a/rgbmanip_amd/csrc/conv_igemm_m32.inc
+++ b/rgbmanip_amd/csrc/conv_igemm_m32.inc
@@ -24,7 +24,7 @@
 
 __device__ __forceinline__ int m32_row_channel(int i) { return ((i >> 2) & 1) * 16 + (i & 3) + 4 * (i >> 3); }
 
-template <typename T, int BPIX, int BCH = 256>
+template <typename T, int BPIX, int BCH = 256, bool RO = false>
 __global__ __launch_bounds__(BPIX == 256 ? 768 : 512) void conv_igemm_m32_kernel(const ConvDesc d) {
   constexpr bool BIG = BPIX == 256;
   constexpr bool STAGED = BIG && BCH == 256;
@@ -46,7 +46,7 @@
   const int tid = threadIdx.x;
   const int lane = tid & 63;
   const int wave = __builtin_amdgcn_readfirstlane(tid >> 6);
-  constexpr bool KSPLIT = !BIG && BCH <= 128;
+  constexpr bool KSPLIT = !BIG && BCH <= 128 && !RO;
   int KT = d.KT, kt0 = 0, part = 0, nsp = 1, vtile = -1;
   if constexpr (KSPLIT) {
     if (d.ksplit > 1) {
@@ -59,9 +59,7 @@
   }
   const bool res_in_acc = d.ident != nullptr && d.res_mode == RES_PRE_ACT;
   const int KR = (res_in_acc && part == nsp - 1) ? BCH / BK : 0;
-  const int KTT = KT + KR;
   const int n_my = vtile >= 0 ? 1 : ((int)d.n_tiles - (int)blockIdx.x + (int)gridDim.x - 1) / (int)gridDim.x;
-  const int total = n_my * KTT;
   auto tile_of = [&](int k, int& pix_tile, int& ch_tile) {
     const int v = vtile >= 0 ? vtile : (int)blockIdx.x + k * (int)gridDim.x;
     const int nblk = d.n_tiles, bq = nblk >> 3, br = nblk & 7, xcd = v & 7, bidx = v >> 3;
@@ -69,8 +67,21 @@
     pix_tile = lid / d.n_ch_tiles;
     ch_tile = lid - pix_tile * d.n_ch_tiles;
   };
+  auto tile_taps = [&](int pix_tile) -> unsigned {
+    int vn = d.N, vh = d.Hq, vw = d.Wq;
+    asm volatile("" : "+s"(vn), "+s"(vh), "+s"(vw));
+    return border_tap_mask(vn, vh, vw, d.dilh, d.dilw, (unsigned)d.m0 + (unsigned)pix_tile * BPIX, BPIX);
+  };
+  auto taps_ksteps = [&](unsigned taps) -> int { return RO ? __builtin_popcount(taps) * (d.Cin / BK) : KT; };
+  auto tile_ksteps = [&](int k) -> int {
+    if (!RO) return KT;
+    int pt, ct;
+    tile_of(k, pt, ct);
+    return taps_ksteps(tile_taps(pt));
+  };
 
   float* lbias = reinterpret_cast<float*>(lds3 + NST * STAGE);
+  unsigned* ltab = reinterpret_cast<unsigned*>(lbias + 2560);
   const bool bias_lds = d.bias != nullptr && d.bias_stride == 0 && d.Cout <= 2560;
   if (bias_lds)
     for (int i = tid; i < d.Cout; i += NTH) lbias[i] = d.bias[i];
@@ -86,44 +97,66 @@
     int tkd = 0, tkh = 0, tkw = 0, tc = 0;
     unsigned wko = 0;
     const unsigned lds0 = __builtin_amdgcn_readfirstlane(lds_addr(lds3 + pw * 64));
-    const long long xbias = ((long long)(d.pd * d.Hi + d.ph) * d.Wi + d.pw) * d.Cin * (long long)sizeof(T);
+    const long long xbias = RO ? ((long long)d.dilh * d.Wq + d.dilw) * d.Cin * (long long)sizeof(T)
+                               : ((long long)(d.pd * d.Hi + d.ph) * d.Wi + d.pw) * d.Cin * (long long)sizeof(T);
     const __amdgpu_buffer_rsrc_t rsrc_x = __builtin_amdgcn_make_buffer_rsrc(
         const_cast<char*>(reinterpret_cast<const char*>(d.in)) - xbias, 0,
-        (int)(unsigned)((long long)d.N * d.Di * d.Hi * d.Wi * d.Cin * (long long)sizeof(T) + xbias), 0x00020000);
+        (int)(unsigned)((RO ? (long long)d.N * d.Hq * d.Wq : (long long)d.N * d.Di * d.Hi * d.Wi) * d.Cin * (long long)sizeof(T) + xbias), 0x00020000);
     const __amdgpu_buffer_rsrc_t rsrc_w = __builtin_amdgcn_make_buffer_rsrc(
         const_cast<char*>(reinterpret_cast<const char*>(d.wgt)), 0, (int)(unsigned)((long long)d.n_ch_tiles * BCH * d.Kpad * (long long)sizeof(T)), 0x00020000);
 
+    const long long res_rows = RO ? (long long)d.N * d.Hq * d.Wq : d.M;
     const __amdgpu_buffer_rsrc_t rsrc_r = __builtin_amdgcn_make_buffer_rsrc(
-        const_cast<char*>(reinterpret_cast<const char*>(d.res)), 0, (int)(unsigned)(d.M * d.ldo * (long long)sizeof(T)), 0x00020000);
+        const_cast<char*>(reinterpret_cast<const char*>(d.res)), 0, (int)(unsigned)(res_rows * d.ldo * (long long)sizeof(T)), 0x00020000);
     const __amdgpu_buffer_rsrc_t rsrc_i = __builtin_amdgcn_make_buffer_rsrc(
         const_cast<char*>(reinterpret_cast<const char*>(d.ident)), 0, (int)(unsigned)(256 * 256 * sizeof(T)), 0x00020000);
     long long mybase = 0;
-    unsigned mymask = 0;
-    int my_ch_tile = 0, my_pix_tile = 0;
+    unsigned mymask = 0, mynat = 0xffffffffu;
+    int my_ch_tile = 0;
+    unsigned itaps = 0x1ffu;
     auto prepare_tile = [&](int k) {
       int pix_tile, ch_tile;
       tile_of(k, pix_tile, ch_tile);
       my_ch_tile = ch_tile;
-      my_pix_tile = pix_tile;
       mybase = 0;
       mymask = 0;
+      mynat = 0xffffffffu;
+      if (RO) itaps = tile_taps(pix_tile);
       if (j < XR) {
         const long long m = d.m0 + (long long)pix_tile * BPIX + r0 + 32 * j;
         int xn = 0, xd0 = -(1 << 20), xh0 = 0, xw0 = 0;
         if (m < d.M) {
           unsigned n, qd, qh, qw;
-          decode_row(d, (unsigned)m, n, qd, qh, qw);
-          xn = (int)n * d.Di;
-          xd0 = (int)qd * d.sd - d.pd;
-          xh0 = (int)qh * d.sh - d.ph;
-          xw0 = (int)qw * d.sw - d.pw;
-        }
-        for (int kk = 0; kk < d.KD; ++kk) mymask |= (unsigned)((unsigned)(xd0 + kk * d.dild) < (unsigned)d.Di) << kk;
-        for (int kk = 0; kk < d.KH; ++kk) mymask |= (unsigned)((unsigned)(xh0 + kk * d.dilh) < (unsigned)d.Hi) << (8 + kk);
-        for (int kk = 0; kk < d.KW; ++kk) mymask |= (unsigned)((unsigned)(xw0 + kk * d.dilw) < (unsigned)d.Wi) << (16 + kk);
-        const long long pix0 = ((long long)(xn + xd0) * d.Hi + xh0) * d.Wi + xw0;
+          if (RO) {
+            qd = 0;
+            border_row_decode(d.N, d.Hq, d.Wq, d.dilh, d.dilw, (unsigned)m, n, qh, qw);
+            mynat = (n * (unsigned)d.Hq + qh) * (unsigned)d.Wq + qw;
+          } else {
+            decode_row(d, (unsigned)m, n, qd, qh, qw);
+            mynat = (unsigned)m;
+          }
+          xn = RO ? (int)n : (int)n * d.Di;
+          xd0 = RO ? 0 : (int)qd * d.sd - d.pd;
+          xh0 = RO ? (int)qh - d.dilh : (int)qh * d.sh - d.ph;
+          xw0 = RO ? (int)qw - d.dilw : (int)qw * d.sw - d.pw;
+        }
+        const int Hi = RO ? d.Hq : d.Hi, Wi = RO ? d.Wq : d.Wi;
+        if (RO) {
+          mymask |= (unsigned)(xd0 == 0);
+#pragma unroll
+          for (int kk = 0; kk < 3; ++kk) mymask |= (unsigned)((unsigned)(xh0 + kk * d.dilh) < (unsigned)Hi) << (8 + kk);
+#pragma unroll
+          for (int kk = 0; kk < 3; ++kk) mymask |= (unsigned)((unsigned)(xw0 + kk * d.dilw) < (unsigned)Wi) << (16 + kk);
+        } else {
+          for (int kk = 0; kk < d.KD; ++kk) mymask |= (unsigned)((unsigned)(xd0 + kk * d.dild) < (unsigned)d.Di) << kk;
+          for (int kk = 0; kk < d.KH; ++kk) mymask |= (unsigned)((unsigned)(xh0 + kk * d.dilh) < (unsigned)d.Hi) << (8 + kk);
+          for (int kk = 0; kk < d.KW; ++kk) mymask |= (unsigned)((unsigned)(xw0 + kk * d.dilw) < (unsigned)d.Wi) << (16 + kk);
+        }
+        const long long pix0 = ((long long)(xn + xd0) * Hi + xh0) * Wi + xw0;
         mybase = pix0 * d.Cin * (long long)sizeof(T);
-      }
+        if (RO) ltab[(k & 1) * BPIX + r0 + 32 * j] = mynat != 0xffffffffu ? mynat * (unsigned)(d.ldo * (int)sizeof(T)) : 0u;
+      }
+      if (RO) asm volatile("s_waitcnt lgkmcnt(0)" ::: "memory");
     };
     auto enter_tile = [&]() {
       const int grp = (tp & 63) & 56;
@@ -133,8 +166,8 @@
         rmask[i] = (unsigned)__shfl((int)mymask, grp | i, 64);
         xoff[i] = (unsigned)(b + xbias + (long long)(js * E) * (long long)sizeof(T));
         if (KR) {
-          const long long m = d.m0 + (long long)my_pix_tile * BPIX + r0 + 32 * i;
-          roff[i] = m < d.M ? (unsigned)((m * d.ldo + my_ch_tile * BCH + js * E) * (long long)sizeof(T)) : 0xffffffffu;
+          const unsigned nat = (unsigned)__shfl((int)mynat, grp | i, 64);
+          roff[i] = nat != 0xffffffffu ? (unsigned)(((long long)nat * d.ldo + my_ch_tile * BCH + js * E) * (long long)sizeof(T)) : 0xffffffffu;
         }
       }
 #pragma unroll
@@ -144,7 +177,12 @@
       }
       tkd = tkh = tkw = tc = 0;
       wko = 0;
-      if (kt0 > 0) {
+      if (RO) {
+        const int itap = __builtin_ctz(itaps);
+        tkh = (itap * 11) >> 5; tkw = itap - 3 * tkh;
+        wko = (unsigned)(itap * d.Cin) * (unsigned)sizeof(T);
+      }
+      if (!RO && kt0 > 0) {
         if (d.korder && d.lcin >= 0) {
           const int tap = kt0 % d.ntaps, cb = kt0 / d.ntaps;
           tkw = tap % d.KW; tkh = (tap / d.KW) % d.KH; tkd = tap / (d.KW * d.KH);
@@ -167,11 +205,13 @@
     auto issue = [&](int stage) {
       if (ikt == 0) enter_tile();
       const unsigned sbase = lds0 + (unsigned)stage * (STAGE * 16);
-      const unsigned sel = (1u << tkd) | (256u << tkh) | (65536u << tkw);
-      const unsigned soff = (unsigned)(((long long)((tkd * d.dild * d.Hi + tkh * d.dilh) * d.Wi + tkw * d.dilw) * d.Cin + tc) * (long long)sizeof(T));
-      const bool cok = tkd < d.KD && tc + js * E < d.Cin;
-      if (ikt >= KT) {
-        const unsigned ro = (unsigned)(ikt - KT) * (unsigned)(BK * sizeof(T));
+      const unsigned sel = (RO ? 1u : 1u << tkd) | (256u << tkh) | (65536u << tkw);
+      const unsigned soff = RO ? (unsigned)(((tkh * d.dilh * d.Wq + tkw * d.dilw) * d.Cin + tc) * (int)sizeof(T))
+                               : (unsigned)(((long long)((tkd * d.dild * d.Hi + tkh * d.dilh) * d.Wi + tkw * d.dilw) * d.Cin + tc) * (long long)sizeof(T));
+      const bool cok = (RO || tkd < d.KD) && tc + js * E < d.Cin;
+      const int iKT = taps_ksteps(itaps);
+      if (ikt >= iKT) {
+        const unsigned ro = (unsigned)(ikt - iKT) * (unsigned)(BK * sizeof(T));
 #pragma unroll
         for (int i = 0; i < XR; ++i) blds16(roff[i], rsrc_r, ro, sbase + (BCH * 8 + i * 256) * 16);
         if (!BIG) {
@@ -187,7 +227,19 @@
 #pragma unroll
         for (int i = 0; i < WL; ++i) blds16(woff[i], rsrc_w, wko, sbase + (i * 256) * 16);
       }
-      if (ikt >= KT) {
+      if (ikt >= iKT) {
+      } else if (RO) {
+        int itap = tkh * 3 + tkw;
+        const unsigned rest = itaps & ~((2u << itap) - 1u);
+        if (d.korder) {
+          if (rest) itap = __builtin_ctz(rest);
+          else { itap = __builtin_ctz(itaps); tc += BK; }
+        } else {
+          tc += BK;
+          if (tc >= d.Cin) { tc = 0; itap = rest ? __builtin_ctz(rest) : 0; }
+        }
+        tkh = (itap * 11) >> 5; tkw = itap - 3 * tkh;
+        wko = (unsigned)(itap * d.Cin + tc) * (unsigned)sizeof(T);
       } else if (d.korder && d.lcin >= 0) {
         wko += (unsigned)d.Cin * (unsigned)sizeof(T);
         if (++tkw == d.KW) { tkw = 0; if (++tkh == d.KH) { tkh = 0; if (++tkd == d.KD) { tkd = 0; tc += BK; wko = (unsigned)tc * (unsigned)sizeof(T); } } }
@@ -199,9 +251,12 @@
           if (++tkw == d.KW) { tkw = 0; if (++tkh == d.KH) { tkh = 0; ++tkd; } }
         }
       }
-      if (++ikt == KTT) { ikt = 0; ++itile; if (itile < n_my) prepare_tile(itile); }
+      if (++ikt == iKT + KR) { ikt = 0; ++itile; if (itile < n_my) prepare_tile(itile); }
     };
 
+    int total = 0;
+    for (int k = 0; k < n_my; ++k) total += tile_ksteps(k) + KR;
+    int cKTT = n_my > 0 ? tile_ksteps(0) + KR : 0;
     if (total > 0) prepare_tile(0);
     if (total > 0) issue(0);
     if (NST == 3 && total > 1) issue(1);
@@ -213,7 +268,7 @@
       if (NST == 3) { if (g + 2 < total) issue(st == 0 ? 2 : st - 1); }
       else { if (g + 1 < total) issue(st ^ 1); }
       st = st == NST - 1 ? 0 : st + 1;
-      if (STAGED) { if (++gk == KTT) { gk = 0; RGBM_BARRIER(); } }
+      if (STAGED) { if (++gk == cKTT) { gk = 0; RGBM_BARRIER(); cKTT = taps_ksteps(itaps) + KR; } }
     }
     return;
   }
@@ -261,6 +316,7 @@
   };
   int st = 0;
   for (int k = 0; k < n_my; ++k) {
+    const int KTt = tile_ksteps(k), KTTt = KTt + KR;
     {
       int pt, ct;
       tile_of(k, pt, ct);
@@ -296,7 +352,7 @@
         hi = make_uint4(c0.x, c0.y, c1.x, c1.y);
         lo = make_uint4(c0.z, c0.w, c1.z, c1.w);
       };
-      const int KTM = BIG ? KT : KTT;
+      const int KTM = BIG ? KTt : KTTt;
       for (int kt = 0; kt < KTM; ++kt) {
         asm volatile("s_waitcnt lgkmcnt(0)" ::: "memory");
         RGBM_BARRIER();
@@ -388,7 +444,7 @@
 #pragma unroll
       for (int a = 0; a < FA; ++a) ldAs(st, 0, a);
       __builtin_amdgcn_sched_barrier(0);
-      for (int kt = 0; kt + 1 < KT; ++kt) {
+      for (int kt = 0; kt + 1 < KTt; ++kt) {
         first3();
         if (M32_SHIFT) {
           asm volatile("s_waitcnt lgkmcnt(0)" ::: "memory");
@@ -456,7 +512,7 @@
       }
     } else {
       uint4 A0[FA], B0[FB], A1[FA], B1[FB];
-      for (int kt = 0; kt < KTT; ++kt) {
+      for (int kt = 0; kt < KTTt; ++kt) {
         asm volatile("s_waitcnt lgkmcnt(0)" ::: "memory");
         RGBM_BARRIER();
         load_step(st, 0, A0, B0);
@@ -542,6 +598,11 @@
     for (int b = 0; b < FB; ++b) {
       const long long m = d.m0 + (long long)pix_tile * BPIX + wpix + b * 32 + li;
       pok[b] = m < d.M;
+      if (RO) {
+        nn[b] = 0;
+        obase[b] = pok[b] ? (long long)(ltab[(k & 1) * BPIX + wpix + b * 32 + li] / (unsigned)sizeof(T)) : 0ll;
+        continue;
+      }
       if (dense_out && (interior || d.bias_stride == 0)) {
         nn[b] = 0;
         obase[b] = (pok[b] ? m : 0ll) * d.ldo;
@@ -606,12 +667,35 @@
 #pragma unroll
               for (int q = 0; q < NQ; ++q)
                 *reinterpret_cast<uint4*>(stg + (wofs ^ (unsigned)((a * 2 * NQ + q) << 4))) = pk[a][q];
+            if (RO) {
+              char* ob = reinterpret_cast<char*>(out + ch0 + ar * AR * 32);
+              const unsigned* tb = ltab + (k & 1) * BPIX + wpix + b * 32;
+              unsigned lq = (unsigned)lane;
+              asm volatile("" : "+v"(lq));
+              const unsigned tl = lq >> 4, cofs = (lq & 15u) * 16u;
+#pragma unroll
+              for (int t = 0; t < 8; ++t) {
+                const uint4 v = *reinterpret_cast<const uint4*>(stg + t * 1024 + (rofs ^ (unsigned)(((4 * t) & 15) << 4)));
+                const unsigned po = tb[4 * t + tl];
+                *reinterpret_cast<uint4*>(ob + (po + cofs)) = v;
+              }
+            } else {
             char* ob = reinterpret_cast<char*>(out + (mrow + b * 32) * d.ldo + ch0 + ar * AR * 32);
 #pragma unroll
             for (int t = 0; t < 8; ++t) {
               const uint4 v = *reinterpret_cast<const uint4*>(stg + t * 1024 + (rofs ^ (unsigned)(((4 * t) & 15) << 4)));
               *reinterpret_cast<uint4*>(ob + (long long)(4 * t) * d.ldo * (long long)sizeof(T) + gofs) = v;
             }
+            }
+          } else if (RO) {
+            unsigned lq = (unsigned)lane;
+            asm volatile("" : "+v"(lq));
+            const unsigned po = ltab[(k & 1) * BPIX + wpix + b * 32 + (lq & 31u)] + (lq >> 5) * (unsigned)(16 * sizeof(T));
+#pragma unroll
+            for (int a = 0; a < AR; ++a)
+#pragma unroll
+              for (int q = 0; q < NQ; ++q)
+                *reinterpret_cast<uint4*>(reinterpret_cast<char*>(out + ch0 + (ar * AR + a) * 32) + po + q * 16) = pk[a][q];
           } else {
 #pragma unroll
             for (int a = 0; a < AR; ++a)
@@ -685,10 +769,14 @@
   }
 }
 
-template <typename T, int BPIX, int BCH = 256>
+template <typename T, int BPIX, int BCH = 256, bool RO = false>
 static int launch_m32_range(ConvDesc d, hipStream_t s) {
+  if constexpr (!RO) {
+    if (d.row_order) return launch_m32_range<T, BPIX, BCH, true>(d, s);
+  }
   constexpr int NST = BPIX == 256 ? 2 : 3;
-  constexpr size_t LDS = ((size_t)NST * (BCH + BPIX) * 8) * sizeof(uint4) + 2560 * sizeof(float);
+  constexpr size_t LDS = ((size_t)NST * (BCH + BPIX) * 8) * sizeof(uint4) + 2560 * sizeof(float) + (RO ? 2 * BPIX * sizeof(unsigned) : 0);
+  static_assert(LDS <= 160 * 1024, "LDS of a CU");
   d.n_pix_tiles = (int)((d.M - d.m0 + BPIX - 1) / BPIX);
   d.n_ch_tiles = (d.Cout + BCH - 1) / BCH;
   const long long ntiles = (long long)d.n_pix_tiles * d.n_ch_tiles;
@@ -697,13 +785,14 @@
   make_fastdiv(d.Wq, d.fd_m[0], d.fd_s[0]);
   make_fastdiv(d.Hq, d.fd_m[1], d.fd_s[1]);
   make_fastdiv(d.Dq, d.fd_m[2], d.fd_s[2]);
-  if (int rc = ensure_dynamic_lds(reinterpret_cast<const void*>(conv_igemm_m32_kernel<T, BPIX, BCH>), (int)LDS)) return rc;
+  if (int rc = ensure_dynamic_lds(reinterpret_cast<const void*>(conv_igemm_m32_kernel<T, BPIX, BCH, RO>), (int)LDS)) return rc;
   int n_cu = 0;
   if (int rc = persistent_grid_cus(&n_cu)) return rc;
+  RGBM_REQUIRE(!RO || d.ksplit <= 1, "no K split in border-class order");
   RGBM_REQUIRE(d.ksplit <= 1 || (BPIX == 128 && BCH <= 128 && ntiles * d.ksplit <= 4096 && d.kscratch && d.kcount), "K split: 64 / 128-channel x 128-pixel tiles, one workgroup per (tile, part)");
   const int grid = d.ksplit > 1 ? (int)(ntiles * d.ksplit) : ntiles < n_cu ? (int)ntiles : n_cu;
   prof_begin_launch(s, BPIX == 256 && BCH == 256 ? (std::is_same<T, bx3_t>::value ? 33 : 31) : (std::is_same<T, bx3_t>::value ? 41 : 40), d.algo_flops, d.algo_bytes);
-  hipLaunchKernelGGL((conv_igemm_m32_kernel<T, BPIX, BCH>), dim3((unsigned)grid), dim3(BPIX == 256 ? 768 : 512), LDS, s, d);
+  hipLaunchKernelGGL((conv_igemm_m32_kernel<T, BPIX, BCH, RO>), dim3((unsigned)grid), dim3(BPIX == 256 ? 768 : 512), LDS, s, d);
   prof_end_launch(s);
   RGBM_CHECK_HIP(hipGetLastError());
   return 0;
@@ -760,6 +849,7 @@
   d.m0 = 0;
   d.ident = nullptr;
   d.korder = p.korder;
+  d.row_order = p.row_order;
   d.ksplit = 1; d.kscratch = nullptr; d.kcount = nullptr;
   if (p.ksplit > 1) {
     if (int rc = m32_ksplit_buffers(s, &d.kscratch, &d.kcount)) return rc;
diff --git a/rgbmanip_amd/csrc/conv_plan.cpp b/rgbmanip_amd/csrc/conv_plan.cpp
--- a/rgbmanip_amd/csrc/conv_plan.cpp
+++ b/rgbmanip_amd/csrc/conv_plan.cpp
@@ -29,6 +29,13 @@
   return d.KD == 1 && d.KH == 3 && d.KW == 3 && d.sd == 1 && d.sh == 1 && d.sw == 1 && d.Dq == 1 && d.Di == 1 &&
          d.dilh == d.dilw && d.dilw >= 1 && d.dilw <= 4 && d.ph == d.dilh && d.pw == d.dilw && d.pd == 0 &&
          d.lcin >= 6 && d.Hq == d.Hi && d.Wq == d.Wi && d.Wi > 2 * d.dilw && d.osh == 1 && d.osw == 1;
+}
+
+bool border_order_ok(const ConvDesc& d, bool dense_out, bool ident_ok, long long esz, int bk) {
+  return d.KD == 1 && d.KH == 3 && d.KW == 3 && d.sd == 1 && d.sh == 1 && d.sw == 1 && d.Dq == 1 && d.Di == 1 && d.pd == 0 &&
+         d.dilh >= 1 && d.dilw >= 1 && d.ph == d.dilh && d.pw == d.dilw && d.Hq == d.Hi && d.Wq == d.Wi && d.Hq >= 2 * d.dilh && d.Wq >= 2 * d.dilw &&
+         dense_out && d.lcin >= 0 && d.Cin % bk == 0 && d.KT == 9 * (d.Cin / bk) && d.M == (long long)d.N * d.Hq * d.Wq &&
+         d.M * d.ldo * esz < (1ll << 32) - 65536 && (d.bias == nullptr || d.bias_stride == 0) && (d.res_mode == RES_NONE || ident_ok);
 }
 
 int m32_small_choice(const ConvDesc& d, int n_cu, bool slim_ok) {
@@ -127,6 +134,7 @@
       }
       p.main_rows = Pm * 256;
       p.identity_residual = ident_ok;
+      p.row_order = t.gemm_tap_skip && uni && border_order_ok(d, dense_out, ident_ok, esz, conv_bk(dtype)) ? 1 : 0;
       p.tail_bch = p.main_rows == d.M ? 0 : 256;
       const long long pt = (d.M - p.main_rows + 127) / 128;
       if (p.tail_bch && t.gemm_kernel != 1 && !(f & DBG_M32_TAILS_R5)) {
diff --git a/rgbmanip_amd/csrc/conv_plan.h b/rgbmanip_amd/csrc/conv_plan.h
--- a/rgbmanip_amd/csrc/conv_plan.h
+++ b/rgbmanip_amd/csrc/conv_plan.h
@@ -8,6 +8,7 @@
   int gemm_kernel;
   long long ws_min_rows;
   int n_cu;
+  int gemm_tap_skip;
 };
 
 enum ConvKernel {
@@ -31,6 +32,7 @@
   int ksplit;
   bool identity_residual;
   int korder, buf_ok;
+  int row_order;
 };
 
 constexpr size_t kM32SplitFloats = 8u << 20, kM32SplitCounters = 16384;
diff --git a/rgbmanip_amd/csrc/conv_row_order.h b/rgbmanip_amd/csrc/conv_row_order.h
--- /dev/null
+++ b/rgbmanip_amd/csrc/conv_row_order.h
@@ -0,0 +1,51 @@
+#pragma once
+
+#if defined(__HIPCC__) || defined(__CUDACC__)
+#define RGBM_HD __host__ __device__ __forceinline__
+#else
+#define RGBM_HD inline
+#endif
+
+namespace rgbm {
+
+RGBM_HD int border_band_start(int n, int dil, int b) { return b == 0 ? 0 : b == 1 ? dil : n - dil; }
+RGBM_HD int border_band_len(int n, int dil, int b) { return b == 1 ? n - 2 * dil : dil; }
+RGBM_HD unsigned border_band_taps(int b) { return b == 0 ? 6u : b == 1 ? 7u : 3u; }
+
+RGBM_HD void border_row_decode(int N, int H, int W, int dh, int dw, unsigned m, unsigned& n, unsigned& y, unsigned& x) {
+  unsigned start = 0, hb = 1, wb = 1, y0 = 0, x0 = 0;
+  bool found = false;
+#pragma unroll
+  for (int r = 0; r < 9; ++r) {
+    const unsigned h = (unsigned)border_band_len(H, dh, r / 3), w = (unsigned)border_band_len(W, dw, r % 3);
+    const unsigned size = (unsigned)N * h * w;
+    if (!found && m - start < size) {
+      found = true;
+      hb = h; wb = w;
+      y0 = (unsigned)border_band_start(H, dh, r / 3); x0 = (unsigned)border_band_start(W, dw, r % 3);
+      m -= start;
+    }
+    start += size;
+  }
+  const unsigned per_view = hb * wb;
+  n = m / per_view;
+  const unsigned rem = m - n * per_view, yy = rem / wb;
+  y = y0 + yy;
+  x = x0 + (rem - yy * wb);
+}
+
+RGBM_HD unsigned border_tap_mask(int N, int H, int W, int dh, int dw, unsigned m, unsigned count) {
+  unsigned mask = 0, start = 0;
+#pragma unroll
+  for (int r = 0; r < 9; ++r) {
+    const unsigned size = (unsigned)N * (unsigned)border_band_len(H, dh, r / 3) * (unsigned)border_band_len(W, dw, r % 3);
+    if (size > 0 && start < m + count && m < start + size) {
+      const unsigned rows = border_band_taps(r / 3), cols = border_band_taps(r % 3);
+      mask |= ((rows & 1u) ? cols : 0u) | ((rows & 2u) ? cols << 3 : 0u) | ((rows & 4u) ? cols << 6 : 0u);
+    }
+    start += size;
+  }
+  return mask;
+}
+
+}
diff --git a/rgbmanip_amd/csrc/kernels.h b/rgbmanip_amd/csrc/kernels.h
--- a/rgbmanip_amd/csrc/kernels.h
+++ b/rgbmanip_amd/csrc/kernels.h
@@ -125,6 +125,7 @@
 extern long long g_ws_min_rows;
 extern int g_tuning_version;
 extern int g_gemm_kernel;
+extern int g_gemm_tap_skip;
 void conv3d_tile_pack(const float* w, const float* scale, int Cin, int Cout, int coutp, bool transposed, int dtype,
                       std::vector<float>& packed);
 int launch_conv3d_tile(int layer, int dtype, const Conv3dTileDesc& d, hipStream_t s);
```

After: 5973, median of 6. Within noise of the previous version (+0.2%).
